# kazuotani14/iLQR

Hardware: AMD Instinct MI355X
Metric: iLQR iterations/sec (batch x T timesteps/sec), acrobot T=500 batch=4096 (higher is better)
Workload: dtype f64; 1 GPU; acrobot n=4 m=1 T=499 (500 knots), box-QP limits active, FD derivatives + backward/box-QP + 11-alpha search + accept, fixed work; batch_per_gpu=4096, global_batch=4096, T=499, parallelism=batch shards x1, one all_gather of costs

## Files before the change

### ilqr_amd/batch.py

```python
import ctypes as C

import numpy as np

from . import capi

ALPHAS = np.array([1.0000, 0.5012, 0.2512, 0.1259, 0.0631, 0.0316, 0.0158, 0.0079, 0.0040,
                   0.0020, 0.0010])
STATUS_NAMES = {0: "running", 1: "converged_grad", 2: "converged_cost", 3: "lambda_max", 4: "max_iter"}
_MODELS = {"acrobot": (capi.MODEL_ACROBOT, 4, 1), "double_integrator": (capi.MODEL_DOUBLE_INTEGRATOR, 4, 2),
           "integrator": (capi.MODEL_DOUBLE_INTEGRATOR, 4, 2),
           "host": (capi.MODEL_HOST, None, None),
           "lq": (capi.MODEL_LQ, None, None),
           "user": (capi.MODEL_USER, None, None)}
_dp = C.POINTER(C.c_double)
_ip = C.POINTER(C.c_int)


def _c(a):
    return np.ascontiguousarray(a, dtype=np.float64)


def _p(a):
    return a.ctypes.data_as(_dp) if a is not None else None

# ... 397 lines not shown
        nw = int(C.shape[-1])
        Cc = self._mat_input(C, self.nx, nw)
        B, T, n, m = self.B, self.T, self.nx, self.nu
        o = dict(K=np.zeros((B, T, n, m)) if K else None,
                 k=np.zeros((B, T, m)) if k else None, Vx=np.zeros((B, T + 1, n)) if Vx else None,
                 Vxx=np.zeros((B, T + 1, n, n)) if Vxx else None, risk_cost=np.zeros(B) if risk_cost else None)
        flags = np.zeros(B, dtype=np.int32) if info else None
        self._check(self.lib.ilqr_get_risk_sensitive(self.h, nw, float(theta), capi.LQ_HOLD_CLAMPED if hold_clamped else 0, float(mu), _p(Cc),
                                                     _p(o["K"]), _p(o["k"]), _p(o["Vx"]), _p(o["Vxx"]), _p(o["risk_cost"]), _pi(flags)))
        out = {name: (np.swapaxes(a, -1, -2) if name in ("K", "Vxx") else a) for name, a in o.items() if a is not None}
        if info:
            out["info"] = flags
        return out

    def copy_risk_sensitive_to_device(self, nw, theta, C_ptr, mu=0.0, hold_clamped=False, K_ptr=None, k_ptr=None, Vx_ptr=None, Vxx_ptr=None,
                                      risk_cost_ptr=None, info_ptr=None):
        self._check(self.lib.ilqr_copy_risk_sensitive_to_device(self.h, int(nw), float(theta), capi.LQ_HOLD_CLAMPED if hold_clamped else 0,
                                                                float(mu), C_ptr, K_ptr, k_ptr, Vx_ptr, Vxx_ptr, risk_cost_ptr, info_ptr))

    def _dirs_input(self, a, lead, width, what):
        if a is None:
            return None, None, False
        a = _c(a)
        flat = a.ndim == 2 + len(lead)
        if flat:
            a = np.ascontiguousarray(a[..., None, :])
        if a.ndim != 3 + len(lead) or a.shape[:1 + len(lead)] != (self.B,) + lead or a.shape[-1] != width or a.shape[-2] < 1:
            raise ValueError("%s must be %s, or the same without the direction axis S; got %s" % (what, ["B"] + list(lead) + ["S", width], a.shape))
        return a, a.shape[-2], flat

    def _dirs_pair(self, x, u, what):
        (x, Sx, fx), (u, Su, fu) = x, u
        if x is None and u is None:
            raise ValueError("%s are both None: the answer would be zero" % what)
        if x is not None and u is not None and (Sx != Su or fx != fu):
            raise ValueError("%s disagree on the directions: %s and %s" % (what, x.shape, u.shape))
        return (Sx if x is not None else Su), (fx if x is not None else fu)

    def _nku(self, t0, n):
        return max(min(int(t0) + n, self.T) - int(t0), 0)

    def tangent(self, dx0=None, dv=None, t0=0, n=None):
        n = self.T + 1 - int(t0) if n is None else int(n)
        X, V = self._dirs_input(dx0, (), self.nx, "dx0"), self._dirs_input(dv, (self.T,), self.nu, "dv")
        S, flat = self._dirs_pair(X, V, "dx0 and dv")
        nku = self._nku(t0, n)
        dxs = np.zeros((self.B, max(n, 0), S, self.nx))
        dus = np.zeros((self.B, nku, S, self.nu))
        self._check(self.lib.ilqr_get_tangent(self.h, int(t0), n, S, _p(X[0]), _p(V[0]), _p(dxs), _p(dus) if nku else None))
        return (dxs[:, :, 0], dus[:, :, 0]) if flat else (dxs, dus)

    def adjoint(self, gx=None, gu=None, t0=0, n=None):
        n = self.T + 1 - int(t0) if n is None else int(n)
        nku = self._nku(t0, n)
        X, U = self._dirs_input(gx, (max(n, 0),), self.nx, "gx"), self._dirs_input(gu, (nku,), self.nu, "gu")
        S, flat = self._dirs_pair(X, U, "gx and gu")
        g_x0, g_v = np.zeros((self.B, S, self.nx)), np.zeros((self.B, self.T, S, self.nu))
        self._check(self.lib.ilqr_get_adjoint(self.h, int(t0), n, S, _p(X[0]), _p(U[0]), _p(g_x0), _p(g_v)))
        return (g_x0[:, 0], g_v[:, :, 0]) if flat else (g_x0, g_v)

    def transition_matrices(self, t0=0, n=None):
        dxs, dus = self.tangent(dx0=np.broadcast_to(np.eye(self.nx), (self.B, self.nx, self.nx)), t0=t0, n=n)
        return np.swapaxes(dxs, -1, -2), np.swapaxes(dus, -1, -2)

    def copy_tangent_to_device(self, t0, n, S, dx0_ptr=None, dv_ptr=None, dxs_ptr=None, dus_ptr=None):
        self._check(self.lib.ilqr_copy_tangent_to_device(self.h, int(t0), int(n), int(S), dx0_ptr, dv_ptr, dxs_ptr, dus_ptr))

    def copy_adjoint_to_device(self, t0, n, S, gx_ptr=None, gu_ptr=None, g_x0_ptr=None, g_v_ptr=None):
        self._check(self.lib.ilqr_copy_adjoint_to_device(self.h, int(t0), int(n), int(S), gx_ptr, gu_ptr, g_x0_ptr, g_v_ptr))

    def lq_solve(self, gx=None, gu=None, dx0=None, mu=0.0, hold_clamped=True, dlam=False):
        X = self._dirs_input(gx, (self.T + 1,), self.nx, "gx")
        U = self._dirs_input(gu, (self.T,), self.nu, "gu")
        X0 = self._dirs_input(dx0, (), self.nx, "dx0")
        given = [a for a in (X, U, X0) if a[0] is not None]
        if not given:
            raise ValueError("gx, gu and dx0 are all None: the answer would be zero")
        S, flat = given[0][1], given[0][2]
        if any(a[1] != S or a[2] != flat for a in given):
            raise ValueError("gx, gu and dx0 disagree on the directions: %s" % [a[0].shape for a in given])
        dxs, dus = np.zeros((self.B, self.T + 1, S, self.nx)), np.zeros((self.B, self.T, S, self.nu))
        lam = np.zeros((self.B, self.T + 1, S, self.nx)) if dlam else None
        info = np.zeros(self.B, dtype=np.int32)
        self._check(self.lib.ilqr_solve_lq(self.h, S, capi.LQ_HOLD_CLAMPED if hold_clamped else 0, float(mu), _p(X0[0]), _p(X[0]), _p(U[0]), _p(dxs),
                                           _p(dus), _p(lam), _pi(info)))
        out = (dxs, dus) + ((lam,) if dlam else ())
        if flat:
            out = tuple(a[:, :, 0] for a in out)
        return out + (info,)

    def copy_lq_solve_to_device(self, S, mu=0.0, hold_clamped=True, dx0_ptr=None, gx_ptr=None, gu_ptr=None, dxs_ptr=None, dus_ptr=None, dlam_ptr=None,
                                info_ptr=None):
        self._check(self.lib.ilqr_solve_lq_on_device(self.h, int(S), capi.LQ_HOLD_CLAMPED if hold_clamped else 0, float(mu), dx0_ptr, gx_ptr, gu_ptr,
                                                     dxs_ptr, dus_ptr, dlam_ptr, info_ptr))

    def derivatives(self):
        n, m, B, T1 = self.nx, self.nu, self.B, self.T + 1
        mem = dict(fx=np.zeros((B, T1, n, n)), fu=np.zeros((B, T1, m, n)), cx=np.zeros((B, T1, n)),
                   cu=np.zeros((B, T1, m)), cxx=np.zeros((B, T1, n, n)), cxu=np.zeros((B, T1, m, n)),
                   cuu=np.zeros((B, T1, m, m)))
        order = ("fx", "fu", "cx", "cu", "cxx", "cxu", "cuu")
        self._check(self.lib.ilqr_get_derivatives(self.h, *[_p(mem[k]) for k in order]))
        return {k: (v if k in ("cx", "cu") else np.swapaxes(v, -1, -2)) for k, v in mem.items()}

    def cost(self):
        c = np.zeros(self.B)
        self._check(self.lib.ilqr_get_cost(self.h, _p(c)))
        return c

    def lambdas(self):
        lam, dlam = np.zeros(self.B), np.zeros(self.B)
        self._check(self.lib.ilqr_get_lambda(self.h, _p(lam), _p(dlam)))
        return lam, dlam

    def dV(self):
        d = np.zeros((self.B, 2))
        self._check(self.lib.ilqr_get_dV(self.h, _p(d)))
        return d

    def gnorm(self):
        g = np.zeros(self.B)
        self._check(self.lib.ilqr_get_gnorm(self.h, _p(g)))
        return g

    def status(self):
        st, it, al = (np.zeros(self.B, dtype=np.int32) for _ in range(3))
        self._check(self.lib.ilqr_get_status(self.h, st.ctypes.data_as(_ip), it.ctypes.data_as(_ip),
                                            al.ctypes.data_as(_ip)))
        return st, it, al

    def candidate(self, a):
        xs = np.zeros((self.B, self.T + 1, self.nx))
        us = np.zeros((self.B, self.T, self.nu))
        self._check(self.lib.ilqr_get_candidate(self.h, int(a), _p(xs), _p(us)))
        return xs, us

    def count_running(self):
        n = C.c_int(0)
        self._check(self.lib.ilqr_count_running(self.h, C.byref(n)))
        return n.value

    def profile(self, enable=True):
        self._check(self.lib.ilqr_profile_enable(self.h, int(enable)))

    def profile_reset(self):
        self._check(self.lib.ilqr_profile_reset(self.h))

    def profile_read(self):
        ms = (C.c_double * capi.NUM_STAGES)()
        n = (C.c_int * capi.NUM_STAGES)()
        self._check(self.lib.ilqr_profile_read(self.h, ms, n))
        return {capi.STAGE_NAMES[i]: (ms[i], n[i]) for i in range(capi.NUM_STAGES)}

    def shader_clock_mhz(self):
        mhz = C.c_double(0)
        self._check(self.lib.ilqr_profile_shader_clock(self.h, C.byref(mhz)))
        return mhz.value
```

### ilqr_amd/capi.py

```python
import ctypes as C
import os

from . import _build

ABI_VERSION = 6
MODEL_ACROBOT, MODEL_DOUBLE_INTEGRATOR, MODEL_LQ, MODEL_HOST, MODEL_USER = 0, 1, 2, 3, 4
FLAG_FIXED_WORK, FLAG_BACKWARD_THREAD_PER_TRAJ, _FLAG_RESERVED_4, FLAG_UNFUSED, FLAG_ANALYTIC_DERIVATIVES, FLAG_STAGED, FLAG_REFERENCE_FIXES, FLAG_REGULARIZE_VXX = 1, 2, 4, 8, 16, 32, 64, 128
DTYPE_F64, DTYPE_F32 = 0, 1
TAIL_HOLD, TAIL_ZERO = 0, 1
RESET_NONFINITE, RESET_LAMBDA_MAX = 1, 2
WAS_MASKED, WAS_NONFINITE, WAS_LAMBDA_MAX = 1, 2, 4
WAS_CLONED, CLONE_REFUSED = 1, 2
LQ_HOLD_CLAMPED = 1
EVAL_CLAMP = 1
ROUTE_TILE_PER_CU, ROUTE_TWO_TILES_PER_CU, ROUTE_WIDE_TILES = 1, 2, 3
ROUTE_WIDE_ONE_PER_CU, ROUTE_WIDE_TWO_PER_CU, ROUTE_NO_COMPACTION, ROUTE_FULL_RECORDS, ROUTE_LQ_THREAD_ROLLOUT, ROUTE_QUAD_CHAIN, ROUTE_LQ_RECOMMIT, ROUTE_BACKWARD_W2, ROUTE_LQ_DENSE_FD = 4, 8, 16, 32, 64, 256, 512, 1024, 2048
ROUTE_WAVE_PER_TRAJECTORY = 4096
ROUTE_TWO_CONTROL_TILES = 8192
NUM_STAGES = 5
STAGE_NAMES = ("derivatives", "backward", "rollout", "accept", "solve")

_dp = C.POINTER(C.c_double)
_ip = C.POINTER(C.c_int)


class Params(C.Structure):
    _fields_ = [("max_iter", C.c_int), ("tol_fun", C.c_double), ("tol_grad", C.c_double),
                ("lambda_init", C.c_double), ("dlambda_init", C.c_double),
                ("lambda_factor", C.c_double), ("lambda_max", C.c_double),
                ("lambda_min", C.c_double), ("z_min", C.c_double)]


class Desc(C.Structure):
    _fields_ = [("abi_version", C.c_int), ("model", C.c_int), ("nx", C.c_int), ("nu", C.c_int),
                ("T", C.c_int), ("B", C.c_int), ("dt", C.c_double), ("device", C.c_int),
                ("flags", C.c_int), ("dtype", C.c_int), ("u_min", _dp), ("u_max", _dp), ("goal", _dp),
                ("lq_A", _dp), ("lq_B", _dp), ("lq_Q", _dp), ("lq_R", _dp), ("lq_Qf", _dp),
                ("stream", C.c_void_p), ("params", C.POINTER(Params)), ("user_params", _dp), ("n_user_params", C.c_int),
                ("route", C.c_int), ("assume_cus", C.c_int)]


_H = C.c_void_p
SYMBOLS = {
    "ilqr_last_error": (C.c_char_p, []),
    "ilqr_abi_version": (C.c_int, []),
    "ilqr_has_user_model": (C.c_int, []),
    "ilqr_default_params": (None, [C.POINTER(Params)]),
    "ilqr_create": (C.c_int, [C.POINTER(Desc), C.POINTER(_H)]),
    "ilqr_destroy": (None, [_H]),
    "ilqr_set_stream": (C.c_int, [_H, C.c_void_p]),
    "ilqr_synchronize": (C.c_int, [_H]),
    "ilqr_init_traj": (C.c_int, [_H, _dp, _dp, _dp]),
    "ilqr_generate_trajectory": (C.c_int, [_H]),
    "ilqr_solve": (C.c_int, [_H, _dp, _dp]),
    "ilqr_warm_start": (C.c_int, [_H, _dp]),
    "ilqr_iterate": (C.c_int, [_H, C.c_int]),
    "ilqr_shift_horizon": (C.c_int, [_H, C.c_int, C.c_int]),
    "ilqr_mpc_step": (C.c_int, [_H, _dp, C.c_void_p, C.c_int, C.c_int, C.c_int]),
    "ilqr_copy_controls_to_device": (C.c_int, [_H, C.c_int, C.c_int, C.c_void_p]),
    "ilqr_set_reset_controls": (C.c_int, [_H, _dp, C.c_void_p]),
    "ilqr_reset_trajectories": (C.c_int, [_H, _ip, C.c_void_p, C.c_int]),
    "ilqr_mpc_step_reset": (C.c_int, [_H, _dp, C.c_void_p, C.c_int, C.c_int, C.c_int, _ip, C.c_void_p, C.c_int]),
    "ilqr_get_reset_flags": (C.c_int, [_H, _ip]),
    "ilqr_copy_reset_flags_to_device": (C.c_int, [_H, C.c_void_p]),
    "ilqr_select_best": (C.c_int, [_H, C.c_int, _ip, C.c_void_p]),
    "ilqr_clone_trajectories": (C.c_int, [_H, _ip, C.c_void_p, C.c_void_p]),
    "ilqr_clone_best": (C.c_int, [_H, C.c_int, C.c_void_p]),
    "ilqr_get_clone_flags": (C.c_int, [_H, _ip]),
    "ilqr_copy_clone_flags_to_device": (C.c_int, [_H, C.c_void_p]),
    "ilqr_get_value": (C.c_int, [_H, C.c_int, C.c_int, _dp, _dp]),
    "ilqr_copy_value_to_device": (C.c_int, [_H, C.c_int, C.c_int, C.c_void_p, C.c_void_p]),
    "ilqr_get_covariance": (C.c_int, [_H, C.c_int, C.c_int, _dp, _dp, _dp, _dp, _dp]),
    "ilqr_copy_covariance_to_device": (C.c_int, [_H, C.c_int, C.c_int, C.c_void_p, C.c_void_p, C.c_void_p, C.c_void_p, C.c_void_p]),
    "ilqr_get_tangent": (C.c_int, [_H, C.c_int, C.c_int, C.c_int, _dp, _dp, _dp, _dp]),
    "ilqr_copy_tangent_to_device": (C.c_int, [_H, C.c_int, C.c_int, C.c_int, C.c_void_p, C.c_void_p, C.c_void_p, C.c_void_p]),
    "ilqr_get_adjoint": (C.c_int, [_H, C.c_int, C.c_int, C.c_int, _dp, _dp, _dp, _dp]),
    "ilqr_copy_adjoint_to_device": (C.c_int, [_H, C.c_int, C.c_int, C.c_int, C.c_void_p, C.c_void_p, C.c_void_p, C.c_void_p]),
    "ilqr_solve_lq": (C.c_int, [_H, C.c_int, C.c_int, C.c_double, _dp, _dp, _dp, _dp, _dp, _dp, _ip]),
    "ilqr_solve_lq_on_device": (C.c_int, [_H, C.c_int, C.c_int, C.c_double, C.c_void_p, C.c_void_p, C.c_void_p, C.c_void_p, C.c_void_p, C.c_void_p, C.c_void_p]),
    "ilqr_get_estimator": (C.c_int, [_H, C.c_int, C.c_int, C.c_int, _dp, _dp, _dp, _dp, _dp, _dp, _dp, _dp, _dp, _dp, _ip]),
    "ilqr_copy_estimator_to_device": (C.c_int, [_H, C.c_int, C.c_int, C.c_int] + [C.c_void_p] * 11),
    "ilqr_get_risk_sensitive": (C.c_int, [_H, C.c_int, C.c_double, C.c_int, C.c_double, _dp, _dp, _dp, _dp, _dp, _dp, _ip]),
    "ilqr_copy_risk_sensitive_to_device": (C.c_int, [_H, C.c_int, C.c_double, C.c_int, C.c_double] + [C.c_void_p] * 7),
    "ilqr_evaluate_policy": (C.c_int, [_H, C.c_int, C.c_int, C.c_int, C.c_int, _dp, _dp, _dp, _dp]),
    "ilqr_evaluate_policy_on_device": (C.c_int, [_H, C.c_int, C.c_int, C.c_int, C.c_int, C.c_void_p, C.c_void_p, C.c_void_p, C.c_void_p]),
    "ilqr_trajectory_params_count": (C.c_int, []),
    "ilqr_set_trajectory_params": (C.c_int, [_H, _dp, C.c_void_p, C.c_int]),
    "ilqr_get_trajectory_params": (C.c_int, [_H, _dp, C.c_int]),
    "ilqr_clear_trajectory_params": (C.c_int, [_H]),
    "ilqr_get_param_gradient": (C.c_int, [_H, C.c_int, C.c_int, C.c_double, _dp, _dp, _dp, _dp, _dp]),
    "ilqr_param_gradient_on_device": (C.c_int, [_H, C.c_int, C.c_int, C.c_double] + [C.c_void_p] * 5),
    "ilqr_compute_derivatives": (C.c_int, [_H]),
    "ilqr_backward_pass": (C.c_int, [_H, _ip]),
    "ilqr_backward_step": (C.c_int, [_H]),
    "ilqr_rollout_candidates": (C.c_int, [_H, _dp]),
    "ilqr_line_search": (C.c_int, [_H]),
    "ilqr_accept_candidates": (C.c_int, [_H, _dp, _ip]),
    "ilqr_reset_state": (C.c_int, [_H, C.c_int]),
    "ilqr_set_trajectory": (C.c_int, [_H, _dp, _dp, _dp, _dp]),
    "ilqr_set_gains": (C.c_int, [_H, _dp, _dp]),
    "ilqr_set_derivatives": (C.c_int, [_H] + [_dp] * 7),
    "ilqr_set_lambda": (C.c_int, [_H, _dp, _dp]),
    "ilqr_get_trajectory": (C.c_int, [_H, _dp, _dp]),
    "ilqr_get_gains": (C.c_int, [_H, _dp, _dp]),
    "ilqr_get_derivatives": (C.c_int, [_H] + [_dp] * 7),
    "ilqr_get_cost": (C.c_int, [_H, _dp]),
    "ilqr_get_lambda": (C.c_int, [_H, _dp, _dp]),
    "ilqr_get_dV": (C.c_int, [_H, _dp]),
    "ilqr_get_gnorm": (C.c_int, [_H, _dp]),
    "ilqr_get_status": (C.c_int, [_H, _ip, _ip, _ip]),
    "ilqr_get_candidate": (C.c_int, [_H, C.c_int, _dp, _dp]),
    "ilqr_count_running": (C.c_int, [_H, _ip]),
    "ilqr_copy_cost_to_device": (C.c_int, [_H, C.c_void_p]),
    "ilqr_copy_trajectory_to_device": (C.c_int, [_H, C.c_void_p, C.c_void_p]),
    "ilqr_copy_gains_to_device": (C.c_int, [_H, C.c_void_p, C.c_void_p]),
    "ilqr_get_results_async": (C.c_int, [_H, _dp, _dp, _dp, _dp, _dp]),
    "ilqr_host_register": (C.c_int, [C.c_void_p, C.c_size_t]),
    "ilqr_host_unregister": (C.c_int, [C.c_void_p]),
    "ilqr_group_create": (C.c_int, [C.POINTER(_H), C.c_int, C.c_int, C.POINTER(C.c_void_p)]),
    "ilqr_group_destroy": (None, [C.c_void_p]),
    "ilqr_group_gather_costs": (C.c_int, [C.c_void_p, _dp]),
    "ilqr_group_uses_rccl": (C.c_int, [C.c_void_p, _ip]),
    "ilqr_profile_enable": (C.c_int, [_H, C.c_int]),
    "ilqr_profile_reset": (C.c_int, [_H]),
    "ilqr_profile_read": (C.c_int, [_H, _dp, _ip]),
    "ilqr_profile_shader_clock": (C.c_int, [_H, _dp]),
    "ilqr_stage_kernel_name": (C.c_char_p, [_H, C.c_int]),
}

_lib = None
_libs = {}


class ILQRError(RuntimeError):
    pass


def lib_path():
    return _build.LIB


def _bind(path):
    lib = C.CDLL(path)
    for name, (res, args) in SYMBOLS.items():
        fn = getattr(lib, name)
        fn.restype = res
        fn.argtypes = args
    return lib


def load(build_if_missing=True, path=None):
    global _lib
    if path is not None:
        path = os.path.abspath(path)
        if path not in _libs:
            if not os.path.exists(path):
                raise ILQRError("%s is missing: build it with ilqr_amd._build.build_user(header, out)" % path)
            _libs[path] = _bind(path)
        return _libs[path]
    if _lib is None:
        if build_if_missing and os.path.exists(_build.HIPCC):
            _build.build()
        if not os.path.exists(_build.LIB):
            raise ILQRError("libilqr_amd.so is missing (%s): build it with "
                            "`python -m ilqr_amd._build`; there is no fallback path" % _build.LIB)
        lib = C.CDLL(os.environ.get("ILQR_AMD_LIB", _build.LIB))
        for name, (res, args) in SYMBOLS.items():
            fn = getattr(lib, name)
            fn.restype = res
            fn.argtypes = args
        _lib = lib
    return _lib


def check(rc, lib=None):
    if rc != 0:
        msg = (lib or load()).ilqr_last_error()
        raise ILQRError("libilqr_amd error %d: %s" % (rc, msg.decode() if msg else "?"))
```

### ilqr_amd/csrc/backward_hex.hpp

```cpp
#pragma once
#include "solve_tile.hpp"

namespace ilqr {

#ifndef ILQR_COMMIT_ROLLED
#define ILQR_COMMIT_ROLLED 1
#endif

#ifndef ILQR_COMMIT_BATCH
#define ILQR_COMMIT_BATCH 2
#endif
constexpr int kCommitBatch = ILQR_COMMIT_BATCH;

constexpr int HT = 4;
#ifndef ILQR_HEX_SLOT_PAD
#define ILQR_HEX_SLOT_PAD 8
#endif
#ifndef ILQR_HEX_PAIR_PERM
#define ILQR_HEX_PAIR_PERM 1
#endif
#ifndef ILQR_HEX_CAND_T
#define ILQR_HEX_CAND_T 1
#endif
constexpr bool kHexCandT = ILQR_HEX_CAND_T != 0;
#ifndef ILQR_HEX_QUAD_ROLLOUT
#define ILQR_HEX_QUAD_ROLLOUT 1
#endif
constexpr bool kHexQuadRollout = ILQR_HEX_QUAD_ROLLOUT != 0;
#ifndef ILQR_HEX_SLOT_PHASES
#define ILQR_HEX_SLOT_PHASES 4
#endif
constexpr int kHexSlotPhases = ILQR_HEX_SLOT_PHASES;
static_assert(kHexSlotPhases == 1 || kHexSlotPhases == 2 || kHexSlotPhases == 4, "backward_hex's step loop is written out for groups of 1, 2 or 4 knots");
#ifndef ILQR_HEX_MFMA_SPREAD
#define ILQR_HEX_MFMA_SPREAD 0
#endif
constexpr bool kHexMfmaSpread = ILQR_HEX_MFMA_SPREAD != 0;

template <int NX, int NU, class real, int SLOTS_, bool COMPACT_ = false>
struct HexRing {
  static constexpr bool COMPACT = COMPACT_;
  static constexpr int US = Rec<NX, NU>::SIZE;
  static constexpr int PAIRS = COMPACT ? CompactRec<NX, NU>::PAIRS : (Rec<NX, NU>::SIZE + NU + 1) / 2;
  static constexpr int ROW = 2 * HT;
  static constexpr int PAD = ROW - 2 * TW;
  static constexpr int ELEMS = PAIRS * ROW + ILQR_HEX_SLOT_PAD;
  static constexpr int Z = PAIRS * ROW;
  static_assert(!COMPACT || ILQR_HEX_SLOT_PAD >= ROW, "the compact slot keeps Z in its pad row");
  static_assert(!COMPACT || (NX == 4 && NU == 1), "compact slots: nx = 4, nu = 1");
  static constexpr int SLOTS = SLOTS_;
  static constexpr bool PERM = (ILQR_HEX_PAIR_PERM != 0) && NX == 4 && NU == 1;
  static constexpr int pos(int pair) { return PERM && (!COMPACT || pair < 8) ? hex_pair_pos(pair) : pair; }
};

constexpr int kHexKnotsPerRound = 64 / HT;
constexpr int kHexFullSlots = 24;
template <int NX, int NU, class real, bool COMPACT>
struct HexRingSize {
  using Full = HexRing<NX, NU, real, kHexFullSlots, false>;
  static constexpr int TERM = COMPACT ? ((NX + NX * NX) / 2) * Full::ROW : 0;
  static constexpr int FIT = COMPACT ? (kHexFullSlots * Full::ELEMS - TERM) / HexRing<NX, NU, real, 1, COMPACT>::ELEMS : kHexFullSlots;
  static constexpr int SLOTS = FIT / kHexSlotPhases * kHexSlotPhases;
  static_assert(SLOTS % kHexSlotPhases == 0 && kHexKnotsPerRound % kHexSlotPhases == 0, "the ring and a producer round are whole groups of slots");
  static constexpr int LEAD = SLOTS - kHexKnotsPerRound - 1;
  static constexpr int STALE = kHexSlotPhases - 1;
  static_assert(SLOTS > LEAD + kHexKnotsPerRound - 1, "a round must not reach a slot the chain has not left");
  static_assert(LEAD - STALE >= 1, "the producer is released ahead of the chain, the published index being up to STALE knots old");
  static_assert(SLOTS * HexRing<NX, NU, real, 1, COMPACT>::ELEMS + TERM <= kHexFullSlots * Full::ELEMS, "the pair's records fit the bytes of 24 full slots");
};

template <class real, int N>
struct HexTerm {
  alignas(16) real term[N];
};
template <class real>
struct HexTerm<real, 0> {
  static constexpr real* term = nullptr;
};

template <class real, int NX, int NU, bool COMPACT = false>
struct HexPair : HexTerm<real, HexRingSize<NX, NU, real, COMPACT>::TERM> {
  using Size = HexRingSize<NX, NU, real, COMPACT>;
  using RS = HexRing<NX, NU, real, Size::SLOTS, COMPACT>;
  static constexpr int LEAD = Size::LEAD;
  alignas(16) real ring[RS::SLOTS * RS::ELEMS];
  int rounds_done;
  int consumer_at;
  int passes_started;
  unsigned long long pass_lanes;
};

template <class P>
struct HexGate {
  static constexpr bool kRing = true;
  static constexpr int NPH = kHexSlotPhases;
  static constexpr int GROUP = NPH * P::RS::ELEMS, RING = P::RS::SLOTS * P::RS::ELEMS;
  P& sh;
  const int T, nrounds, N;
  int pass = -1, have = 0;
  int g_grp = 0, off_grp = 0;
  __device__ __forceinline__ HexGate(P& s, int T_) : sh(s), T(T_), nrounds((T_ + 1 + kHexKnotsPerRound - 1) / kHexKnotsPerRound), N(nrounds * kHexKnotsPerRound) {}
  __device__ __forceinline__ int begin_pass() {
    pass++;
    have = pass * N;
    g_grp = pass * N;
    const int was = off_grp;
    off_grp = (g_grp % P::RS::SLOTS) * P::RS::ELEMS;
    __hip_atomic_store(&sh.pass_lanes, __ballot(1), __ATOMIC_RELAXED, __HIP_MEMORY_SCOPE_WORKGROUP);
    __hip_atomic_store(&sh.passes_started, pass + 1, __ATOMIC_RELEASE, __HIP_MEMORY_SCOPE_WORKGROUP);
    return off_grp - was;
  }
  __device__ __forceinline__ int next_group() {
    g_grp += NPH;
    const int d = (off_grp + GROUP == RING) ? GROUP - RING : GROUP;
    off_grp += d;
    return d;
  }
  template <int PH>
  __device__ __forceinline__ void wait() {
    if constexpr (PH != 0) return;
    const int G = g_grp;
    __hip_atomic_store(&sh.consumer_at, G, __ATOMIC_RELAXED, __HIP_MEMORY_SCOPE_WORKGROUP);
    if (G < have) return;
    const int round = pass * nrounds + (G - pass * N) / kHexKnotsPerRound;
    while (__hip_atomic_load(&sh.rounds_done, __ATOMIC_ACQUIRE, __HIP_MEMORY_SCOPE_WORKGROUP) <= round) __builtin_amdgcn_s_sleep(1);
    have = pass * N + ((G - pass * N) / kHexKnotsPerRound + 1) * kHexKnotsPerRound;
  }
  __device__ __forceinline__ void finish() {
    __hip_atomic_store(&sh.consumer_at, 0x3fffffff, __ATOMIC_RELAXED, __HIP_MEMORY_SCOPE_WORKGROUP);
    __hip_atomic_store(&sh.passes_started, -1, __ATOMIC_RELEASE, __HIP_MEMORY_SCOPE_WORKGROUP);
  }
};

__device__ __forceinline__ int hex_first(unsigned long long bal, int t4) {
  return __builtin_ctzll(((bal >> t4) & 0x000F000F000F000Full) | 0x8000000000000000ull);
}
template <class Under>
__device__ __forceinline__ void qp1_search_hex(QP1StateT<double>& q, int j, int t4, double step_j0, const double* __restrict__ lds_steps, Under under_read) {
  const double t_x1 = clamp_of(q.x + step_j0 * q.search, q.lo, q.hi);
  const double t_v1 = qp1_value(q, t_x1);
  const bool t_pass = !qp1_armijo_fails(q, t_v1, step_j0);
  const int pp = hex_first(__ballot(t_pass), t4);
  const bool success = pp < 52;
  const int jw = success ? (((pp >> 4) << 2) | (pp & 3)) : 0;
#ifdef ILQR_EXP_NO_STEP_LDS
  const double step_w = jw == 0 ? 1.0 : 0.6;
#else
  const double step_w = lds_steps[jw];
#endif
  under_read();
  q.step = step_w;
  q.x1 = clamp_of(q.x + q.step * q.search, q.lo, q.hi);
  q.v1 = qp1_value(q, q.x1);
  bool more = p_and(!success, !q.early);
  if (__builtin_expect(__ballot(more) == 0ull, 1)) return;
  {
    const bool stuck = p_and(j >= 1, t_x1 == q.x);
    const int qs = hex_first(__ballot(p_and(stuck, more)), t4);
    if (p_and(more, qs < 52)) {
      q.ls_failed = true;
      more = false;
    }
    if (__ballot(more) == 0ull) return;
  }
  for (int base = 16;; base += 16) {
    const int kn = base + j;
    const double my_step = lds_steps[kn < 104 ? kn : 103];
    const double my_x1 = qp1_trial(q, my_step);
    const double my_v1 = qp1_value(q, my_x1);
    const bool pass = !qp1_armijo_fails(q, my_v1, my_step);
    const bool stuck = p_or(my_step < kMinStep, my_x1 == q.x);
    const int qp = hex_first(__ballot(p_and(pass, more)), t4), qs = hex_first(__ballot(p_and(stuck, more)), t4);
    if (more) {
      if (qp < qs) {
        q.step = lds_steps[base + (((qp >> 4) << 2) | (qp & 3))];
        q.x1 = qp1_trial(q, q.step);
        q.v1 = qp1_value(q, q.x1);
        more = false;
      } else if (qs < 52) {
        q.ls_failed = true;
        more = false;
      }
    }
    if (__ballot(more) == 0ull) return;
  }
}

template <class RS>
__device__ __forceinline__ int hex_pos_rt(int pair) { return RS::pos(pair); }

template <class real>
struct HexStep {
  typedef real pair_t __attribute__((ext_vector_type(2)));
  real F, cxx_rc, cxx_cr, fu_r, cx_r, cxu_r, cxu_c;
  pair_t tail, uw;
};

template <class M, class Gate, class RS>
__device__ __forceinline__ void backward_hex(const BatchViewT<typename M::real>& v, const M& model, const SolverParams& sp, int mode, int tile, int sub,
                                             int lane, const double* __restrict__ lds_steps, Gate& gate, const typename M::real* __restrict__ ring,
                                             const typename M::real* __restrict__ term ) {
  using real = typename M::real;
  using creal = double;
  static_assert(M::NX == 4 && M::NU == 1, "hex chain: nx = 4, nu = 1");
  using R = Rec<4, 1>;
  typedef real real2_t __attribute__((ext_vector_type(2)));
  const int r_ = lane >> 4, t_ = (lane >> 2) & 3, c_ = lane & 3, j16 = 4 * r_ + c_;
  const int t4 = 4 * t_;
  const int l = sub * HT + t_;
  const int b = tile * TW + l;
  if (b >= v.B) return;
  if (mode == 1 && v.status[b] != 0) return;
  const int T = v.T;
  double lambda = v.lambda[b], dlambda = v.dlambda[b];
  const real* __restrict__ ust = v.us + tidx(tile, 0, 0, l, T, 1);
  real* __restrict__ kt = v.kff + tidx(tile, 0, 0, l, T, 1);
  real* __restrict__ Kt = v.Kfb + tidx(tile, 0, 0, l, T, 4);
  typedef const __attribute__((address_space(3))) real lds_cd;
  typedef const __attribute__((address_space(3))) real2_t lds_cd2;
  const creal step_j0 = lds_steps[j16];
  auto mm = [](creal a, creal bb) __attribute__((always_inline)) { return __builtin_amdgcn_mfma_f64_4x4x4f64(a, bb, 0.0, 0, 0, 0); };

  using C = CompactRec<4, 1>;
  enum { A_ROW, A_FX, A_FU, A_CXX_RC, A_CXX_CR, A_CX, A_CXU_R, A_CXU_C, A_FULL };
  constexpr int NADDR = RS::COMPACT ? A_FU + 1 : A_FULL;
  lds_cd* at[NADDR];
  {
    lds_cd* r = (lds_cd*)(ring + t_ * 2);
    auto one = [&](int e) { return r + hex_pos_rt<RS>(e >> 1) * RS::ROW + (e & 1); };
    at[A_ROW] = r;
    at[A_FX] = one((RS::COMPACT ? C::FX : R::FX) + r_ + 4 * c_);
    at[A_FU] = one((RS::COMPACT ? C::FU : R::FU) + r_);
    if constexpr (!RS::COMPACT) {
      at[A_CXX_RC] = one(R::CXX + r_ + 4 * c_);
      at[A_CXX_CR] = one(R::CXX + c_ + 4 * r_);
      at[A_CX] = one(R::CX + r_);
      at[A_CXU_R] = one(R::CXU + r_);
      at[A_CXU_C] = one(R::CXU + c_);
    }
  }
  auto move = [&](int d) __attribute__((always_inline)) {
#pragma unroll
    for (int a = 0; a < NADDR; a++) at[a] += d;
  };
  constexpr int NPH = kHexSlotPhases;
  auto load = [&](auto phase, HexStep<real>& d) __attribute__((always_inline)) {
    constexpr int PH = decltype(phase)::value, o = PH * RS::ELEMS;
    gate.template wait<PH>();
    auto pair = [&](int e) { return *(lds_cd2*)(at[A_ROW] + o + RS::pos(e >> 1) * RS::ROW); };
    if constexpr (RS::COMPACT) {
      d.F = at[A_FX][o];
      d.fu_r = at[A_FU][o];
      d.cxx_rc = d.cxx_cr = d.cx_r = d.cxu_r = d.cxu_c = at[A_ROW][o + RS::Z];
      d.tail = pair(C::CU);
      d.uw = pair(C::US);
    } else {
      d.F = at[A_FX][o];
      d.cxx_rc = at[A_CXX_RC][o];
      d.cxx_cr = at[A_CXX_CR][o];
      d.fu_r = at[A_FU][o];
      d.cx_r = at[A_CX][o];
      d.cxu_r = at[A_CXU_R][o];
      d.cxu_c = at[A_CXU_C][o];
      d.tail = pair(R::CU);
      d.uw = pair(RS::US);
    }
    if constexpr (PH == NPH - 1) move(gate.next_group());
  };

  int diverge = 0;
  bool done = false;
  double dV0 = 0, dV1 = 0, gacc = 0;
  auto one_pass = [&]() __attribute__((always_inline)) {
    move(gate.begin_pass());
    creal V, RVx, kprev;
    const creal lam_r = (creal)lambda;
    {
      gate.template wait<0>();
      if constexpr (RS::COMPACT) {
        lds_cd* r = (lds_cd*)(term + t_ * 2);
        RVx = (creal)r[((C::TERM_CX + r_) >> 1) * RS::ROW + ((C::TERM_CX + r_) & 1)];
        V = (creal)r[((C::TERM_CXX + r_ + 4 * c_) >> 1) * RS::ROW + ((C::TERM_CXX + r_ + 4 * c_) & 1)];
      } else {
        RVx = (creal)at[A_CX][0];
        V = (creal)at[A_CXX_RC][0];
      }
      if constexpr (NPH == 1) move(gate.next_group());
    }
    kprev = (creal)kt[(unsigned)((T - 1) * TW)];
    __builtin_amdgcn_s_waitcnt(0x0F70);
    dV0 = dV1 = 0;
    diverge = 0;
    gacc = 0;
    real* __restrict__ Kt_i = Kt + (unsigned)(((T - 1) * 4 + c_) * TW);
    real* __restrict__ kt_i = kt + (unsigned)((T - 1) * TW);

    auto step = [&](auto phase, int i, const HexStep<real>& raw, HexStep<real>& nxt) -> bool {
      const creal F = (creal)raw.F, Rfu = (creal)raw.fu_r;
      const creal cu = (creal)raw.tail.x, cuu = (creal)raw.tail.y, us = (creal)raw.uw.x, usw = (creal)raw.uw.y;
      creal W, aQx, Tm, Tt, aQux_c, aQux_r;
      auto products_1 = [&]() __attribute__((always_inline)) {
        W = mm(V, F);
        aQx = mm(F, RVx);
        Tm = mm(F, W);
      };
      auto products_2 = [&]() __attribute__((always_inline)) {
        Tt = mm(W, F);
        aQux_c = mm(Rfu, W);
        aQux_r = mm(W, Rfu);
      };
      const creal wv = mm(V, Rfu);
      const creal aQu = mm(Rfu, RVx);
      const creal aQuu = mm(Rfu, wv);
      if constexpr (!kHexMfmaSpread) {
        products_1();
        products_2();
      }
      const creal Qu = cu + aQu;
      const creal Quu = cuu + aQuu, QuuF = (cuu + lam_r) + aQuu;
      const creal lo = (creal)model.u_min[0] - us, hi = (creal)model.u_max[0] - us;
      __builtin_amdgcn_sched_barrier(0);
      if (i >= 1) load(phase, nxt);
      __builtin_amdgcn_sched_barrier(0);
      creal x;
      int free0;
      creal minv;
      QP1StateT<creal> q1;
      qp1_begin<false>(QuuF, Qu, kprev, lo, hi, q1, false);
      qp1_search_hex(q1, j16, t4, step_j0, lds_steps, [&]() __attribute__((always_inline)) {
        if constexpr (kHexMfmaSpread) {
          __builtin_amdgcn_sched_barrier(0);
          products_1();
          __builtin_amdgcn_sched_barrier(0);
        }
      });
      if constexpr (kHexMfmaSpread) products_2();
      bool goes_on;
      bool ok = qp1_finish_ok(q1, x, free0, minv, goes_on);
      if (goes_on)
        ok = qp1_continue(
                 q1, [&](QP1StateT<creal>& qs) __attribute__((always_inline)) { qp1_search_hex(qs, j16, t4, step_j0, lds_steps, [] {}); }, x, free0) >= 1;
      if (!ok) diverge = i;
      const creal Qxx_rc = (creal)raw.cxx_rc + Tm, Qxx_cr = (creal)raw.cxx_cr + Tt;
      const creal Qx_r = (creal)raw.cx_r + aQx;
      const creal Qux_c = (creal)raw.cxu_c + aQux_c, Qux_r = (creal)raw.cxu_r + aQux_r;
      const creal k_scale = free0 ? -minv : creal(0);
      const creal K_r = k_scale * Qux_r, K_c = k_scale * Qux_c;
      creal d0 = 0, d1 = 0;
      {
        d0 += x * Qu;
        creal rq = 0;
        rq += (creal(0.5) * x) * Quu;
        d1 += rq * x;
      }
      creal T1_r, T1_c;
      {
        creal acc = 0;
        acc += K_r * Quu;
        T1_r = acc;
      }
      {
        creal acc = 0;
        acc += K_c * Quu;
        T1_c = acc;
      }
      creal Vxn_r, Vn_rc, Vn_cr;
      {
        creal t1 = 0, t2 = 0, t3 = 0;
        t1 += T1_r * x;
        t2 += K_r * Qu;
        t3 += Qux_r * x;
        Vxn_r = ((Qx_r + t1) + t2) + t3;
      }
      {
        creal u1 = 0, u2 = 0, u3 = 0;
        u1 += T1_r * K_c;
        u2 += K_r * Qux_c;
        u3 += Qux_r * K_c;
        Vn_rc = ((Qxx_rc + u1) + u2) + u3;
      }
      {
        creal u1 = 0, u2 = 0, u3 = 0;
        u1 += T1_c * K_r;
        u2 += K_c * Qux_r;
        u3 += Qux_c * K_r;
        Vn_cr = ((Qxx_cr + u1) + u2) + u3;
      }
      V = creal(0.5) * (Vn_rc + Vn_cr);
      RVx = Vxn_r;
      if (ok) {
        dV0 += (double)d0;
        dV1 += (double)d1;
        gacc += (double)(abs_of(x) * usw);
        kprev = (creal)(real)x;
        Kt_i[0] = (real)K_c;
        kt_i[0] = (real)x;
      }
      Kt_i -= 4 * TW;
      kt_i -= TW;
      return ok;
    };

    HexStep<real> A, Bd;
    int i = T - 1;
    auto ph = [](auto n) { return std::integral_constant<int, decltype(n)::value % NPH>(); };
    load(ph(std::integral_constant<int, 1>()), A);
    while (true) {
      if (!step(ph(std::integral_constant<int, 2>()), i, A, Bd)) break;
      if (--i < 0) break;
      if (!step(ph(std::integral_constant<int, 3>()), i, Bd, A)) break;
      if (--i < 0) break;
      if constexpr (NPH == 4) {
        if (!step(ph(std::integral_constant<int, 4>()), i, A, Bd)) break;
        if (--i < 0) break;
        if (!step(ph(std::integral_constant<int, 5>()), i, Bd, A)) break;
        if (--i < 0) break;
      }
    }
  };

  while (true) {
    one_pass();
    if (mode == 0) {
      done = (diverge == 0);
      break;
    }
    if (diverge != 0) {
      dlambda = raised_dlambda(dlambda, sp);
      lambda = raised_lambda(lambda, dlambda, sp);
      if (lambda > sp.lambda_max) break;
      continue;
    }
    done = true;
    break;
  }

  double acc = gacc;
  if (!done) {
    __builtin_amdgcn_fence(__ATOMIC_RELEASE, "workgroup");
    __builtin_amdgcn_s_waitcnt(0);
    acc = 0;
    for (int t0 = 0; t0 < T; t0 += 8) {
      real kv[8], uv[8];
#pragma unroll
      for (int jj = 0; jj < 8; jj++) {
        const int t = (t0 + jj < T) ? t0 + jj : T - 1;
        kv[jj] = kt[(size_t)t * TW];
        uv[jj] = ust[(size_t)t * TW];
      }
#pragma unroll
      for (int jj = 0; jj < 8; jj++) {
        const real mx = abs_of(kv[jj]) / (abs_of(uv[jj]) + 1);
        if (t0 + jj < T) acc += (double)mx;
      }
    }
  }
  const double gnorm = acc / T;
  if (j16 == 0) {
    v.dV[b] = dV0;
    v.dV[v.Bp + b] = dV1;
    v.diverge[b] = diverge;
    v.backpass_done[b] = done ? 1 : 0;
    v.gnorm[b] = gnorm;
    if (mode == 1) {
      v.lambda[b] = lambda;
      v.dlambda[b] = dlambda;
      if (!sp.fixed_work && gnorm < sp.tol_grad && lambda < kLambdaConverged) {
        v.status[b] = 1;
        v.iters[b] += 1;
      }
    }
  }
}

template <class M, class MFD, class P>
__device__ __forceinline__ void sweep_backward_hex(const BatchViewT<typename M::real>& v, const M& model, const MFD& fdm, const SolverParams& sp, int mode,
                                                   int force, int tile, P* pairs, const double* __restrict__ lds_steps, int role) {
  using RS = typename P::RS;
  const int lane = threadIdx.x & 63;
  if (threadIdx.x < 4) {
    pairs[threadIdx.x].rounds_done = 0;
    pairs[threadIdx.x].consumer_at = 0;
    pairs[threadIdx.x].passes_started = 0;
  }
  __syncthreads();
  const int T = v.T;
  P& sh = pairs[role & 3];
  if (role < 4) {
    __builtin_amdgcn_s_setprio(3);
    HexGate<P> gate(sh, T);
    backward_hex<M, decltype(gate), RS>(v, model, sp, mode, tile, role, lane, lds_steps, gate, sh.ring, sh.term);
    gate.finish();
    __builtin_amdgcn_s_setprio(0);
  } else {
    const int sub = role - 4;
    const int lp = lane & (HT - 1), ks = lane >> 2;
    const int l = sub * HT + lp;
    const int nrounds = (T + 1 + kHexKnotsPerRound - 1) / kHexKnotsPerRound, N = nrounds * kHexKnotsPerRound;
    for (int pass = 0;; pass++) {
      unsigned long long lanes = ~0ull;
      if (pass > 0) {
        int started;
        while ((started = __hip_atomic_load(&sh.passes_started, __ATOMIC_ACQUIRE, __HIP_MEMORY_SCOPE_WORKGROUP)) >= 0 && started <= pass)
          __builtin_amdgcn_s_sleep(8);
        if (started < 0) break;
        lanes = __hip_atomic_load(&sh.pass_lanes, __ATOMIC_RELAXED, __HIP_MEMORY_SCOPE_WORKGROUP);
      }
      const bool mine = (lanes >> (4 * lp)) & 1ull;
      for (int r = 0; r < nrounds; r++) {
        const int j0 = r * kHexKnotsPerRound, G0 = pass * N + j0;
        while (G0 > __hip_atomic_load(&sh.consumer_at, __ATOMIC_RELAXED, __HIP_MEMORY_SCOPE_WORKGROUP) + P::LEAD) __builtin_amdgcn_s_sleep(4);
        const int started = __hip_atomic_load(&sh.passes_started, __ATOMIC_RELAXED, __HIP_MEMORY_SCOPE_WORKGROUP);
        if ((started < 0) | (started > pass + 1)) break;
        const int t = T - (j0 + ks);
        if (t >= 0 && (pass == 0 || mine)) {
          typename M::real* rs = sh.ring + ((G0 + ks) % RS::SLOTS) * RS::ELEMS + lp * 2;
          if constexpr (RS::COMPACT) {
            if (t == T) rs = sh.term + lp * 2;
          }
          derivatives_of_knot<M, true, MFD, RS::PAD, RS::PERM, RS::COMPACT>(v, model, fdm, force, nullptr, tile, t, l, rs, true);
        }
        __builtin_amdgcn_s_waitcnt(0xC07F);
        if (lane == 0) __hip_atomic_store(&sh.rounds_done, pass * nrounds + r + 1, __ATOMIC_RELEASE, __HIP_MEMORY_SCOPE_WORKGROUP);
      }
    }
  }
}

template <class M, bool CANDT = false>
__device__ __forceinline__ void commit_tile_chunks(const BatchViewT<typename M::real>& v, const M& model, const int* commit_of_lane , int tile) {
  using real = typename M::real;
  constexpr int NX = M::NX, NU = M::NU;
  static_assert(!CANDT || (NX == 4 && NU == 1 && CT == 8 && CG == 4), "grouped candidates: nx = 4, nu = 1");
  static_assert(HT == kQuad, "a chain wavefront rolls out its own sub-tile");
  const int T = v.T;
  const real dt = (real)v.dt;
  const int ntask = v.nch * TW;
  struct Task {
    int l, c;
    real x[NX], uq[CT][NU];
  };
  auto load = [&](int task, Task& k) __attribute__((always_inline)) {
    k.l = 0;
    k.c = -1;
    if (task < 0) return;
    const int l = task & (TW - 1), c = task >> 4;
    const int b = tile * TW + l;
    const int ci = (b < v.B) ? commit_of_lane[l] : -1;
    if (ci < 0) return;
    k.l = l;
    k.c = c;
    const int ta = ci * v.ntiles + tile;
    real* const x = k.x;
    real(*const uq)[NU] = k.uq;
    if constexpr (CANDT) {
      typedef real real4v __attribute__((ext_vector_type(4)));
      const real4v xv = *reinterpret_cast<const real4v*>(v.cand_x + cand_g_x(ta, c, l, v.nch, NX));
      x[0] = xv.x;
      x[1] = xv.y;
      x[2] = xv.z;
      x[3] = xv.w;
      const real4v u0 = *reinterpret_cast<const real4v*>(v.cand_u + cand_g_u(ta, 2 * c, l, T));
      const real4v u1 = *reinterpret_cast<const real4v*>(v.cand_u + cand_g_u(ta, 2 * c + 1, l, T));
      uq[0][0] = u0.x;
      uq[1][0] = u0.y;
      uq[2][0] = u0.z;
      uq[3][0] = u0.w;
      uq[4][0] = u1.x;
      uq[5][0] = u1.y;
      uq[6][0] = u1.z;
      uq[7][0] = u1.w;
    } else {
#pragma unroll
    for (int i = 0; i < NX; i++) x[i] = v.cand_x[tidx(ta, c, i, l, v.nch, NX)];
#pragma unroll
    for (int q = 0; q < CT; q++) {
      const int tq = (c * CT + q < T) ? c * CT + q : T - 1;
#pragma unroll
      for (int jj = 0; jj < NU; jj++) uq[q][jj] = v.cand_u[tidx(ta, tq, jj, l, T, NU)];
    }
    }
  };
  auto steps = [&](Task& k) __attribute__((always_inline)) {
    if (k.c < 0) return;
    const int l = k.l, c = k.c;
    real* const x = k.x;
    real(*const uq)[NU] = k.uq;
#if ILQR_COMMIT_ROLLED
#pragma unroll 1
    for (int q = 0; q < CT; q++) {
      const int t = c * CT + q;
      if (t > T) break;
#pragma unroll
      for (int i = 0; i < NX; i++) v.xs[tidx(tile, t, i, l, T + 1, NX)] = x[i];
      if (t < T) {
#pragma unroll
        for (int jj = 0; jj < NU; jj++) v.us[tidx(tile, t, jj, l, T, NU)] = uq[0][jj];
        if (q + 1 < CT) {
          real x1[NX];
          integrate_dynamics(model, x, uq[0], dt, x1);
#pragma unroll
          for (int i = 0; i < NX; i++) x[i] = x1[i];
        }
      }
#pragma unroll
      for (int qq = 0; qq + 1 < CT; qq++)
#pragma unroll
        for (int jj = 0; jj < NU; jj++) uq[qq][jj] = uq[qq + 1][jj];
    }
#else
#pragma unroll
    for (int q = 0; q < CT; q++) {
      const int t = c * CT + q;
      if (t <= T) {
#pragma unroll
        for (int i = 0; i < NX; i++) v.xs[tidx(tile, t, i, l, T + 1, NX)] = x[i];
        if (t < T) {
#pragma unroll
          for (int jj = 0; jj < NU; jj++) v.us[tidx(tile, t, jj, l, T, NU)] = uq[q][jj];
          if (q + 1 < CT) {
            real x1[NX];
            integrate_dynamics(model, x, uq[q], dt, x1);
#pragma unroll
            for (int i = 0; i < NX; i++) x[i] = x1[i];
          }
        }
      }
    }
#endif
  };
  for (int first = ntask - 1 - (int)threadIdx.x; first >= 0; first -= kCommitBatch * (int)blockDim.x) {
    Task k[kCommitBatch];
#pragma unroll
    for (int j = 0; j < kCommitBatch; j++) load(first - j * (int)blockDim.x, k[j]);
#pragma unroll
    for (int j = 0; j < kCommitBatch; j++) steps(k[j]);
  }
}

template <class M, class MFD>
__global__ __launch_bounds__(512) __attribute__((amdgpu_waves_per_eu(2, 2))) void k_solve_hex(BatchViewT<typename M::real> v, M model, MFD fdm, AlphaSet alphas,
                                                                                                 SolverParams sp, int n_iters, int force,
                                                                                                 int* __restrict__ commit_idx, int commit_pending,
                                                                                                 long long* __restrict__ phase_ticks) {
  using real = typename M::real;
  using P = HexPair<real, M::NX, M::NU, state_free_running_cost<M>::value>;
  __shared__ P pairs[4];
  __shared__ double steps[104];
  __shared__ double lds_cost[NALPHA * TW];
  __shared__ int tile_running;
  __shared__ int simd_count[4];
  __shared__ int lds_commit[TW];
  if (threadIdx.x < 4) simd_count[threadIdx.x] = 0;
  load_step_table(steps);
  const int wave = (int)(threadIdx.x >> 6);
  int role = wave;
  {
    const int simd = hw_simd_id();
    int slot = 0;
    if ((threadIdx.x & 63) == 0) slot = atomicAdd(&simd_count[simd], 1);
    slot = __shfl(slot, 0, 64);
    __syncthreads();
    if (simd_count[0] == 2 && simd_count[1] == 2 && simd_count[2] == 2 && simd_count[3] == 2) role = simd + 4 * slot;
  }
  const int rwave = kHexQuadRollout ? ((role < 4) ? role : 4) : ((role < 3) ? role : 3);
  const int tile = blockIdx.x;
  constexpr int kShareReals = 4 * ((2 * M::NU + M::NU * M::NX + M::NX + 3) / 4) * TW;
  static_assert(kShareReals <= (int)(sizeof(pairs[0].ring) / sizeof(real)), "a pair's ring holds a wavefront's rollout rows");
  long long t_sweep = 0, t_roll = 0, t0 = 0;
#ifdef ILQR_HEX_SECTIONS
  long long t_sweep_last = 0;
#endif
  const bool timing = (phase_ticks != nullptr) & (threadIdx.x == 0);
  const long long c_begin = timing ? clock64() : 0, w_begin = timing ? wall_clock64() : 0;
  if (commit_pending) {
    commit_tile_chunks<M>(v, model, commit_idx + tile * TW, tile);
    phase_barrier();
  }
  int it = 0;
  for (; it < n_iters; it++) {
    if (timing) t0 = wall_clock64();
    sweep_backward_hex<M, MFD, P>(v, model, fdm, sp, 1, force, tile, pairs, steps, role);
    phase_barrier();
    if (timing) {
      const long long t1 = wall_clock64();
#ifdef ILQR_HEX_SECTIONS
      t_sweep_last = t1 - t0;
#endif
      t_sweep += t1 - t0;
      t0 = t1;
    }
    rollout_tile<M, true, true, kDeepPrefetch<M>, true, true, true, 1, kHexCandT, kHexQuadRollout>(v, model, alphas, NALPHA, v.cost_c, 1, sp, commit_idx, tile, lds_cost, it == n_iters - 1, rwave,
                                               pairs[role & 3].ring);
#ifdef ILQR_HEX_SECTIONS
#define ILQR_HEX_MARK(n)                                   \
    if (ILQR_HEX_SECTIONS == n && timing) {                \
      const long long t1 = wall_clock64();                 \
      t_sweep = t_sweep - t_sweep_last + (t1 - t0);        \
      t0 = t1;                                             \
    }
#else
#define ILQR_HEX_MARK(n)
#endif
    ILQR_HEX_MARK(1)
    if (threadIdx.x < TW) lds_commit[threadIdx.x] = commit_idx[tile * TW + threadIdx.x];
    if (threadIdx.x == 0) tile_running = 0;
    phase_barrier();
    ILQR_HEX_MARK(2)
    commit_tile_chunks<M, kHexCandT>(v, model, lds_commit, tile);
    ILQR_HEX_MARK(3)
    phase_barrier();
    if (timing) t_roll += wall_clock64() - t0;
    if (!sp.fixed_work) {
      const int b = tile * TW + (int)threadIdx.x;
      if (threadIdx.x < TW && b < v.B && v.status[b] == 0) tile_running = 1;
      __syncthreads();
      if (!tile_running) {
        it++;
        break;
      }
    }
  }
  if (timing) {
    phase_ticks[5 * tile + 0] += t_sweep;
    phase_ticks[5 * tile + 1] += t_roll;
    phase_ticks[5 * tile + 2] += it;
    phase_ticks[5 * tile + 3] += clock64() - c_begin;
    phase_ticks[5 * tile + 4] += wall_clock64() - w_begin;
  }
}

}
```

### ilqr_amd/csrc/capi.hip

```cpp
#include "../../include/ilqr_amd.h"

#include <stdarg.h>
#include <stdio.h>
#include <limits.h>
#include <string.h>

#include <algorithm>
#include <cstdlib>
#include <string>
#include <vector>

#include "backward_wave.hpp"
#include "backward_wave2.hpp"
#include "backward_wave3.hpp"
#include "generic.hpp"
#include "kernels_wide.hpp"
#include "kernels_wide2.hpp"
#include "kernels.hpp"
#include "value_thread.hpp"
#include "value_wave.hpp"
#include "covariance_thread.hpp"
#include "covariance_wave.hpp"
#include "sensitivity_thread.hpp"
#include "sensitivity_wave.hpp"
#include "lq_solve_thread.hpp"
#include "lq_solve_wave.hpp"
#include "estimator_thread.hpp"
#include "estimator_wave.hpp"
#include "risk_thread.hpp"
#include "risk_wave.hpp"
#include "evaluate.hpp"
#include "param_gradient.hpp"
#include "clone.hpp"

using namespace ilqr;

#include "route.hpp"
#include "handle.hpp"
#include "launch.hpp"

extern "C" {

const char* ilqr_last_error(void) { return g_err; }
int ilqr_abi_version(void) { return ILQR_AMD_ABI_VERSION; }
int ilqr_has_user_model(void) {
#ifdef ILQR_HAVE_USER_MODEL
  return 1;
#else
  return 0;
#endif
}

void ilqr_default_params(ilqr_params* p) {
  p->max_iter = 100;
  p->tol_fun = 1e-6;
  p->tol_grad = 1e-6;
  p->lambda_init = 1;
  p->dlambda_init = 1;
  p->lambda_factor = 1.6;
  p->lambda_max = 1e11;
  p->lambda_min = 1e-8;
  p->z_min = 0;
}

void ilqr_destroy(ilqr_batch* h) {
  if (!h) return;
  (void)hipSetDevice(h->device);
  if (h->stream) (void)hipStreamSynchronize(h->stream);
#ifdef ILQR_W2_TIMING
  if (h->aos) {
    long long st[8], qp[8], cnt[4];
    if (hipMemcpyFromSymbol(st, HIP_SYMBOL(g_w2_cycles), sizeof(st)) == hipSuccess && hipMemcpyFromSymbol(qp, HIP_SYMBOL(g_q_cycles), sizeof(qp)) == hipSuccess &&
        hipMemcpyFromSymbol(cnt, HIP_SYMBOL(g_q_counts), sizeof(cnt)) == hipSuccess && cnt[0] > 0) {
      const double q = (double)cnt[0];
      fprintf(stderr, "[k_backward_w2, wavefront 0] shader cycles per step: load+Qx/Qu %.0f  Vxx'fx,Vxx'fu %.0f  Qxx/Qux/Quu %.0f  box-QP %.0f  K %.0f  dV+T1+Vx %.0f  Vn+symmetrise+stores %.0f  (loop top %.0f)\n",
              st[0] / q, st[1] / q, st[2] / q, st[3] / q, st[4] / q, st[5] / q, st[6] / q, st[7] / q);
      fprintf(stderr, "[box-QP] per QP: %.2f iterations, %.2f factorisations, %.2f Armijo trips beyond the first; cycles: gradient+clamp set %.0f  Cholesky %.0f  inverse+R^-1R^-T %.0f  direction %.0f  line search %.0f  rest %.0f\n",
              cnt[1] / q, cnt[2] / q, cnt[3] / q, qp[0] / q, qp[1] / q, qp[2] / q, qp[3] / q, qp[4] / q, qp[5] / q);
    }
    long long w3[4];
    if (hipMemcpyFromSymbol(w3, HIP_SYMBOL(g_w3_counts), sizeof(w3)) == hipSuccess && w3[0] + w3[1] > 0)
      fprintf(stderr, "[k_backward_w3, wavefront 0] box-QPs on the matrix-core path %lld, handed to the literal path %lld, Newton-Schulz iterations per refinement %.2f\n",
              w3[0], w3[1], (double)w3[2] / (double)(w3[0] > 0 ? w3[0] : 1));
  }
#endif
  for (void* p : h->allocs) (void)hipFree(p);
  if (h->staging) (void)hipFree(h->staging);
  if (h->lq_scratch) (void)hipFree(h->lq_scratch);
  if (h->est_scratch) (void)hipFree(h->est_scratch);
  if (h->pg_scratch) (void)hipFree(h->pg_scratch);
  if (h->d_perm) (void)hipFree(h->d_perm);
  if (h->perm_scratch) (void)hipFree(h->perm_scratch);
  (void)timers_drain(h);
  for (hipEvent_t e : h->event_pool) (void)hipEventDestroy(e);
  if (h->own_stream && h->stream) (void)hipStreamDestroy(h->stream);
  delete h;
}

static int check_desc(const ilqr_desc* d) {
  REQUIRE(d->abi_version == ILQR_AMD_ABI_VERSION || d->abi_version == 5, "ABI version %d, library is %d (accepts 5 and %d)", d->abi_version,
          ILQR_AMD_ABI_VERSION, ILQR_AMD_ABI_VERSION);
  REQUIRE(d->B >= 1 && d->T >= 1 && d->nx >= 1 && d->nu >= 1, "B, T, nx, nu must be positive");
  REQUIRE(d->nx <= MAXN && d->nu <= kMaxControls, "nx <= %d and nu <= %d", MAXN, kMaxControls);
  REQUIRE(d->dt > 0, "dt must be positive");
  if (d->route & 128)
    return fail(ILQR_ERR_UNSUPPORTED, "route bit 128 (round 1's LDS kernel k_backward_w) was retired in ABI 5: ILQR_ROUTE_BACKWARD_W2 gives the same bits");
  if ((d->route & ILQR_ROUTE_WIDE_TWO_PER_CU) && d->nu == 2 && d->nx == 4)
    return fail(ILQR_ERR_UNSUPPORTED, "ILQR_ROUTE_WIDE_TWO_PER_CU: the m = 2 wide tiles (k_solve_wide2) run one tile per CU (four wavefronts at <= 512 registers); the bit applies to k_solve_wide (m = 1)");
  if (d->dtype != ILQR_DTYPE_F64 && d->dtype != ILQR_DTYPE_F32) return fail(ILQR_ERR_INVALID, "dtype %d: ILQR_DTYPE_F64 or ILQR_DTYPE_F32", d->dtype);
  if (d->nu > WM) {
    const char* what = (d->dtype == ILQR_DTYPE_F32) ? "fp32" : (d->route & ILQR_ROUTE_BACKWARD_W2) ? "ILQR_ROUTE_BACKWARD_W2" : (d->route & ILQR_ROUTE_LQ_DENSE_FD) ? "ILQR_ROUTE_LQ_DENSE_FD"
                       : (d->flags & ILQR_FLAG_REGULARIZE_VXX) ? "ILQR_FLAG_REGULARIZE_VXX" : nullptr;
    if (what) return fail(ILQR_ERR_UNSUPPORTED, "%s supports at most %d controls (nu = %d)", what, WM, d->nu);
  }
  if ((d->route & ILQR_ROUTE_TWO_CONTROL_TILES) && (d->route & ILQR_ROUTE_BACKWARD_W2))
    return fail(ILQR_ERR_UNSUPPORTED, "ILQR_ROUTE_TWO_CONTROL_TILES and ILQR_ROUTE_BACKWARD_W2 name two different backward kernels");
  if ((d->route & ILQR_ROUTE_TWO_CONTROL_TILES) && (d->flags & ILQR_FLAG_REGULARIZE_VXX))
    return fail(ILQR_ERR_UNSUPPORTED, "ILQR_FLAG_REGULARIZE_VXX is implemented in k_backward_w3 (at most 16 controls): drop ILQR_ROUTE_TWO_CONTROL_TILES");
  const bool aos = generic_layout(d->model, d->route, kUserTiled, kUserSmall);
  if (d->dtype == ILQR_DTYPE_F32 && aos) {
    if (d->model == ILQR_MODEL_HOST)
      return fail(ILQR_ERR_UNSUPPORTED, "fp32 is not available for ILQR_MODEL_HOST: the caller evaluates the model and owns its records (fp64)");
    if (d->route & ILQR_ROUTE_BACKWARD_W2)
      return fail(ILQR_ERR_UNSUPPORTED, "fp32 is not available on ILQR_ROUTE_BACKWARD_W2 (the literal-order fp64 cross-check): fp32 handles run k_backward_w3");
    if (d->route & ILQR_ROUTE_TWO_CONTROL_TILES)
      return fail(ILQR_ERR_UNSUPPORTED, "fp32 is not available on ILQR_ROUTE_TWO_CONTROL_TILES: fp32 handles run k_backward_w3 with one control tile");
  }
  if (d->model == ILQR_MODEL_ACROBOT) {
    REQUIRE(d->nx == 4 && d->nu == 1, "acrobot is nx=4 nu=1 (include/acrobot.h:27-28), got %d/%d", d->nx, d->nu);
  } else if (d->model == ILQR_MODEL_DOUBLE_INTEGRATOR) {
    REQUIRE(d->nx == 4 && d->nu == 2, "double integrator is nx=4 nu=2 (include/double_integrator.h:16-17), got %d/%d", d->nx, d->nu);
#ifdef ILQR_HAVE_USER_MODEL
  } else if (d->model == ILQR_MODEL_USER) {
    using UM = UserModelT<double>;
    REQUIRE(d->nx == UM::NX && d->nu == UM::NU, "this build's user model is nx=%d nu=%d, got %d/%d", UM::NX, UM::NU, d->nx, d->nu);
    REQUIRE(d->u_min && d->u_max, "ILQR_MODEL_USER needs u_min/u_max (Model::u_min/u_max, include/model.h:17)");
    REQUIRE(!(d->flags & ILQR_FLAG_ANALYTIC_DERIVATIVES) || has_analytic_record<UM>::value, "this user model has no analytic_record()");
    if (aos && kUserSmall) REQUIRE(d->dtype == ILQR_DTYPE_F64, "ILQR_ROUTE_WAVE_PER_TRAJECTORY on a small twin is the fp64 cross-check of its tiled kernels: fp64 only");
    REQUIRE(d->n_user_params >= 0 && (d->n_user_params == 0 || d->user_params), "ILQR_MODEL_USER: n_user_params = %d with user_params = %p", d->n_user_params, (const void*)d->user_params);
#endif
  } else if (d->model == ILQR_MODEL_HOST || d->model == ILQR_MODEL_LQ) {
    REQUIRE(d->nx <= WN && d->nu <= WMW, "generic kernels: nx <= %d, nu <= %d", WN, WMW);
    REQUIRE(d->u_min && d->u_max, "generic handles need u_min/u_max (Model::u_min/u_max, include/model.h:17)");
    if (d->model == ILQR_MODEL_LQ)
      REQUIRE(d->lq_A && d->lq_B && d->lq_Q && d->lq_R && d->lq_Qf, "ILQR_MODEL_LQ needs lq_A, lq_B, lq_Q, lq_R, lq_Qf");
  } else {
    return fail(ILQR_ERR_UNSUPPORTED, "model id %d is not available in this build", d->model);
  }
  if ((d->flags & ILQR_FLAG_REGULARIZE_VXX) && aos && (d->route & ILQR_ROUTE_BACKWARD_W2))
    return fail(ILQR_ERR_UNSUPPORTED, "ILQR_FLAG_REGULARIZE_VXX on the generic path is implemented in k_backward_w3: drop ILQR_ROUTE_BACKWARD_W2");
  return 0;
}

static void copy_desc(const ilqr_desc* d, ilqr_batch* h) {
  h->lq_wide = d->model == ILQR_MODEL_LQ && d->nu > WM;
  h->route.full_records = (d->route & ILQR_ROUTE_FULL_RECORDS) != 0;
  h->route.no_compaction = (d->route & ILQR_ROUTE_NO_COMPACTION) != 0;
  h->route.wide_occ = (d->route & ILQR_ROUTE_WIDE_ONE_PER_CU) ? 1 : (d->route & ILQR_ROUTE_WIDE_TWO_PER_CU) ? 2 : 0;
  h->aos = generic_layout(d->model, d->route, kUserTiled, kUserSmall);
  h->model = d->model; h->dtype = d->dtype; h->flags = d->flags;
  h->nx = d->nx; h->nu = d->nu; h->T = d->T; h->B = d->B; h->dt = d->dt;
  h->Bp = ((d->B + 63) / 64) * 64;
  h->ntiles = h->Bp / TW;
  if (d->params)
    h->params = *d->params;
  else
    ilqr_default_params(&h->params);
}

static int open_device(const ilqr_desc* d, ilqr_batch* h) {
  int ndev = 0;
  if (hipGetDeviceCount(&ndev) != hipSuccess || ndev <= 0)
    return fail(ILQR_ERR_NO_DEVICE, "no HIP device visible: libilqr_amd has no CPU path");
  if (d->device < 0 || d->device >= ndev) return fail(ILQR_ERR_NO_DEVICE, "device %d out of range (%d visible)", d->device, ndev);
  HIPCHK(hipSetDevice(d->device));
  h->device = d->device;
  HIPCHK(hipDeviceGetAttribute(&h->num_cus, hipDeviceAttributeMultiprocessorCount, d->device));
  if (d->assume_cus > 0) h->num_cus = d->assume_cus;
  int khz = 0;
  if (hipDeviceGetAttribute(&khz, hipDeviceAttributeWallClockRate, d->device) == hipSuccess && khz > 0) h->wall_clock_khz = khz;
  h->stream = (hipStream_t)d->stream;
  h->own_stream = !d->stream;
  if (h->own_stream) HIPCHK(hipStreamCreateWithFlags(&h->stream, hipStreamNonBlocking));
  return 0;
}

static void set_model_params(const ilqr_desc* d, ilqr_batch* h) {
  if (d->model == ILQR_MODEL_ACROBOT) {
    AcrobotModel& m = h->acrobot;
    m.goal[0] = 3.1415;
    m.goal[1] = m.goal[2] = m.goal[3] = 0;
    m.u_min[0] = d->u_min ? d->u_min[0] : -5.0;
    m.u_max[0] = d->u_max ? d->u_max[0] : 5.0;
    if (h->dtype == ILQR_DTYPE_F32) {
      AcrobotModelT<float>& f = h->acrobot_f;
      for (int i = 0; i < 4; i++) m.goal[i] = (double)(f.goal[i] = (float)m.goal[i]);
      m.u_min[0] = (double)(f.u_min[0] = (float)m.u_min[0]);
      m.u_max[0] = (double)(f.u_max[0] = (float)m.u_max[0]);
    }
  } else if (d->model == ILQR_MODEL_DOUBLE_INTEGRATOR) {
    DoubleIntegratorModel& m = h->dint;
    const double g0[4] = {1.0, 0.5, 0.0, 0.0};
    for (int i = 0; i < 4; i++) m.goal[i] = d->goal ? d->goal[i] : g0[i];
    for (int j = 0; j < 2; j++) {
      m.u_min[j] = d->u_min ? d->u_min[j] : -0.5;
      m.u_max[j] = d->u_max ? d->u_max[j] : 0.5;
    }
    if (h->dtype == ILQR_DTYPE_F32) {
      DoubleIntegratorModelT<float>& f = h->dint_f;
      for (int i = 0; i < 4; i++) m.goal[i] = (double)(f.goal[i] = (float)m.goal[i]);
      for (int j = 0; j < 2; j++) {
        m.u_min[j] = (double)(f.u_min[j] = (float)m.u_min[j]);
        m.u_max[j] = (double)(f.u_max[j] = (float)m.u_max[j]);
      }
    }
#ifdef ILQR_HAVE_USER_MODEL
  } else if (d->model == ILQR_MODEL_USER) {
    using UM = UserModelT<double>;
    h->user_f.set_params(d->user_params, d->n_user_params);
    if (h->dtype == ILQR_DTYPE_F32) {
      std::vector<double> p32(d->user_params, d->user_params + (d->user_params ? d->n_user_params : 0));
      for (double& q : p32) q = (double)(float)q;
      h->user.set_params(p32.data(), (int)p32.size());
    } else {
      h->user.set_params(d->user_params, d->n_user_params);
    }
    for (int j = 0; j < UM::NU; j++) {
      h->user_f.u_min[j] = (float)d->u_min[j];
      h->user_f.u_max[j] = (float)d->u_max[j];
      h->user.u_min[j] = (h->dtype == ILQR_DTYPE_F32) ? (double)h->user_f.u_min[j] : d->u_min[j];
      h->user.u_max[j] = (h->dtype == ILQR_DTYPE_F32) ? (double)h->user_f.u_max[j] : d->u_max[j];
    }
    static_cast<UM&>(h->user_g) = h->user;
    static_cast<UserModelT<float>&>(h->user_gf) = h->user_f;
#endif
  }
}

static int alloc_arrays(const ilqr_desc* d, ilqr_batch* h) {
  const size_t nt = h->ntiles, T = h->T, T1 = h->T + 1, nx = h->nx, nu = h->nu, REC = rec_of(h), Bp = h->Bp;
  BatchView& v = h->v;
  v.B = h->B; v.Bp = h->Bp; v.ntiles = h->ntiles; v.T = h->T; v.dt = h->dt;
  v.analytic = (h->flags & ILQR_FLAG_ANALYTIC_DERIVATIVES) ? 1 : 0;
  v.D = nullptr;
  int rc = 0;
  if (h->aos) {
    const size_t Bn = h->B;
    v.nch = 0;
    rc |= dev_alloc_real(h, &v.x0, Bn * nx);
    rc |= dev_alloc_real(h, &v.xs, Bn * T1 * nx);
    rc |= dev_alloc_real(h, &v.us, Bn * T * nu);
    rc |= dev_alloc_real(h, &v.kff, Bn * T * nu);
    rc |= dev_alloc_real(h, &v.Kfb, Bn * T * nu * nx);
    rc |= dev_alloc(h, &h->const_rec, 2 * REC + GN);
    rc |= dev_alloc(h, &h->d_umin, nu);
    rc |= dev_alloc(h, &h->d_umax, nu);
    v.cand_u = nullptr;
    v.cand_x = nullptr;
    if (lq_matrix_core_search(d->model, d->nu, d->route) && !(d->route & ILQR_ROUTE_LQ_RECOMMIT) && d->dtype == ILQR_DTYPE_F64) {
      void *cx = nullptr, *cu = nullptr;
      if (hipMalloc(&cx, Bn * NALPHA * T1 * nx * sizeof(double)) == hipSuccess && hipMalloc(&cu, Bn * NALPHA * T * nu * sizeof(double)) == hipSuccess) {
        h->allocs.push_back(cx);
        h->allocs.push_back(cu);
        v.cand_x = (double*)cx;
        v.cand_u = (double*)cu;
      } else {
        if (cx) (void)hipFree(cx);
        (void)hipGetLastError();
      }
    }
  } else {
    rc |= dev_alloc_real(h, &v.x0, nt * nx * TW);
    const size_t slack = rollout_fetch_slack_elems(h->nx, h->nu);
    rc |= dev_alloc_real(h, &v.xs, nt * T1 * nx * TW + slack);
    rc |= dev_alloc_real(h, &v.us, nt * T * nu * TW + slack);
    rc |= dev_alloc_real(h, &v.kff, nt * T * nu * TW + slack);
    rc |= dev_alloc_real(h, &v.Kfb, nt * T * nu * nx * TW + slack);
    v.nch = h->T / CT + 1;
    rc |= dev_alloc_real(h, &v.cand_u, (size_t)(NALPHA + 1) * nt * (size_t)(cand_groups(T) * CG) * nu * TW);
    rc |= dev_alloc_real(h, &v.cand_x, (size_t)(NALPHA + 1) * nt * v.nch * nx * TW);
  }
  rc |= dev_alloc(h, &v.cost_c, (size_t)NALPHA * Bp);
  for (double** p : {&v.cost, &v.lambda, &v.dlambda, &v.gnorm}) rc |= dev_alloc(h, p, Bp);
  for (int** p : {&v.status, &v.iters, &v.flg_change, &v.alpha_idx, &v.diverge, &v.backpass_done, &h->commit_idx}) rc |= dev_alloc(h, p, Bp);
  rc |= dev_alloc(h, &v.dV, 2 * Bp);
  rc |= dev_alloc(h, &v.n_running, 1);
  rc |= dev_alloc(h, &h->x0_stage, (size_t)h->B * nx);
  rc |= dev_alloc(h, &h->phase_ticks, 5 * (size_t)h->ntiles);
  if (rc) return ILQR_ERR_HIP;
  HIPCHK(hipMemsetAsync(h->commit_idx, 0xFF, Bp * sizeof(int), h->stream));
  sync_float_view(h);
  return 0;
}

static int upload_generic_model(const ilqr_desc* d, ilqr_batch* h) {
  if (!h->aos) return 0;
  const size_t nx = h->nx, nu = h->nu;
  std::vector<double> hp;
  std::vector<float> hf;
  if (d->model == ILQR_MODEL_LQ) {
    const size_t GMC = h->lq_wide ? GMW : GM;
    const size_t nA = GN * GN, nB = GN * GMC, nR = GMC * GMC, tot = 3 * nA + nB + nR;
    double* pad = nullptr;
    if (int rc = dev_alloc(h, &pad, tot)) return rc;
    hp.assign(tot, 0.0);
    double *pA = hp.data(), *pB = pA + nA, *pQ = pB + nB, *pR = pQ + nA, *pQf = pR + nR;
    for (size_t i = 0; i < nx; i++) {
      for (size_t j = 0; j < nx; j++) {
        pA[i * GN + j] = d->lq_A[i * nx + j];
        pQ[i * GN + j] = d->lq_Q[i * nx + j];
        pQf[i * GN + j] = d->lq_Qf[i * nx + j];
      }
      for (size_t j = 0; j < nu; j++) pB[i * GMC + j] = d->lq_B[i * nu + j];
    }
    for (size_t i = 0; i < nu; i++)
      for (size_t j = 0; j < nu; j++) pR[i * GMC + j] = d->lq_R[i * nu + j];
    if (h->dtype == ILQR_DTYPE_F32) {
      float* padf = nullptr;
      if (int rc = dev_alloc(h, &padf, tot)) return rc;
      hf.resize(tot);
      for (size_t e = 0; e < tot; e++) hp[e] = (double)(hf[e] = (float)hp[e]);
      HIPCHK(hipMemcpyAsync(padf, hf.data(), tot * sizeof(float), hipMemcpyHostToDevice, h->stream));
      bind_lq(h->lq_f, padf, GMC, h);
    }
    HIPCHK(hipMemcpyAsync(pad, hp.data(), tot * sizeof(double), hipMemcpyHostToDevice, h->stream));
    bind_lq(h->lq, pad, GMC, h);
    bind_lq(h->lq_w, pad, GMC, h);
  }
  std::vector<double> lim(d->u_min, d->u_min + nu);
  lim.insert(lim.end(), d->u_max, d->u_max + nu);
  if (h->dtype == ILQR_DTYPE_F32)
    for (double& q : lim) q = (double)(float)q;
  HIPCHK(hipMemcpyAsync(h->d_umin, lim.data(), nu * sizeof(double), hipMemcpyHostToDevice, h->stream));
  HIPCHK(hipMemcpyAsync(h->d_umax, lim.data() + nu, nu * sizeof(double), hipMemcpyHostToDevice, h->stream));
  HIPCHK(hipStreamSynchronize(h->stream));
  return 0;
}

static int plan_and_reset(const ilqr_desc* d, ilqr_batch* h) {
  h->plan = plan_route({d->model, d->nx, d->nu, d->flags, d->route, h->ntiles, h->num_cus, kUserTiled, kUserSmall, h->v.cand_x != nullptr, d->dtype});
  SolverParams& sp = h->sp;
  const ilqr_params& p = h->params;
  sp.max_iter = p.max_iter; sp.tol_fun = p.tol_fun; sp.tol_grad = p.tol_grad; sp.z_min = p.z_min;
  sp.lambda_factor = p.lambda_factor; sp.lambda_max = p.lambda_max; sp.lambda_min = p.lambda_min;
  sp.fixed_work = (h->flags & ILQR_FLAG_FIXED_WORK) ? 1 : 0;
  sp.fixes = ((h->flags & ILQR_FLAG_REFERENCE_FIXES) ? 3 : 0) | ((h->flags & ILQR_FLAG_REGULARIZE_VXX) ? 4 : 0);
  if (int rc = launch_per_slot(h, k_reset_state<double>, h->v, p.lambda_init, p.dlambda_init)) return rc;
  if (h->plan.derivatives == Derivatives::fused_lq) {
    BatchView cv = h->v;
    if (h->dtype == ILQR_DTYPE_F32) cv.xs = h->const_rec + 2 * rec_of(h);
    hipLaunchKernelGGL(k_analytic_lq<double>, dim3(1), dim3(64), 0, h->stream, cv, h->lq, 1, 3, h->const_rec, kAnalyticChunk);
    HIPCHK(hipGetLastError());
  }
  HIPCHK(hipStreamSynchronize(h->stream));
  return 0;
}

static int create_impl(const ilqr_desc* d, ilqr_batch* h) {
  copy_desc(d, h);
  if (int rc = open_device(d, h)) return rc;
  set_model_params(d, h);
  if (int rc = alloc_arrays(d, h)) return rc;
  if (int rc = upload_generic_model(d, h)) return rc;
  return plan_and_reset(d, h);
}

int ilqr_create(const ilqr_desc* d, ilqr_batch** out) {
  if (!d || !out) return fail(ILQR_ERR_INVALID, "null argument");
  *out = nullptr;
  if (int rc = check_desc(d)) return rc;
  ilqr_batch* h = new ilqr_batch();
  const int rc = create_impl(d, h);
  if (rc) {
    char keep[sizeof(g_err)];
    memcpy(keep, g_err, sizeof(keep));
    if (rc != ILQR_ERR_NO_DEVICE) ilqr_destroy(h); else delete h;
    memcpy(g_err, keep, sizeof(keep));
    return rc;
  }
  *out = h;
  return 0;
}

int ilqr_set_stream(ilqr_batch* h, void* s) {
  if (!h) return fail(ILQR_ERR_INVALID, "null handle");
  HIPCHK(hipSetDevice(h->device));
  HIPCHK(hipStreamSynchronize(h->stream));
  if (h->own_stream) {
    HIPCHK(hipStreamDestroy(h->stream));
    h->own_stream = false;
  }
  if (s) {
    h->stream = (hipStream_t)s;
  } else {
    HIPCHK(hipStreamCreateWithFlags(&h->stream, hipStreamNonBlocking));
    h->own_stream = true;
  }
  return 0;
}

int ilqr_synchronize(ilqr_batch* h) {
  if (!h) return fail(ILQR_ERR_INVALID, "null handle");
  HIPCHK(hipSetDevice(h->device));
  HIPCHK(hipStreamSynchronize(h->stream));
  return 0;
}

int ilqr_init_traj(ilqr_batch* h, const double* x0, const double* u0, double* cost_out) {
  if (!h || !x0 || !u0) return fail(ILQR_ERR_INVALID, "null argument");
  if (host_model(h)) return no_device_model();
  HIPCHK(hipSetDevice(h->device));
  if (int rc = upload(h, x0, {h->v.x0, 1, h->nx})) return rc;
  if (int rc = upload(h, u0, {h->v.us, h->T, h->nu})) return rc;
  if (int rc = fresh_trajectory(h)) return rc;
  AlphaSet al = line_search_alphas();
  if (int rc = launch_rollout(h, false, false, al, 1, h->v.cost, 0)) return rc;
  h->initialised = true;
  if (cost_out) return scalars_to_host(h, h->v.cost, cost_out);
  return 0;
}

int ilqr_iterate(ilqr_batch* h, int n_iters) {
  if (!h) return fail(ILQR_ERR_INVALID, "null handle");
  if (host_model(h)) return no_device_model();
  if (!h->initialised) return fail(ILQR_ERR_STATE, "ilqr_iterate before ilqr_init_traj/ilqr_set_trajectory");
  HIPCHK(hipSetDevice(h->device));
  struct Chain {
    ilqr_batch* h;
    explicit Chain(ilqr_batch* hh) : h(hh) { h->chain_timers = true; h->chain_event = nullptr; }
    ~Chain() { h->chain_timers = false; h->chain_event = nullptr; }
  } chain(h);
  if (n_iters > 0) h->cands = (h->active_tiles > 0 && h->active_tiles < h->ntiles) ? Cands::none : Cands::planes;
  if (h->plan.solve != Solve::none && n_iters > 0) {
    if (int rc = launch_solve_tiles(h, n_iters)) return rc;
    return flush_commit(h);
  }
  for (int it = 0; it < n_iters; it++) {
    if (h->plan.sweep != Sweep::none) {
      if (int rc = launch_sweep_backward(h, 1, h->sp.fixed_work)) return rc;
    } else {
      if (int rc = launch_derivatives(h, h->sp.fixed_work)) return rc;
      if (int rc = launch_backward(h, 1)) return rc;
    }
    if (h->plan.rollout == Rollout::tiled || h->plan.rollout == Rollout::lq_accept) {
      if (int rc = launch_rollout(h, true, true, line_search_alphas(), NALPHA, h->v.cost_c, 1, true)) return rc;
      h->commit_pending = true;
    } else {
      if (int rc = do_rollout_candidates(h, 1)) return rc;
      if (int rc = launch_accept(h)) return rc;
    }
  }
  if (!h->aos && n_iters > 0) h->recs = ilqr_batch::REC_STALE;
  return flush_commit(h);
}

int ilqr_count_running(ilqr_batch* h, int* n) {
  if (!h || !n) return fail(ILQR_ERR_INVALID, "null argument");
  HIPCHK(hipSetDevice(h->device));
  std::vector<int> st(h->B);
  if (int rc = scalars_to_host(h, h->v.status, st.data())) return rc;
  int c = 0;
  for (int s : st) c += (s == 0);
  *n = c;
  return 0;
}

static int apply_permutation(ilqr_batch* h, const std::vector<int>& perm) {
  const size_t es = elem_size(h), Bp = (size_t)h->Bp;
  const size_t biggest = std::max<size_t>((size_t)h->ntiles * (h->T + 1) * h->nx * TW, (size_t)h->ntiles * h->T * h->nu * h->nx * TW) * es;
  const size_t need = std::max<size_t>(biggest, 2 * Bp * sizeof(double));
  if (h->perm_scratch_bytes < need) {
    if (h->perm_scratch) HIPCHK(hipFree(h->perm_scratch));
    h->perm_scratch = nullptr;
    HIPCHK(hipMalloc(&h->perm_scratch, need));
    h->perm_scratch_bytes = need;
  }
  if (!h->d_perm) HIPCHK(hipMalloc((void**)&h->d_perm, Bp * sizeof(int)));
  HIPCHK(hipMemcpyAsync(h->d_perm, perm.data(), Bp * sizeof(int), hipMemcpyHostToDevice, h->stream));
  auto tiled = [&](void* arr, int S, int E) -> int {
    const size_t n = (size_t)h->ntiles * S * E * TW;
    with_real(h, [&](auto r) {
      using real = decltype(r);
      hipLaunchKernelGGL(k_permute_tiled<real>, dim3(grid_for(n, 256)), dim3(256), 0, h->stream, (const real*)arr, (real*)h->perm_scratch, h->d_perm, h->ntiles, S, E);
      return 0;
    });
    HIPCHK(hipGetLastError());
    HIPCHK(hipMemcpyAsync(arr, h->perm_scratch, n * es, hipMemcpyDeviceToDevice, h->stream));
    return 0;
  };
  auto scalar = [&](auto* arr, size_t n) -> int {
    using T = std::remove_pointer_t<decltype(arr)>;
    hipLaunchKernelGGL(k_permute_scalar<T>, dim3((unsigned)((n + 255) / 256)), dim3(256), 0, h->stream, (const T*)arr, (T*)h->perm_scratch, h->d_perm, (int)n);
    HIPCHK(hipGetLastError());
    HIPCHK(hipMemcpyAsync(arr, h->perm_scratch, n * sizeof(T), hipMemcpyDeviceToDevice, h->stream));
    return 0;
  };
  BatchView& v = h->v;
  int rc = 0;
  rc |= tiled(v.x0, 1, h->nx);
  rc |= tiled(v.xs, h->T + 1, h->nx);
  rc |= tiled(v.us, h->T, h->nu);
  rc |= tiled(v.kff, h->T, h->nu);
  rc |= tiled(v.Kfb, h->T, h->nu * h->nx);
  rc |= scalar(v.cost, Bp);
  rc |= scalar(v.lambda, Bp);
  rc |= scalar(v.dlambda, Bp);
  rc |= scalar(v.dV, Bp);
  rc |= scalar(v.dV + Bp, Bp);
  rc |= scalar(v.gnorm, Bp);
  rc |= scalar(v.status, Bp);
  rc |= scalar(v.iters, Bp);
  rc |= scalar(v.flg_change, Bp);
  rc |= scalar(v.alpha_idx, Bp);
  rc |= scalar(v.diverge, Bp);
  rc |= scalar(v.backpass_done, Bp);
  if (rc) return rc;
  h->recs = ilqr_batch::REC_STALE;
  h->cands = Cands::none;
  return 0;
}

int ilqr_generate_trajectory(ilqr_batch* h) {
  if (!h) return fail(ILQR_ERR_INVALID, "null handle");
  if (!h->initialised) return fail(ILQR_ERR_STATE, "generate_trajectory needs x0/xs/us (asserts of ilqr_core.cpp:80-82)");
  const bool persistent = h->plan.solve != Solve::none;
  const bool compacting = persistent && h->ntiles > h->num_cus && !(h->sp.fixed_work) && !h->route.no_compaction;
  int done_iters = 0;
  const int chunk = persistent ? (compacting ? std::min(std::max(1, h->params.max_iter), 8) : std::max(1, h->params.max_iter)) : 10;
  std::vector<int> slot_orig;
  h->active_tiles = h->ntiles;
  auto chunks = [&]() -> int {
  while (done_iters < h->params.max_iter) {
    const int n = std::min(chunk, h->params.max_iter - done_iters);
    if (int rc = ilqr_iterate(h, n)) return rc;
    done_iters += n;
    int running = 0;
    HIPCHK(hipMemcpyAsync(&running, h->v.n_running, sizeof(int), hipMemcpyDeviceToHost, h->stream));
    HIPCHK(hipStreamSynchronize(h->stream));
    if (running == 0) break;
    if (compacting && done_iters < h->params.max_iter && 2 * ((running + TW - 1) / TW) <= h->active_tiles && h->active_tiles > 1) {
      std::vector<int> st(h->Bp);
      HIPCHK(hipMemcpyAsync(st.data(), h->v.status, (size_t)h->Bp * sizeof(int), hipMemcpyDeviceToHost, h->stream));
      HIPCHK(hipStreamSynchronize(h->stream));
      if (slot_orig.empty()) {
        slot_orig.resize(h->Bp);
        for (int j = 0; j < h->Bp; j++) slot_orig[j] = j;
      }
      std::vector<int> perm;
      perm.reserve(h->Bp);
      for (int j = 0; j < h->Bp; j++)
        if (st[j] == 0) perm.push_back(j);
      const int n_run = (int)perm.size();
      for (int j = 0; j < h->Bp; j++)
        if (st[j] != 0) perm.push_back(j);
      if (int rc = apply_permutation(h, perm)) {
        h->initialised = false;
        return rc;
      }
      std::vector<int> so(h->Bp);
      for (int j = 0; j < h->Bp; j++) so[j] = slot_orig[perm[j]];
      slot_orig.swap(so);
      h->active_tiles = std::max(1, (n_run + TW - 1) / TW);
    }
  }
  return 0;
  };
  const int rc_out = chunks();
  h->active_tiles = h->ntiles;
  if (!slot_orig.empty() && h->initialised) {
    std::vector<int> back(h->Bp);
    for (int j = 0; j < h->Bp; j++) back[slot_orig[j]] = j;
    if (int rc = apply_permutation(h, back)) {
      h->initialised = false;
      return rc_out ? rc_out : rc;
    }
  }
  return rc_out;
}

int ilqr_solve(ilqr_batch* h, const double* x0, const double* u0) {
  if (int rc = ilqr_init_traj(h, x0, u0, nullptr)) return rc;
  return ilqr_generate_trajectory(h);
}

static int warm_rollout_commit(ilqr_batch* h, bool repeat) {
  AlphaSet al;
  for (int i = 0; i < NALPHA; i++) al.a[i] = 0.0;
  if (h->plan.commit != Commit::tiled) {
    if (!repeat) HIPCHK(hipMemsetAsync(h->commit_idx, 0, (size_t)h->Bp * sizeof(int), h->stream));
    if (int rc = launch_rollout(h, true, true, al, 1, h->v.cost, 0)) return rc;
  } else {
    if (int rc = launch_rollout(h, true, true, al, 1, repeat ? h->v.cost_c : h->v.cost, 0)) return rc;
    if (!repeat) HIPCHK(hipMemsetAsync(h->commit_idx, 0, (size_t)h->Bp * sizeof(int), h->stream));
    if (int rc = launch_commit(h)) return rc;
    if (repeat) {
      hipLaunchKernelGGL(k_take_reset_cost, dim3((h->B + 255) / 256), dim3(256), 0, h->stream, h->v.cost_c, reset_sel(h), h->v.cost, h->B);
      HIPCHK(hipGetLastError());
    }
  }
  HIPCHK(hipMemsetAsync(h->commit_idx, 0xFF, (size_t)h->Bp * sizeof(int), h->stream));
  return 0;
}

int ilqr_warm_start(ilqr_batch* h, const double* x0) {
  if (!h || !x0) return fail(ILQR_ERR_INVALID, "null argument");
  if (host_model(h)) return no_device_model();
  if (!h->initialised) return fail(ILQR_ERR_STATE, "warm start needs a previous solve (assert us.size()>0, ilqr_core.cpp:66)");
  HIPCHK(hipSetDevice(h->device));
  if (int rc = upload(h, x0, {h->v.x0, 1, h->nx})) return rc;
  if (int rc = warm_rollout_commit(h, false)) return rc;
  if (int rc = launch_per_slot(h, k_warm_reset<double>, h->v)) return rc;
  return ilqr_generate_trajectory(h);
}

static int shift_nominal(ilqr_batch* h, int shift, int tail) {
  if (int rc = nominal_changes(h)) return rc;
  if (shift == 0) return 0;
  const NominalArrays n = nominal_arrays(h);
  const int tails[4] = {SHIFT_TAIL_HOLD, tail, SHIFT_TAIL_ZERO, tail};
  ShiftSet set;
  for (int i = 0; i < 4; i++) set.arr[i] = {n.arr[i].p, n.arr[i].S, n.arr[i].W, tails[i]};
  set.nseg = n.nseg;
  set.shift = shift;
  const dim3 grid((unsigned)std::min(set.nseg, 65535), 4), block(256);
  with_real(h, [&](auto r) {
    hipLaunchKernelGGL(k_shift_horizon<decltype(r)>, grid, block, 0, h->stream, set);
    return 0;
  });
  HIPCHK(hipGetLastError());
  return 0;
}
static int check_shift(ilqr_batch* h, int shift, int tail) {
  REQUIRE(shift >= 0 && shift < h->T, "shift %d: 0 <= shift < T = %d", shift, h->T);
  REQUIRE(tail == ILQR_TAIL_HOLD || tail == ILQR_TAIL_ZERO, "tail %d: ILQR_TAIL_HOLD or ILQR_TAIL_ZERO", tail);
  return 0;
}

int ilqr_shift_horizon(ilqr_batch* h, int shift, int tail) {
  if (!h) return fail(ILQR_ERR_INVALID, "null handle");
  if (int rc = check_shift(h, shift, tail)) return rc;
  if (!h->initialised) return fail(ILQR_ERR_STATE, "shift_horizon before ilqr_init_traj/ilqr_set_trajectory: there is no nominal to shift");
  HIPCHK(hipSetDevice(h->device));
  return shift_nominal(h, shift, tail == ILQR_TAIL_HOLD ? SHIFT_TAIL_HOLD : SHIFT_TAIL_ZERO);
}

int ilqr_copy_controls_to_device(ilqr_batch* h, int t0, int n_knots, void* u_device) {
  if (!h || !u_device) return fail(ILQR_ERR_INVALID, "null argument");
  REQUIRE(t0 >= 0 && n_knots >= 1 && t0 + n_knots <= h->T, "control window [%d, %d): inside [0, T = %d), at least one knot", t0, t0 + n_knots, h->T);
  if (!h->initialised) return fail(ILQR_ERR_STATE, "copy_controls_to_device before ilqr_init_traj/ilqr_set_trajectory");
  HIPCHK(hipSetDevice(h->device));
  return to_canonical(h, {h->v.us, h->T, h->nu, t0, n_knots}, (double*)u_device);
}

static int check_reset_args(const int* mask, const void* mask_device, int rules, const char* who) {
  REQUIRE(!(mask && mask_device), "%s: at most one of mask (host) and mask_device", who);
  REQUIRE((rules & ~(ILQR_RESET_NONFINITE | ILQR_RESET_LAMBDA_MAX)) == 0, "%s: rules %d: bits of ILQR_RESET_NONFINITE | ILQR_RESET_LAMBDA_MAX", who, rules);
  return 0;
}
static int stage_reset_mask(ilqr_batch* h, const int* mask, const void* mask_device, const int** out) {
  if (!h->reset_ints)
    if (int rc = dev_alloc(h, &h->reset_ints, 3 * (size_t)h->Bp)) return rc;
  *out = (const int*)mask_device;
  if (mask) {
    HIPCHK(hipMemcpyAsync(reset_mask_stage(h), mask, (size_t)h->B * sizeof(int), hipMemcpyHostToDevice, h->stream));
    *out = reset_mask_stage(h);
  }
  return 0;
}
static int select_and_reset(ilqr_batch* h, const int* d_mask, int rules, int repeat) {
// ... 690 lines not shown
  return 0;
}

int ilqr_clear_trajectory_params(ilqr_batch* h) {
  if (!h) return fail(ILQR_ERR_INVALID, "null handle");
  if (int rc = check_trajectory_params(h, "ilqr_clear_trajectory_params")) return rc;
  h->plan.traj_params = false;
  return 0;
}

static int prepare_param_gradient(ilqr_batch* h, int n_dirs, int flags, double eps_p, const void* dxs, const void* dus, const void* dlam, const void* gp,
                                  const void* lam, const char* who) {
  REQUIRE(n_dirs >= 1, "%s: n_dirs %d must be >= 1", who, n_dirs);
  REQUIRE(flags == 0, "%s: unknown flag bits 0x%x", who, (unsigned)flags);
  REQUIRE(eps_p >= 0.0 && eps_p <= 1.7976931348623157e308, "%s: eps_p %g must be finite and >= 0", who, eps_p);
  REQUIRE(dxs || dus || dlam, "%s: dxs, dus and dlam are all null: the answer would be zero", who);
  REQUIRE(gp || lam, "%s: gp and lam are both null", who);
  if (!h) return fail(ILQR_ERR_INVALID, "null handle");
  if (int rc = check_trajectory_params(h, who)) return rc;
  const long long widest = (long long)h->B * (h->T + 1) * n_dirs * std::max(std::max(h->nx, h->nu), kUserNTP);
  REQUIRE(widest <= (long long)INT_MAX, "%s: B * (T + 1) * n_dirs * max(nx, nu, NTP) = %lld elements do not fit an int", who, widest);
  if (!h->initialised) return fail(ILQR_ERR_STATE, "%s before ilqr_init_traj/ilqr_set_trajectory: no trajectory is stored", who);
  if (!h->plan.traj_params)
    return fail(ILQR_ERR_STATE, "%s: no per-trajectory parameters are set (ilqr_create's user_params have no mapping onto the NTP fields)", who);
  HIPCHK(hipSetDevice(h->device));
  if (int rc = flush_commit(h)) return rc;
  return materialise_records(h);
}
static int run_param_gradient(ilqr_batch* h, int n_dirs, double eps_p, const double* dxs, const double* dus, const double* dlam, double* gp, double* lam,
                              const char* who) {
  const size_t nchunk = ((size_t)h->T + 1 + kPgChunk - 1) / kPgChunk;
  const size_t n_lam = lam ? 0 : (size_t)h->B * (h->T + 1) * h->nx, n_part = gp ? (size_t)h->B * nchunk * n_dirs * kUserNTP : 0;
  if (int rc = ensure_pg_scratch(h, n_lam + n_part)) return rc;
  PgArgs a;
  a.nd = n_dirs, a.nchunk = (int)nchunk, a.eps_p = eps_p == 0.0 ? 1e-3 : eps_p;
  a.dxs = dxs, a.dus = dus, a.dlam = dlam, a.gp = gp;
  a.lam = lam ? lam : h->pg_scratch;
  a.part = h->pg_scratch + n_lam;
  const char* kernel = "";
  const int rc = launch_param_gradient(h, a, &kernel);
  return name_refused_kernel(rc, who, kernel);
}

int ilqr_param_gradient_on_device(ilqr_batch* h, int n_dirs, int flags, double eps_p, const void* dxs_device, const void* dus_device,
                                  const void* dlam_device, void* gp_device, void* lam_device) {
  const char* who = "ilqr_param_gradient_on_device";
  if (int rc = prepare_param_gradient(h, n_dirs, flags, eps_p, dxs_device, dus_device, dlam_device, gp_device, lam_device, who)) return rc;
  return run_param_gradient(h, n_dirs, eps_p, (const double*)dxs_device, (const double*)dus_device, (const double*)dlam_device, (double*)gp_device,
                            (double*)lam_device, who);
}

int ilqr_get_param_gradient(ilqr_batch* h, int n_dirs, int flags, double eps_p, const double* dxs, const double* dus, const double* dlam, double* gp,
                            double* lam) {
  const char* who = "ilqr_get_param_gradient";
  if (int rc = prepare_param_gradient(h, n_dirs, flags, eps_p, dxs, dus, dlam, gp, lam, who)) return rc;
  const size_t per_x = (size_t)h->B * n_dirs * h->nx, per_u = (size_t)h->B * n_dirs * h->nu;
  const size_t n_dx = dxs ? per_x * (h->T + 1) : 0, n_du = dus ? per_u * h->T : 0, n_dl = dlam ? per_x * (h->T + 1) : 0,
               n_gp = gp ? (size_t)h->B * n_dirs * kUserNTP : 0, n_lam = lam ? (size_t)h->B * (h->T + 1) * h->nx : 0;
  if (int rc = ensure_staging(h, n_dx + n_du + n_dl + n_gp + n_lam)) return rc;
  double* const d_dx = dxs ? h->staging : nullptr;
  double* const d_du = dus ? h->staging + n_dx : nullptr;
  double* const d_dl = dlam ? h->staging + n_dx + n_du : nullptr;
  double* const d_gp = gp ? h->staging + n_dx + n_du + n_dl : nullptr;
  double* const d_lam = lam ? h->staging + n_dx + n_du + n_dl + n_gp : nullptr;
  if (dxs) HIPCHK(hipMemcpyAsync(d_dx, dxs, n_dx * sizeof(double), hipMemcpyHostToDevice, h->stream));
  if (dus) HIPCHK(hipMemcpyAsync(d_du, dus, n_du * sizeof(double), hipMemcpyHostToDevice, h->stream));
  if (dlam) HIPCHK(hipMemcpyAsync(d_dl, dlam, n_dl * sizeof(double), hipMemcpyHostToDevice, h->stream));
  if (int rc = run_param_gradient(h, n_dirs, eps_p, d_dx, d_du, d_dl, d_gp, d_lam, who)) return rc;
  if (gp) HIPCHK(hipMemcpyAsync(gp, d_gp, n_gp * sizeof(double), hipMemcpyDeviceToHost, h->stream));
  if (lam) HIPCHK(hipMemcpyAsync(lam, d_lam, n_lam * sizeof(double), hipMemcpyDeviceToHost, h->stream));
  HIPCHK(hipStreamSynchronize(h->stream));
  return 0;
}

static int begin_stage(ilqr_batch* h, bool device_model) {
  if (!h) return fail(ILQR_ERR_INVALID, "null handle");
  if (device_model && host_model(h)) return no_device_model();
  HIPCHK(hipSetDevice(h->device));
  if (!h->initialised) return fail(ILQR_ERR_STATE, "stage call before ilqr_init_traj/ilqr_set_trajectory (the reference asserts, ilqr_core.cpp:80-82)");
  return 0;
}
int ilqr_compute_derivatives(ilqr_batch* h) {
  if (int rc = begin_stage(h, true)) return rc;
  return launch_derivatives(h, 1);
}

int ilqr_backward_pass(ilqr_batch* h, int* diverge_out) {
  if (int rc = begin_stage(h, false)) return rc;
  if (int rc = launch_backward(h, 0)) return rc;
  if (diverge_out) return scalars_to_host(h, h->v.diverge, diverge_out);
  return 0;
}

int ilqr_backward_step(ilqr_batch* h) {
  if (int rc = begin_stage(h, false)) return rc;
  return launch_backward(h, 1);
}

int ilqr_rollout_candidates(ilqr_batch* h, double* cost_out) {
  if (int rc = begin_stage(h, true)) return rc;
  if (int rc = do_rollout_candidates(h, 0)) return rc;
  if (cost_out) {
    std::vector<double> tmp((size_t)NALPHA * h->Bp);
    HIPCHK(hipMemcpyAsync(tmp.data(), h->v.cost_c, tmp.size() * sizeof(double), hipMemcpyDeviceToHost, h->stream));
    HIPCHK(hipStreamSynchronize(h->stream));
    for (int b = 0; b < h->B; b++)
      for (int a = 0; a < NALPHA; a++) cost_out[(size_t)b * NALPHA + a] = tmp[(size_t)a * h->Bp + b];
  }
  return 0;
}

int ilqr_line_search(ilqr_batch* h) {
  if (int rc = begin_stage(h, true)) return rc;
  if (int rc = flush_commit(h)) return rc;
  if (int rc = do_rollout_candidates(h, 1)) return rc;
  if (int rc = launch_accept(h)) return rc;
  return flush_commit(h);
}

int ilqr_accept_candidates(ilqr_batch* h, const double* cost_c, int* accepted) {
  if (!h || !cost_c || !accepted) return fail(ILQR_ERR_INVALID, "null argument");
  if (!h->v.cost_c) return fail(ILQR_ERR_UNSUPPORTED, "this handle has no candidate-cost buffer");
  if (int rc = begin_stage(h, false)) return rc;
  if (int rc = flush_commit(h)) return rc;
  std::vector<double> tmp((size_t)NALPHA * h->Bp, 0.0);
  for (int b = 0; b < h->B; b++)
    for (int a = 0; a < NALPHA; a++) tmp[(size_t)a * h->Bp + b] = cost_c[(size_t)b * NALPHA + a];
  HIPCHK(hipMemcpyAsync(h->v.cost_c, tmp.data(), tmp.size() * sizeof(double), hipMemcpyHostToDevice, h->stream));
  HIPCHK(hipMemsetAsync(h->v.n_running, 0, sizeof(int), h->stream));
  if (int rc = launch_accept(h)) return rc;
  std::vector<int> ci(h->Bp);
  HIPCHK(hipMemcpyAsync(ci.data(), h->commit_idx, (size_t)h->Bp * sizeof(int), hipMemcpyDeviceToHost, h->stream));
  HIPCHK(hipMemsetAsync(h->commit_idx, 0xFF, (size_t)h->Bp * sizeof(int), h->stream));
  HIPCHK(hipStreamSynchronize(h->stream));
  h->commit_pending = false;
  for (int b = 0; b < h->B; b++) accepted[b] = ci[b];
  return 0;
}

int ilqr_reset_state(ilqr_batch* h, int warm) {
  if (!h) return fail(ILQR_ERR_INVALID, "null handle");
  HIPCHK(hipSetDevice(h->device));
  if (int rc = flush_commit(h)) return rc;
  return warm ? launch_per_slot(h, k_warm_reset<double>, h->v) : fresh_trajectory(h);
}

int ilqr_set_trajectory(ilqr_batch* h, const double* x0, const double* xs, const double* us, const double* cost) {
  if (!h) return fail(ILQR_ERR_INVALID, "null handle");
  HIPCHK(hipSetDevice(h->device));
  if (x0) if (int rc = upload(h, x0, {h->v.x0, 1, h->nx})) return rc;
  if (xs) if (int rc = upload(h, xs, {h->v.xs, h->T + 1, h->nx})) return rc;
  if (us) if (int rc = upload(h, us, {h->v.us, h->T, h->nu})) return rc;
  if (cost) if (int rc = scalars_to_dev(h, cost, h->v.cost)) return rc;
  h->initialised = true;
  return 0;
}
int ilqr_set_gains(ilqr_batch* h, const double* k, const double* K) {
  if (!h) return fail(ILQR_ERR_INVALID, "null handle");
  HIPCHK(hipSetDevice(h->device));
  if (k) if (int rc = upload(h, k, {h->v.kff, h->T, h->nu})) return rc;
  if (K) if (int rc = upload(h, K, {h->v.Kfb, h->T, h->nu * h->nx})) return rc;
  return 0;
}
int ilqr_set_derivatives(ilqr_batch* h, const double* fx, const double* fu, const double* cx, const double* cu,
                         const double* cxx, const double* cxu, const double* cuu) {
  if (!h) return fail(ILQR_ERR_INVALID, "null handle");
  HIPCHK(hipSetDevice(h->device));
  int off[7], len[7];
  rec_offsets(h->nx, h->nu, off, len);
  const double* srcs[7] = {fx, fu, cx, cu, cxx, cxu, cuu};
  for (int i = 0; i < 7; i++)
    if (srcs[i]) if (int rc = upload_rec(h, srcs[i], off[i], len[i])) return rc;
  return 0;
}
int ilqr_set_lambda(ilqr_batch* h, const double* lambda, const double* dlambda) {
  if (!h) return fail(ILQR_ERR_INVALID, "null handle");
  HIPCHK(hipSetDevice(h->device));
  if (lambda) if (int rc = scalars_to_dev(h, lambda, h->v.lambda)) return rc;
  if (dlambda) if (int rc = scalars_to_dev(h, dlambda, h->v.dlambda)) return rc;
  return 0;
}

int ilqr_get_trajectory(ilqr_batch* h, double* xs, double* us) {
  if (!h) return fail(ILQR_ERR_INVALID, "null handle");
  HIPCHK(hipSetDevice(h->device));
  if (xs) if (int rc = download(h, {h->v.xs, h->T + 1, h->nx}, xs)) return rc;
  if (us) if (int rc = download(h, {h->v.us, h->T, h->nu}, us)) return rc;
  return 0;
}
int ilqr_get_gains(ilqr_batch* h, double* k, double* K) {
  if (!h) return fail(ILQR_ERR_INVALID, "null handle");
  HIPCHK(hipSetDevice(h->device));
  if (k) if (int rc = download(h, {h->v.kff, h->T, h->nu}, k)) return rc;
  if (K) if (int rc = download(h, {h->v.Kfb, h->T, h->nu * h->nx}, K)) return rc;
  return 0;
}
int ilqr_get_derivatives(ilqr_batch* h, double* fx, double* fu, double* cx, double* cu, double* cxx, double* cxu,
                         double* cuu) {
  if (!h) return fail(ILQR_ERR_INVALID, "null handle");
  HIPCHK(hipSetDevice(h->device));
  int off[7], len[7];
  rec_offsets(h->nx, h->nu, off, len);
  double* dsts[7] = {fx, fu, cx, cu, cxx, cxu, cuu};
  if (int rc = materialise_records(h)) return rc;
  for (int i = 0; i < 7; i++)
    if (dsts[i]) if (int rc = download(h, rec_block(h, off[i], len[i]), dsts[i])) return rc;
  return 0;
}
int ilqr_get_cost(ilqr_batch* h, double* cost) {
  if (!h || !cost) return fail(ILQR_ERR_INVALID, "null argument");
  HIPCHK(hipSetDevice(h->device));
  return scalars_to_host(h, h->v.cost, cost);
}
int ilqr_get_lambda(ilqr_batch* h, double* lambda, double* dlambda) {
  if (!h) return fail(ILQR_ERR_INVALID, "null handle");
  HIPCHK(hipSetDevice(h->device));
  if (lambda) if (int rc = scalars_to_host(h, h->v.lambda, lambda)) return rc;
  if (dlambda) if (int rc = scalars_to_host(h, h->v.dlambda, dlambda)) return rc;
  return 0;
}
int ilqr_get_dV(ilqr_batch* h, double* dV) {
  if (!h || !dV) return fail(ILQR_ERR_INVALID, "null argument");
  HIPCHK(hipSetDevice(h->device));
  std::vector<double> tmp(2 * (size_t)h->Bp);
  HIPCHK(hipMemcpyAsync(tmp.data(), h->v.dV, tmp.size() * sizeof(double), hipMemcpyDeviceToHost, h->stream));
  HIPCHK(hipStreamSynchronize(h->stream));
  for (int b = 0; b < h->B; b++) {
    dV[2 * b] = tmp[b];
    dV[2 * b + 1] = tmp[h->Bp + b];
  }
  return 0;
}
int ilqr_get_gnorm(ilqr_batch* h, double* g) {
  if (!h || !g) return fail(ILQR_ERR_INVALID, "null argument");
  HIPCHK(hipSetDevice(h->device));
  return scalars_to_host(h, h->v.gnorm, g);
}
int ilqr_get_status(ilqr_batch* h, int* status, int* iters, int* alpha_idx) {
  if (!h) return fail(ILQR_ERR_INVALID, "null handle");
  HIPCHK(hipSetDevice(h->device));
  if (status) if (int rc = scalars_to_host(h, h->v.status, status)) return rc;
  if (iters) if (int rc = scalars_to_host(h, h->v.iters, iters)) return rc;
  if (alpha_idx) if (int rc = scalars_to_host(h, h->v.alpha_idx, alpha_idx)) return rc;
  return 0;
}
int ilqr_get_candidate(ilqr_batch* h, int a, double* xs, double* us) {
  if (!h) return fail(ILQR_ERR_INVALID, "null handle");
  if (host_model(h)) return no_device_model();
  REQUIRE(a >= 0 && a < NALPHA, "alpha index %d out of range", a);
  if (h->cands == Cands::none)
    return fail(ILQR_ERR_STATE, "no candidates: none rolled out yet, or the solve re-packed running trajectories (compaction) and left the "
                                "candidate buffers behind -- call ilqr_rollout_candidates / ilqr_iterate first");
  HIPCHK(hipSetDevice(h->device));
  if (h->aos) {
    if (!(h->plan.commit == Commit::lq_copy && h->lq_cands_kept))
      return fail(ILQR_ERR_UNSUPPORTED, "this handle's line search keeps no candidate trajectories (only their costs: ilqr_rollout_candidates)");
    const size_t wx = (size_t)(h->T + 1) * h->nx * sizeof(double), wu = (size_t)h->T * h->nu * sizeof(double);
    if (xs) HIPCHK(hipMemcpy2DAsync(xs, wx, (const char*)h->v.cand_x + (size_t)a * wx, (size_t)NALPHA * wx, wx, h->B, hipMemcpyDeviceToHost, h->stream));
    if (us) HIPCHK(hipMemcpy2DAsync(us, wu, (const char*)h->v.cand_u + (size_t)a * wu, (size_t)NALPHA * wu, wu, h->B, hipMemcpyDeviceToHost, h->stream));
    HIPCHK(hipStreamSynchronize(h->stream));
    return 0;
  }
  const size_t nx_el = (size_t)h->B * (h->T + 1) * h->nx, nu_el = (size_t)h->B * h->T * h->nu;
  if (int rc = ensure_staging(h, nx_el + nu_el)) return rc;
  double* dxs = h->staging;
  double* dus = h->staging + nx_el;
  const dim3 grid(grid_for((size_t)h->B * (h->T + 1), 256)), block(256);
  if (int rc = with_model(h, [&](auto& v, auto& m, auto&) {
        using MM = std::decay_t<decltype(m)>;
        constexpr bool kHexModel = MM::NX == 4 && MM::NU == 1;
        return with_bool(h->cands == Cands::grouped, [&](auto grouped) {
          hipLaunchKernelGGL((k_unpack_cand<MM, kHexModel && decltype(grouped)::value>), grid, block, 0, h->stream, v, m, a, dxs, dus);
          return 0;
        });
      }))
    return rc;
  HIPCHK(hipGetLastError());
  if (xs) HIPCHK(hipMemcpyAsync(xs, dxs, nx_el * sizeof(double), hipMemcpyDeviceToHost, h->stream));
  if (us) HIPCHK(hipMemcpyAsync(us, dus, nu_el * sizeof(double), hipMemcpyDeviceToHost, h->stream));
  HIPCHK(hipStreamSynchronize(h->stream));
  return 0;
}
int ilqr_copy_cost_to_device(ilqr_batch* h, void* dst) {
  if (!h || !dst) return fail(ILQR_ERR_INVALID, "null argument");
  HIPCHK(hipSetDevice(h->device));
  HIPCHK(hipMemcpyAsync(dst, h->v.cost, (size_t)h->B * sizeof(double), hipMemcpyDeviceToDevice, h->stream));
  return 0;
}
int ilqr_copy_trajectory_to_device(ilqr_batch* h, void* xs_dev, void* us_dev) {
  if (!h) return fail(ILQR_ERR_INVALID, "null handle");
  HIPCHK(hipSetDevice(h->device));
  if (xs_dev) if (int rc = to_canonical(h, {h->v.xs, h->T + 1, h->nx}, (double*)xs_dev)) return rc;
  if (us_dev) if (int rc = to_canonical(h, {h->v.us, h->T, h->nu}, (double*)us_dev)) return rc;
  return 0;
}
int ilqr_copy_gains_to_device(ilqr_batch* h, void* k_dev, void* K_dev) {
  if (!h) return fail(ILQR_ERR_INVALID, "null handle");
  HIPCHK(hipSetDevice(h->device));
  if (k_dev) if (int rc = to_canonical(h, {h->v.kff, h->T, h->nu}, (double*)k_dev)) return rc;
  if (K_dev) if (int rc = to_canonical(h, {h->v.Kfb, h->T, h->nu * h->nx}, (double*)K_dev)) return rc;
  return 0;
}
int ilqr_get_results_async(ilqr_batch* h, double* xs, double* us, double* k, double* K, double* cost) {
  if (!h) return fail(ILQR_ERR_INVALID, "null handle");
  HIPCHK(hipSetDevice(h->device));
  struct Item { DevArray src; double* dst; };
// ... 37 lines not shown
```

### ilqr_amd/csrc/common.hpp

```cpp
#pragma once
#include <type_traits>
#include <hip/hip_runtime.h>
#include <stddef.h>
#include <stdint.h>

namespace ilqr {

constexpr int TW = 16;
constexpr int NALPHA = 11;
constexpr int MAXN = 32;
constexpr int MAXM = 16;
constexpr int kMaxControls = 32;

__device__ __constant__ const double kAlpha[NALPHA] = {1.0000, 0.5012, 0.2512, 0.1259, 0.0631, 0.0316,
                                                       0.0158, 0.0079, 0.0040, 0.0020, 0.0010};
static const double kAlphaHost[NALPHA] = {1.0000, 0.5012, 0.2512, 0.1259, 0.0631, 0.0316,
                                          0.0158, 0.0079, 0.0040, 0.0020, 0.0010};

constexpr double kEps = 1e-3;

constexpr int kQpMaxIter = 100;
constexpr double kMinGrad = 1e-8;
constexpr double kMinRelImprove = 1e-8;
constexpr double kStepDec = 0.6;
constexpr double kMinStep = 1e-22;
constexpr double kArmijo = 0.1;
constexpr double kClampTol = 1e-4;

constexpr int CT = 8;

__host__ __device__ inline size_t tidx(int tile, int s, int e, int l, int S, int E) {
  return (((size_t)tile * S + s) * E + e) * TW + l;
}

template <int NX, int NU>
struct Rec {
  static constexpr int FX = 0;
  static constexpr int FU = FX + NX * NX;
  static constexpr int CX = FU + NX * NU;
  static constexpr int CXX = CX + NX;
  static constexpr int CXU = CXX + NX * NX;
  static constexpr int CU = CXU + NX * NU;
  static constexpr int CUU = CU + NU;
  static constexpr int SIZE = CUU + NU * NU;
  static_assert(NX % 2 == 0, "pair layout assumes an even state dimension");
  static_assert(SIZE % 2 == 0, "record must be a whole number of pairs");
};
inline int rec_size(int nx, int nu) { return 2 * nx * nx + 2 * nx * nu + nx + nu + nu * nu; }
inline void rec_offsets(int nx, int nu, int off[7], int len[7]) {
  const int FX = 0, FU = FX + nx * nx, CX = FU + nx * nu, CXX = CX + nx, CXU = CXX + nx * nx, CU = CXU + nx * nu, CUU = CU + nu;
  const int o[7] = {FX, FU, CX, CU, CXX, CXU, CUU};
  const int n[7] = {nx * nx, nx * nu, nx, nu, nx * nx, nx * nu, nu * nu};
  for (int i = 0; i < 7; i++) {
    off[i] = o[i];
    len[i] = n[i];
  }
}
template <int N, int I = 0, class F>
__host__ __device__ __forceinline__ void static_for(F&& f) {
  if constexpr (I < N) {
    f(std::integral_constant<int, I>());
    static_for<N, I + 1>(f);
  }
}
__host__ __device__ inline size_t didx(int tile, int t, int e, int l, int T1, int REC) {
  return ((((size_t)tile * T1 + t) * (REC / 2) + (e >> 1)) * TW + l) * 2 + (e & 1);
}

struct SolverParams {
  int max_iter;
  double tol_fun, tol_grad, lambda_factor, lambda_max, lambda_min, z_min;
  int fixed_work;
  int fixes;
};

template <class real>
struct BatchViewT {
  int B, Bp, ntiles, T;
  double dt;
  real* x0;
  real* xs;
  real* us;
  real* kff;
  real* Kfb;
  real* D;
  real* cand_u;
  real* cand_x;
  int nch;
  double* cost_c;
  double* cost;
  double* lambda;
  double* dlambda;
  double* dV;
  double* gnorm;
  int* status;
  int* iters;
  int* flg_change;
  int* alpha_idx;
  int* diverge;
  int* backpass_done;
  int* n_running;
  int analytic;
};
using BatchView = BatchViewT<double>;

}
```

### ilqr_amd/csrc/handle.hpp

```cpp
#pragma once
static thread_local char g_err[512] = "";
static int fail(int code, const char* fmt, ...) {
  va_list ap;
  va_start(ap, fmt);
  vsnprintf(g_err, sizeof(g_err), fmt, ap);
  va_end(ap);
  return code;
}
#define HIPCHK(call)                                                                         \
  do {                                                                                       \
    hipError_t e_ = (call);                                                                  \
    if (e_ != hipSuccess)                                                                    \
      return fail(ILQR_ERR_HIP, "%s failed: %s (%s:%d)", #call, hipGetErrorString(e_), __FILE__, __LINE__); \
  } while (0)
#define REQUIRE(cond, ...)                              \
  do {                                                  \
    if (!(cond)) return fail(ILQR_ERR_INVALID, __VA_ARGS__); \
  } while (0)

struct StageTimer {
  std::vector<std::pair<hipEvent_t, hipEvent_t>> pending;
  double ms = 0;
  int launches = 0;
};

enum class Cands { none, planes, grouped };

struct ilqr_batch {
  int model, nx, nu, T, B, Bp, ntiles, device, flags;
  int dtype = ILQR_DTYPE_F64;
  double dt;
  ilqr_params params;
  AcrobotModel acrobot;
  DoubleIntegratorModel dint;
  AcrobotModelT<float> acrobot_f;
  DoubleIntegratorModelT<float> dint_f;
  LqModel lq;
  LqModelT<float> lq_f;
  LqModelW lq_w;
  bool lq_wide = false;
#ifdef ILQR_HAVE_USER_MODEL
  UserModelT<double> user;
  GenericModelOf<UserModelT<double>> user_g;
  UserModelT<float> user_f;
  GenericModelOf<UserModelT<float>> user_gf;
#endif
  double* traj_params = nullptr;
  int* reset_ints = nullptr;
  double* reset_us = nullptr;
  double* reset_us_stage = nullptr;
  bool reset_us_set = false;
  bool reset_flags_valid = false;
  int* clone_ints = nullptr;
  bool clone_flags_valid = false;
  double* lq_scratch = nullptr;
  size_t lq_scratch_elems = 0;
  double* est_scratch = nullptr;
  size_t est_scratch_elems = 0;
  int* risk_fail = nullptr;
  double* pg_scratch = nullptr;
  size_t pg_scratch_elems = 0;
  BatchView v;
  BatchViewT<float> vf;
  SolverParams sp;
  hipStream_t stream = nullptr;
  bool own_stream = false;
  int* commit_idx = nullptr;
  long long* phase_ticks = nullptr;
  double wall_clock_khz = 100000.0;
  double* staging = nullptr;
  double* x0_stage = nullptr;
  double* const_rec = nullptr;
  bool records_partial = false;
  bool lq_fused_stale = false;
  bool lq_caller_records = false;
  enum { REC_ZERO, REC_VALID, REC_STALE } recs = REC_ZERO;
  size_t staging_elems = 0;
  std::vector<void*> allocs;
  bool initialised = false;
  bool commit_pending = false;
  bool lq_cands_kept = false;
  Cands cands = Cands::none;
  bool aos = false;
  double* d_umin = nullptr;
  double* d_umax = nullptr;
  bool profile = false;
  int num_cus = 256;
  int active_tiles = 0;
  int* d_perm = nullptr;
  void* perm_scratch = nullptr;
  size_t perm_scratch_bytes = 0;
  RoutePlan plan;
  struct {
    bool full_records = false, no_compaction = false;
    int wide_occ = 0;
  } route;
  StageTimer timers[ILQR_NUM_STAGES];
  std::vector<hipEvent_t> event_pool;
  bool chain_timers = false;
  hipEvent_t chain_event = nullptr;
};

static int* reset_mask_stage(ilqr_batch* h) { return h->reset_ints; }
static int* reset_sel(ilqr_batch* h) { return h->reset_ints + h->Bp; }
static int* reset_flags(ilqr_batch* h) { return h->reset_ints + 2 * (size_t)h->Bp; }
static int* clone_map(ilqr_batch* h) { return h->clone_ints; }
static int* clone_sel(ilqr_batch* h) { return h->clone_ints + h->Bp; }
static int* clone_flags(ilqr_batch* h) { return h->clone_ints + 2 * (size_t)h->Bp; }
static int rec_of(const ilqr_batch* h) { return rec_size(h->nx, h->nu); }
static size_t elem_size(const ilqr_batch* h) { return h->dtype == ILQR_DTYPE_F32 ? sizeof(float) : sizeof(double); }
static void sync_float_view(ilqr_batch* h) {
  const BatchView& v = h->v;
  BatchViewT<float>& f = h->vf;
  f.B = v.B; f.Bp = v.Bp; f.ntiles = v.ntiles; f.T = v.T; f.dt = v.dt;
  f.x0 = (float*)v.x0; f.xs = (float*)v.xs; f.us = (float*)v.us; f.kff = (float*)v.kff; f.Kfb = (float*)v.Kfb;
  f.D = (float*)v.D; f.cand_u = (float*)v.cand_u; f.cand_x = (float*)v.cand_x; f.nch = v.nch;
  f.cost_c = v.cost_c; f.cost = v.cost; f.lambda = v.lambda; f.dlambda = v.dlambda; f.dV = v.dV; f.gnorm = v.gnorm;
  f.status = v.status; f.iters = v.iters; f.flg_change = v.flg_change; f.alpha_idx = v.alpha_idx; f.diverge = v.diverge;
  f.backpass_done = v.backpass_done; f.n_running = v.n_running; f.analytic = v.analytic;
}
template <class F>
static int with_real(ilqr_batch* h, F&& f) {
  if (h->dtype == ILQR_DTYPE_F32) return f(float());
  return f(double());
}
template <class R>
static const BatchViewT<R>& view_of(const ilqr_batch* h) {
  if constexpr (std::is_same<R, float>::value) return h->vf; else return h->v;
}
template <class F>
static int with_view(ilqr_batch* h, F&& f) {
  return with_real(h, [&](auto r) { return f(view_of<decltype(r)>(h)); });
}
template <class F>
static int with_bool(bool b, F&& f) {
  return b ? f(std::true_type()) : f(std::false_type());
}
template <int... Is, class F>
static int with_int(int i, F&& f) {
  int rc = 0;
  const bool found = ((i == Is && ((rc = f(std::integral_constant<int, Is>())), true)) || ...);
  return found ? rc : fail(ILQR_ERR_STATE, "no kernel is built for the value %d of a launch-time switch", i);
}
template <class F>
static int with_model(ilqr_batch* h, F&& f) {
  if (h->dtype == ILQR_DTYPE_F32) {
    switch (h->model) {
      case ILQR_MODEL_ACROBOT: return f(h->vf, h->acrobot_f, h->acrobot);
      case ILQR_MODEL_DOUBLE_INTEGRATOR: return f(h->vf, h->dint_f, h->dint);
#ifdef ILQR_HAVE_USER_MODEL
      case ILQR_MODEL_USER:
        if constexpr (kUserTiled) return f(h->vf, h->user_f, h->user);
        break;
#endif
      default: break;
    }
  } else {
    switch (h->model) {
      case ILQR_MODEL_ACROBOT: return f(h->v, h->acrobot, h->acrobot);
      case ILQR_MODEL_DOUBLE_INTEGRATOR: return f(h->v, h->dint, h->dint);
#ifdef ILQR_HAVE_USER_MODEL
      case ILQR_MODEL_USER:
        if constexpr (kUserTiled) return f(h->v, h->user, h->user);
        break;
#endif
      default: break;
    }
  }
  return fail(ILQR_ERR_UNSUPPORTED, "model %d has no device kernels of this kind", h->model);
}
static bool host_model(const ilqr_batch* h) { return h->model == ILQR_MODEL_HOST; }
static int no_device_model();
static size_t dev_elems(const ilqr_batch* h, size_t S, size_t E) {
  return layout_elems(h->aos, h->B, h->ntiles, S, E);
}

template <class T>
static int dev_alloc(ilqr_batch* h, T** p, size_t n) {
  void* q = nullptr;
  HIPCHK(hipMalloc(&q, std::max<size_t>(n, 1) * sizeof(T)));
  HIPCHK(hipMemsetAsync(q, 0, std::max<size_t>(n, 1) * sizeof(T), h->stream));
  h->allocs.push_back(q);
  *p = (T*)q;
  return 0;
}

static int dev_alloc_real(ilqr_batch* h, double** p, size_t n) {
  void* q = nullptr;
  const size_t bytes = std::max<size_t>(n, 1) * elem_size(h);
  HIPCHK(hipMalloc(&q, bytes));
  HIPCHK(hipMemsetAsync(q, 0, bytes, h->stream));
  h->allocs.push_back(q);
  *p = (double*)q;
  return 0;
}

template <class M, class Real>
static void bind_lq(M& m, const Real* pad, size_t gm, const ilqr_batch* h) {
  const size_t nA = (size_t)GN * GN, nB = GN * gm, nR = gm * gm;
  m.nx = h->nx; m.nu = h->nu; m.umin = h->d_umin; m.umax = h->d_umax;
  m.A = pad; m.Bm = pad + nA; m.Q = pad + nA + nB; m.R = pad + 2 * nA + nB; m.Qf = pad + 2 * nA + nB + nR;
}

static int grid_for(size_t n, int block) { return (int)std::min<size_t>((n + block - 1) / block, 65535u * 16u); }

static int no_device_model() {
  return fail(ILQR_ERR_UNSUPPORTED, "host-evaluated model: rollouts and finite differences stay on the host; only the backward pass (ilqr_set_derivatives + ilqr_backward_pass/_step) runs on the device");
}

static int timer_event(ilqr_batch* h, hipEvent_t* e) {
  if (!h->event_pool.empty()) {
    *e = h->event_pool.back();
    h->event_pool.pop_back();
    return 0;
  }
  HIPCHK(hipEventCreate(e));
  return 0;
}
static int timer_begin(ilqr_batch* h, int stage, std::pair<hipEvent_t, hipEvent_t>* ev) {
  if (!h->profile) return 0;
  (void)stage;
  if (h->chain_timers && h->chain_event) {
    ev->first = h->chain_event;
  } else {
    if (int rc = timer_event(h, &ev->first)) return rc;
    HIPCHK(hipEventRecord(ev->first, h->stream));
  }
  h->chain_event = nullptr;
  return timer_event(h, &ev->second);
}
static int timer_end(ilqr_batch* h, int stage, const std::pair<hipEvent_t, hipEvent_t>& ev) {
  if (!h->profile) return 0;
  HIPCHK(hipEventRecord(ev.second, h->stream));
  h->timers[stage].pending.push_back(ev);
  h->timers[stage].launches++;
  h->chain_event = h->chain_timers ? ev.second : nullptr;
  return 0;
}
static int timers_drain(ilqr_batch* h) {
  std::vector<hipEvent_t> used;
  for (int s = 0; s < ILQR_NUM_STAGES; s++) {
    StageTimer& t = h->timers[s];
    for (auto& ev : t.pending) {
      float ms = 0;
      HIPCHK(hipEventSynchronize(ev.second));
      HIPCHK(hipEventElapsedTime(&ms, ev.first, ev.second));
      t.ms += ms;
      used.push_back(ev.first);
      used.push_back(ev.second);
    }
    t.pending.clear();
  }
  std::sort(used.begin(), used.end());
  used.erase(std::unique(used.begin(), used.end()), used.end());
  h->event_pool.insert(h->event_pool.end(), used.begin(), used.end());
  h->chain_event = nullptr;
  return 0;
}

static int ensure_staging(ilqr_batch* h, size_t elems) {
  if (elems <= h->staging_elems) return 0;
  if (h->staging) {
    HIPCHK(hipStreamSynchronize(h->stream));
    HIPCHK(hipFree(h->staging));
    h->staging = nullptr;
    h->staging_elems = 0;
  }
  HIPCHK(hipMalloc((void**)&h->staging, elems * sizeof(double)));
  h->staging_elems = elems;
  return 0;
}
static int ensure_lq_scratch(ilqr_batch* h, size_t elems) {
// ... 156 lines not shown
```

### ilqr_amd/csrc/launch.hpp

```cpp
#pragma once
#include "handle.hpp"

template <class... P, class... A>
static int launch_per_slot(ilqr_batch* h, void (*kernel)(P...), const A&... a) {
  hipLaunchKernelGGL(kernel, dim3((h->Bp + 255) / 256), dim3(256), 0, h->stream, static_cast<P>(a)...);
  HIPCHK(hipGetLastError());
  return 0;
}

template <class V, class M>
static int launch_rollout_t(ilqr_batch* h, const V& v, const M& m, bool gains, bool cand, const AlphaSet& al, int n_alpha,
                            double* cost_out, int mode, bool with_accept) {
  if (gains != cand) return fail(ILQR_ERR_INVALID, "unsupported rollout variant");
  const int aw = (n_alpha + 3) / 4;
  const int depth = h->ntiles <= h->num_cus ? kDeepPrefetch<M> : 4;
  return with_bool(gains, [&](auto g) { return with_bool(with_accept, [&](auto acc) { return with_int<kDeepPrefetch<M>, 4>(depth, [&](auto pd) {
    constexpr bool G = decltype(g)::value, ACCEPT = G && decltype(acc)::value;
    hipLaunchKernelGGL((k_rollout<M, G, G, G ? decltype(pd)::value : 4, ACCEPT>), dim3(h->ntiles), dim3(64 * aw), 0, h->stream, v, m, al, n_alpha,
                       cost_out, mode, h->sp, ACCEPT ? h->commit_idx : nullptr);
    HIPCHK(hipGetLastError());
    return 0;
  }); }); });
}
template <class F>
static int with_generic_model(ilqr_batch* h, F&& f) {
  if (h->model == ILQR_MODEL_LQ) return h->lq_wide ? f(h->lq_w) : f(h->lq);
#ifdef ILQR_HAVE_USER_MODEL
  if constexpr (kUserGeneric)
    if (h->model == ILQR_MODEL_USER) return f(h->user_g);
#endif
  return fail(ILQR_ERR_UNSUPPORTED, "model %d has no generic device kernels", h->model);
}
template <class F>
static int with_rollout_model(ilqr_batch* h, F&& f) {
  if (h->dtype != ILQR_DTYPE_F32) return with_generic_model(h, f);
  if (h->model == ILQR_MODEL_LQ) return f(h->lq_f);
#ifdef ILQR_HAVE_USER_MODEL
  if constexpr (kUserGeneric)
    if (h->model == ILQR_MODEL_USER) return f(h->user_gf);
#endif
  return fail(ILQR_ERR_UNSUPPORTED, "model %d has no fp32 generic device kernels", h->model);
}
template <class M>
static PerTrajectory<M> per_trajectory(const ilqr_batch* h, const M& m) {
  PerTrajectory<M> pm;
  static_cast<M&>(pm) = m;
  pm.traj_params = h->traj_params;
  return pm;
}
template <class M, class F>
static int with_trajectory_params(const ilqr_batch* h, const M& m, F&& f) {
  if constexpr (has_trajectory_params<M>::value)
    if (h->plan.traj_params) return f(per_trajectory(h, m), std::true_type());
  return f(m, std::false_type());
}
template <int WHAT, class M>
static int launch_rollout_g(ilqr_batch* h, const M& m, const AlphaSet& al, double* cost_out, int mode, int write_cost, bool with_accept = false) {
  constexpr bool search = WHAT == RG_SEARCH, commit = WHAT == RG_COMMIT;
  const int md = search ? mode : 0, wc = search ? 0 : commit ? write_cost : 1;
  if constexpr (std::is_same<M, LqModel>::value)
  if (h->plan.rollout != Rollout::generic) {
    const bool keeps = h->plan.rollout == Rollout::lq_accept;
    if (search) h->lq_cands_kept = keeps;
    return with_bool(search && with_accept && keeps, [&](auto acc) {
      constexpr bool ACCEPT = search && decltype(acc)::value;
      hipLaunchKernelGGL((k_rollout_lq<WHAT, ACCEPT>), dim3(h->B), dim3(64), 0, h->stream, h->v, m, al, cost_out,
                         (ACCEPT || commit) ? h->commit_idx : nullptr, md, wc, h->sp);
      HIPCHK(hipGetLastError());
      return 0;
    });
  }
  const dim3 grid(search ? (h->B + kSearchTraj - 1) / kSearchTraj : (h->B + 63) / 64);
  return with_trajectory_params(h, m, [&](const auto& pm, auto pt) {
    hipLaunchKernelGGL((k_rollout_g<M, WHAT, decltype(pt)::value>), grid, dim3(64), 0, h->stream, view_of<typename M::real>(h), pm, al, cost_out,
                       commit ? h->commit_idx : nullptr, md, wc, h->sp.fixes);
    HIPCHK(hipGetLastError());
    return 0;
  });
}

static int launch_rollout(ilqr_batch* h, bool gains, bool cand, const AlphaSet& al, int n_alpha, double* cost_out, int mode,
                          bool with_accept = false) {
  std::pair<hipEvent_t, hipEvent_t> ev;
  if (int rc = timer_begin(h, ILQR_STAGE_ROLLOUT, &ev)) return rc;
  const int rc = (h->plan.rollout != Rollout::tiled)
      ? with_rollout_model(h, [&](auto& m) {
          if (!gains) return launch_rollout_g<RG_INIT>(h, m, al, cost_out, 0, 1);
          if (n_alpha == NALPHA) return launch_rollout_g<RG_SEARCH>(h, m, al, cost_out, mode, 0, with_accept);
          return launch_rollout_g<RG_COMMIT>(h, m, al, cost_out, 0, 1);
        })
      : with_model(h, [&](auto& v, auto& m, auto&) { return launch_rollout_t(h, v, m, gains, cand, al, n_alpha, cost_out, mode, with_accept); });
  if (rc) return rc;
  if (cand && h->cands == Cands::grouped) h->cands = Cands::planes;
  return timer_end(h, ILQR_STAGE_ROLLOUT, ev);
}

static int refuse_grouped_cands(ilqr_batch* h) {
  return h->cands != Cands::grouped ? 0 : fail(ILQR_ERR_STATE, "the candidate buffers hold k_solve_hex's grouped layout: nothing reads them as alpha planes");
}

static AlphaSet line_search_alphas();
static int launch_commit(ilqr_batch* h) {
  if (h->plan.commit == Commit::lq_copy && h->lq_cands_kept) {
    hipLaunchKernelGGL(k_commit_lq, dim3(h->B), dim3(256), 0, h->stream, h->v, h->nx, h->nu, h->commit_idx);
    HIPCHK(hipGetLastError());
    return 0;
  }
  if (h->plan.commit != Commit::tiled)
    return with_rollout_model(h, [&](auto& m) { return launch_rollout_g<RG_COMMIT>(h, m, line_search_alphas(), h->v.cost, 0, 0); });
  if (int rc = refuse_grouped_cands(h)) return rc;
  dim3 grid((h->T + 1 + 15) / 16, h->ntiles), block(256);
  if (int rc = with_model(h, [&](auto& v, auto& m, auto&) {
        hipLaunchKernelGGL((k_commit<std::decay_t<decltype(m)>>), grid, block, 0, h->stream, v, m, h->commit_idx);
        return 0;
      }))
    return rc;
  HIPCHK(hipGetLastError());
  return 0;
}

static int flush_commit(ilqr_batch* h) {
  if (!h->commit_pending) return 0;
  std::pair<hipEvent_t, hipEvent_t> ev;
  if (int rc = timer_begin(h, ILQR_STAGE_ACCEPT, &ev)) return rc;
  if (int rc = launch_commit(h)) return rc;
  h->commit_pending = false;
  HIPCHK(hipMemsetAsync(h->commit_idx, 0xFF, (size_t)h->Bp * sizeof(int), h->stream));
  return timer_end(h, ILQR_STAGE_ACCEPT, ev);
}

static int forget_pending(ilqr_batch* h) {
  h->records_partial = false;
  h->lq_fused_stale = false;
  h->lq_caller_records = false;
  h->cands = Cands::none;
  h->commit_pending = false;
  HIPCHK(hipMemsetAsync(h->commit_idx, 0xFF, (size_t)h->Bp * sizeof(int), h->stream));
  return 0;
}
static int fresh_trajectory(ilqr_batch* h) {
  const size_t T = h->T, T1 = h->T + 1;
  if (h->v.D) HIPCHK(hipMemsetAsync(h->v.D, 0, dev_elems(h, T1, rec_of(h)) * elem_size(h), h->stream));
  h->recs = ilqr_batch::REC_ZERO;
  HIPCHK(hipMemsetAsync(h->v.kff, 0, dev_elems(h, T, h->nu) * elem_size(h), h->stream));
  HIPCHK(hipMemsetAsync(h->v.Kfb, 0, dev_elems(h, T, h->nu * h->nx) * elem_size(h), h->stream));
  if (int rc = forget_pending(h)) return rc;
  return launch_per_slot(h, k_reset_state<double>, h->v, h->params.lambda_init, h->params.dlambda_init);
}
static int nominal_changes(ilqr_batch* h) {
  if (int rc = flush_commit(h)) return rc;
  h->cands = Cands::none;
  h->lq_cands_kept = false;
  if (!h->aos && h->recs == ilqr_batch::REC_VALID) h->recs = ilqr_batch::REC_STALE;
  return 0;
}
struct NominalArrays {
  struct { void* p; int S, W; } arr[4];
  int nseg, lanes;
};
static NominalArrays nominal_arrays(const ilqr_batch* h) {
  const int nx = h->nx, nu = h->nu, T = h->T, lanes = h->aos ? 1 : TW;
  return {{{h->v.xs, T + 1, nx * lanes}, {h->v.us, T, nu * lanes}, {h->v.kff, T, nu * lanes}, {h->v.Kfb, T, nu * nx * lanes}},
          h->aos ? h->B : h->ntiles, lanes};
}

template <class M>
static int launch_derivatives_g(ilqr_batch* h, const M& m, int force, int t_only) {
  const dim3 grid(t_only < 0 ? h->B * (h->T + 1) : h->B);
  return with_trajectory_params(h, m, [&](const auto& pm, auto pt) { return with_view(h, [&](auto& v) {
    using S = std::remove_pointer_t<decltype(v.D)>;
    if constexpr (std::is_same_v<S, float> && (M::NU > WM)) {
      return fail(ILQR_ERR_UNSUPPORTED, "k_derivatives_g: no fp32 handle has more than %d controls", WM);
    } else {
      hipLaunchKernelGGL((k_derivatives_g<M, S, decltype(pt)::value>), grid, dim3(64), 0, h->stream, v, pm, force, t_only);
      return 0;
    }
  }); });
}
static int launch_derivatives(ilqr_batch* h, int force) {
  const Derivatives route = h->plan.derivatives;
  if (route != Derivatives::tiled)
    if (int rc = flush_commit(h)) return rc;
  if (route == Derivatives::fused_lq) {
    h->lq_fused_stale = true;
    h->lq_caller_records = false;
    return 0;
  }
  if (route == Derivatives::tiled && h->commit_pending)
    if (int rc = refuse_grouped_cands(h)) return rc;
  if (int rc = ensure_records(h)) return rc;
  h->recs = ilqr_batch::REC_VALID;
  std::pair<hipEvent_t, hipEvent_t> ev;
  if (int rc = timer_begin(h, ILQR_STAGE_DERIVATIVES, &ev)) return rc;
  dim3 grid((h->T + 1 + 15) / 16, h->ntiles), block(256);
  const int* ci = h->commit_pending ? h->commit_idx : nullptr;
  if (route != Derivatives::tiled) {
    int rc = 0;
    if (route == Derivatives::analytic_lq) {
      const int what = (h->route.full_records || h->dtype == ILQR_DTYPE_F32) ? 0 : 1;
      const int chunk = (what == 1) ? 4 * kAnalyticChunk : kAnalyticChunk;
      const int nchunk = (h->T + 1 + chunk - 1) / chunk;
      rc = with_view(h, [&](auto& v) {
        hipLaunchKernelGGL((k_analytic_lq<std::remove_pointer_t<decltype(v.D)>>), dim3(h->B * nchunk), dim3(64), 0, h->stream, v, h->lq, force, what, h->const_rec, chunk);
        return 0;
      });
      h->records_partial = (what == 1);
    } else if (route == Derivatives::lq) {
      const int nchunk = (h->T + kLqKnotsPerWave - 1) / kLqKnotsPerWave;
      rc = with_view(h, [&](auto& v) {
        hipLaunchKernelGGL((k_derivatives_lq<std::remove_pointer_t<decltype(v.D)>>), dim3(h->B * nchunk), dim3(64), 0, h->stream, v, h->lq, force);
        return launch_derivatives_g(h, h->lq, force, h->T);
      });
    } else {
      rc = with_generic_model(h, [&](auto& m) { return launch_derivatives_g(h, m, force, -1); });
    }
    if (rc) return rc;
    HIPCHK(hipGetLastError());
    return timer_end(h, ILQR_STAGE_DERIVATIVES, ev);
  }
  if (int rc = with_model(h, [&](auto& v, auto& m, auto& fdm) {
        hipLaunchKernelGGL((k_derivatives<std::decay_t<decltype(m)>, std::decay_t<decltype(fdm)>>), grid, block, 0, h->stream, v, m, fdm, force, ci);
        return 0;
      }))
    return rc;
  HIPCHK(hipGetLastError());
  h->commit_pending = false;
  return timer_end(h, ILQR_STAGE_DERIVATIVES, ev);
}

static int launch_backward_w(ilqr_batch* h, const WaveVariant& w, bool w2, int mode, const double* crec) {
  const dim3 grid(h->B), block(64);
  if (w2)
    return with_int<1, 2>(w.nt, [&](auto nt) {
      hipLaunchKernelGGL(k_backward_w2<decltype(nt)::value>, grid, block, 0, h->stream, h->v, h->nx, h->nu, h->d_umin, h->d_umax, h->sp, mode, crec);
      return 0;
    });
  return with_int<1, 2>(w.nt, [&](auto nt) { return with_int<1, 2>(w.mt, [&](auto mt) { return with_bool(w.full, [&](auto full) {
    return with_bool(w.lqf, [&](auto lqf) { return with_bool(w.regv, [&](auto regv) { return with_bool(w.f32, [&](auto f32) {
      constexpr int NT = decltype(nt)::value, MT = decltype(mt)::value;
      constexpr bool FULL = decltype(full)::value, LQF = decltype(lqf)::value, REGV = decltype(regv)::value, F32 = decltype(f32)::value;
      if constexpr ((FULL && NT != 2) || (REGV && (FULL || LQF)) || (MT == 2 && (FULL || LQF || REGV || F32))) {
        return fail(ILQR_ERR_STATE, "k_backward_w3<%d, %d, %d, %d, %d, %s> is not built", NT, FULL, LQF, REGV, MT, F32 ? "float" : "double");
      } else {
        using S = std::conditional_t<F32, float, double>;
        hipLaunchKernelGGL((k_backward_w3<NT, FULL, LQF, REGV, MT, S>), grid, block, 0, h->stream, view_of<S>(h), h->nx, h->nu, h->d_umin, h->d_umax,
                           h->sp, mode, crec);
        return 0;
      }
    }); }); });
  }); }); });
}

static int launch_backward(ilqr_batch* h, int mode) {
  if (!h->aos)
    if (int rc = materialise_records(h)) return rc;
  std::pair<hipEvent_t, hipEvent_t> ev;
  if (int rc = timer_begin(h, ILQR_STAGE_BACKWARD, &ev)) return rc;
  const Backward route = h->plan.backward;
  if (route != Backward::quad && route != Backward::thread) {
    const bool fused = h->plan.derivatives == Derivatives::fused_lq && !h->lq_caller_records;
    if (!fused)
      if (int rc = ensure_records(h)) return rc;
    const double* crec = (fused || h->records_partial) ? h->const_rec : nullptr;
    if (int rc = launch_backward_w(h, backward_wave_variant(route, h->nx, h->nu, h->dtype, fused), route == Backward::w2, mode, crec)) return rc;
  } else if (int rc = with_model(h, [&](auto& v, auto& m, auto&) {
               using MM = std::decay_t<decltype(m)>;
               if (route == Backward::thread)
                 hipLaunchKernelGGL((k_backward_t<MM>), dim3(h->Bp / 64), dim3(64), 0, h->stream, v, m, h->sp, mode);
               else if constexpr (MM::NX == 4)
                 hipLaunchKernelGGL((k_backward_q<MM>), dim3(h->ntiles), dim3(64), 0, h->stream, v, m, h->sp, mode);
               return 0;
             }))
    return rc;
  HIPCHK(hipGetLastError());
  return timer_end(h, ILQR_STAGE_BACKWARD, ev);
}

constexpr int kRingKbTwoBlocks = 60;
static int launch_sweep_backward(ilqr_batch* h, int mode, int force) {
  std::pair<hipEvent_t, hipEvent_t> ev;
  if (int rc = timer_begin(h, ILQR_STAGE_BACKWARD, &ev)) return rc;
  const int* ci = h->commit_pending ? h->commit_idx : nullptr;
  if (int rc = with_model(h, [&](auto& v, auto& m, auto& fdm) {
        using MM = std::decay_t<decltype(m)>;
        using MF = std::decay_t<decltype(fdm)>;
        if constexpr (MM::NX == 4)
          return with_bool(h->plan.sweep == Sweep::one_producer, [&](auto one) {
            constexpr int P = decltype(one)::value ? 1 : kProducers, KB = decltype(one)::value ? kRingKbTwoBlocks : ILQR_RING_KB;
            hipLaunchKernelGGL((k_sweep_backward<MM, P, KB, MF>), dim3(h->ntiles), dim3(64 * (1 + P)), 0, h->stream, v, m, fdm, h->sp, mode, force, ci);
            return 0;
          });
        return 0;
      }))
    return rc;
  HIPCHK(hipGetLastError());
  h->commit_pending = false;
  h->recs = ilqr_batch::REC_STALE;
  return timer_end(h, ILQR_STAGE_BACKWARD, ev);
}

static int launch_accept(ilqr_batch* h) {
  std::pair<hipEvent_t, hipEvent_t> ev;
  if (int rc = timer_begin(h, ILQR_STAGE_ACCEPT, &ev)) return rc;
  if (int rc = launch_per_slot(h, k_accept<double>, h->v, h->sp, h->commit_idx)) return rc;
  h->commit_pending = true;
  return timer_end(h, ILQR_STAGE_ACCEPT, ev);
}

static int launch_solve_tiles(ilqr_batch* h, int n_iters) {
  std::pair<hipEvent_t, hipEvent_t> ev;
  HIPCHK(hipMemsetAsync(h->v.n_running, 0, sizeof(int), h->stream));
  if (int rc = timer_begin(h, ILQR_STAGE_SOLVE, &ev)) return rc;
  const AlphaSet al = line_search_alphas();
  const int pending = h->commit_pending ? 1 : 0;
  long long* ticks = h->profile ? h->phase_ticks : nullptr;
  const Solve solve = h->plan.solve;
  const int grid_tiles = (h->active_tiles > 0 && h->active_tiles < h->ntiles) ? h->active_tiles : h->ntiles;
  if (int rc = with_model(h, [&](auto& v, auto& m, auto& fdm) {
        using MM = std::decay_t<decltype(m)>;
        using MF = std::decay_t<decltype(fdm)>;
        if constexpr (MM::NX != 4) {
          return fail(ILQR_ERR_STATE, "persistent tiles are nx = 4 kernels");
        } else {
          auto solve_with = [&](auto kernel, int blocks, int threads) {
            hipLaunchKernelGGL(kernel, dim3(blocks), dim3(threads), 0, h->stream, v, m, fdm, al, h->sp, n_iters, h->sp.fixed_work, h->commit_idx, pending, ticks);
          };
          const int wide_blocks = (grid_tiles + 3) / 4;
          const bool wide_one = h->route.wide_occ == 1 || (h->route.wide_occ == 0 && wide_blocks <= h->num_cus);
          switch (solve) {
            case Solve::wide: if constexpr (MM::NU == 1) { if (wide_one) solve_with(k_solve_wide<MM, MF, 1>, wide_blocks, 512); else solve_with(k_solve_wide<MM, MF, 2>, wide_blocks, 256); } break;
            case Solve::wide2: if constexpr (MM::NU == 2) solve_with(k_solve_wide2<MM, MF>, wide_blocks, 256); break;
            case Solve::hex: if constexpr (MM::NU == 1) solve_with(k_solve_hex<MM, MF>, grid_tiles, 512); break;
            case Solve::tile1: solve_with(k_solve_tile<MM, MF, 1>, grid_tiles, 256); break;
            case Solve::tile2: solve_with(k_solve_tile<MM, MF, 2>, grid_tiles, 256); break;
            case Solve::none: break;
          }
        }
        return 0;
      }))
    return rc;
  HIPCHK(hipGetLastError());
  h->commit_pending = (solve != Solve::hex);
  if (h->cands != Cands::none)
    h->cands = (solve == Solve::hex && kHexCandT) ? Cands::grouped : Cands::planes;
  h->recs = ilqr_batch::REC_STALE;
  return timer_end(h, ILQR_STAGE_SOLVE, ev);
}

static int launch_value(ilqr_batch* h, int t0, int nk, double* Vx, double* Vxx, const char** name) {
  const WaveVariant w = value_wave_variant(h->nx, h->nu, h->dtype);
  *name = value_kernel_name(h->aos, w);
  if (!h->aos) {
    const dim3 grid(h->Bp / 64), block(64);
    if (int rc = with_model(h, [&](auto& v, auto& m, auto&) {
          hipLaunchKernelGGL((k_value_t<std::decay_t<decltype(m)>>), grid, block, 0, h->stream, v, t0, nk, Vx, Vxx);
          return 0;
        }))
      return rc;
  } else if (int rc = with_int<1, 2>(w.nt, [&](auto nt) { return with_int<1, 2>(w.mt, [&](auto mt) { return with_bool(w.f32, [&](auto f32) {
               constexpr int MT = decltype(mt)::value;
               using S = std::conditional_t<decltype(f32)::value, float, double>;
               if constexpr (MT == 2 && decltype(f32)::value) {
                 return fail(ILQR_ERR_UNSUPPORTED, "%s: no fp32 handle has more than %d controls", *name, WM);
               } else {
                 hipLaunchKernelGGL((k_value_w<decltype(nt)::value, MT, S>), dim3(h->B), dim3(64), 0, h->stream, view_of<S>(h), h->nx, h->nu, t0, nk, Vx, Vxx);
                 return 0;
               }
             }); }); }))
    return rc;
  HIPCHK(hipGetLastError());
  return 0;
}

static int launch_covariance(ilqr_batch* h, const CovArgs& q, const char** name) {
  const WaveVariant w = value_wave_variant(h->nx, h->nu, h->dtype);
  *name = covariance_kernel_name(h->aos, w);
  if (!h->aos) {
    const dim3 grid(h->Bp / 64), block(64);
    if (int rc = with_model(h, [&](auto& v, auto& m, auto&) {
          hipLaunchKernelGGL((k_covariance_t<std::decay_t<decltype(m)>>), grid, block, 0, h->stream, v, q);
          return 0;
        }))
      return rc;
  } else if (int rc = with_int<1, 2>(w.nt, [&](auto nt) { return with_int<1, 2>(w.mt, [&](auto mt) { return with_bool(w.f32, [&](auto f32) {
               constexpr int MT = decltype(mt)::value;
               using S = std::conditional_t<decltype(f32)::value, float, double>;
               if constexpr (MT == 2 && decltype(f32)::value) {
                 return fail(ILQR_ERR_UNSUPPORTED, "%s: no fp32 handle has more than %d controls", *name, WM);
               } else {
                 hipLaunchKernelGGL((k_covariance_w<decltype(nt)::value, MT, S>), dim3(h->B), dim3(64), 0, h->stream, view_of<S>(h), h->nx, h->nu, q);
                 return 0;
               }
             }); }); }))
    return rc;
  HIPCHK(hipGetLastError());
  return 0;
}

template <class Args, class Tiled, class Wave>
static int launch_sensitivity(ilqr_batch* h, const Args& q, const char* kernel_name, Tiled&& tiled, Wave&& wave) {
  const WaveVariant w = value_wave_variant(h->nx, h->nu, h->dtype);
  if (!h->aos) {
    const dim3 grid((unsigned)(h->Bp / 64) * (unsigned)q.nd), block(64);
    if (int rc = with_model(h, [&](auto& v, auto& m, auto&) {
          tiled(v, m, grid, block);
          return 0;
        }))
      return rc;
  } else if (int rc = with_int<1, 2>(w.nt, [&](auto nt) { return with_int<1, 2>(w.mt, [&](auto mt) { return with_bool(w.f32, [&](auto f32) {
               constexpr int MT = decltype(mt)::value;
               using S = std::conditional_t<decltype(f32)::value, float, double>;
               if constexpr (MT == 2 && decltype(f32)::value) {
                 return fail(ILQR_ERR_UNSUPPORTED, "%s: no fp32 handle has more than %d controls", kernel_name, WM);
               } else {
                 wave(nt, mt, S(), dim3((unsigned)h->B * (unsigned)((q.nd + 15) / 16)), dim3(64));
                 return 0;
               }
             }); }); }))
    return rc;
  HIPCHK(hipGetLastError());
  return 0;
}
static int launch_tangent(ilqr_batch* h, const TangentArgs& q, const char** name) {
  *name = tangent_kernel_name(h->aos, value_wave_variant(h->nx, h->nu, h->dtype));
  return launch_sensitivity(h, q, *name,
      [&](auto& v, auto& m, dim3 grid, dim3 block) { hipLaunchKernelGGL((k_tangent_t<std::decay_t<decltype(m)>>), grid, block, 0, h->stream, v, q); },
      [&](auto nt, auto mt, auto s, dim3 grid, dim3 block) {
        using S = decltype(s);
        hipLaunchKernelGGL((k_tangent_w<decltype(nt)::value, decltype(mt)::value, S>), grid, block, 0, h->stream, view_of<S>(h), h->nx, h->nu, q);
      });
}
static int launch_adjoint(ilqr_batch* h, const AdjointArgs& q, const char** name) {
  *name = adjoint_kernel_name(h->aos, value_wave_variant(h->nx, h->nu, h->dtype));
  return launch_sensitivity(h, q, *name,
      [&](auto& v, auto& m, dim3 grid, dim3 block) { hipLaunchKernelGGL((k_adjoint_t<std::decay_t<decltype(m)>>), grid, block, 0, h->stream, v, q); },
      [&](auto nt, auto mt, auto s, dim3 grid, dim3 block) {
        using S = decltype(s);
        hipLaunchKernelGGL((k_adjoint_w<decltype(nt)::value, decltype(mt)::value, S>), grid, block, 0, h->stream, view_of<S>(h), h->nx, h->nu, q);
      });
}

static int launch_lq_solve(ilqr_batch* h, const LqArgs& q, const char** name) {
  const WaveVariant w = value_wave_variant(h->nx, h->nu, h->dtype);
  *name = lq_solve_kernel_name(h->aos, w);
  if (!h->aos) {
    const dim3 block(64), per_traj((unsigned)(h->Bp / 64)), per_dir((unsigned)(h->Bp / 64) * (unsigned)q.nd);
    if (int rc = with_model(h, [&](auto& v, auto& m, auto&) {
          using Mdl = std::decay_t<decltype(m)>;
          hipLaunchKernelGGL((k_lq_gain_t<Mdl>), per_traj, block, 0, h->stream, v, q);
          hipLaunchKernelGGL((k_lq_dir_t<Mdl>), per_dir, block, 0, h->stream, v, q);
          return 0;
        }))
      return rc;
  } else if (int rc = with_int<1, 2>(w.nt, [&](auto nt) { return with_int<1, 2>(w.mt, [&](auto mt) { return with_bool(w.f32, [&](auto f32) {
               constexpr int NT = decltype(nt)::value, MT = decltype(mt)::value;
               using S = std::conditional_t<decltype(f32)::value, float, double>;
               if constexpr (MT == 2 && decltype(f32)::value) {
                 return fail(ILQR_ERR_UNSUPPORTED, "%s: no fp32 handle has more than %d controls", *name, WM);
               } else {
                 const dim3 block(64), per_traj((unsigned)h->B), per_tile((unsigned)h->B * (unsigned)((q.nd + 15) / 16));
                 hipLaunchKernelGGL((k_lq_gain_w<NT, MT, S>), per_traj, block, 0, h->stream, view_of<S>(h), h->nx, h->nu, q);
                 hipLaunchKernelGGL((k_lq_back_w<NT, MT, S>), per_tile, block, 0, h->stream, view_of<S>(h), h->nx, h->nu, q);
                 hipLaunchKernelGGL((k_lq_fwd_w<NT, MT, S>), per_tile, block, 0, h->stream, view_of<S>(h), h->nx, h->nu, q);
                 return 0;
               }
             }); }); }))
    return rc;
  HIPCHK(hipGetLastError());
  return 0;
}

static int launch_estimator(ilqr_batch* h, const EstArgs& q, const char** name) {
  const WaveVariant w = value_wave_variant(h->nx, h->nu, h->dtype);
  const int yt = q.ny > 16 ? 2 : 1;
  *name = estimator_kernel_name(h->aos, w.nt, yt);
  if (!h->aos) {
    const dim3 grid(h->Bp / 64), block(64);
    if (int rc = with_model(h, [&](auto& v, auto& m, auto&) {
          hipLaunchKernelGGL((k_estimator_t<std::decay_t<decltype(m)>>), grid, block, 0, h->stream, v, q);
          return 0;
        }))
      return rc;
    HIPCHK(hipGetLastError());
    return 0;
  }
// ... 113 lines not shown
```

### ilqr_amd/csrc/profile.hpp

```cpp
#pragma once
#include "launch.hpp"

extern "C" {
int ilqr_profile_enable(ilqr_batch* h, int enable) {
  if (!h) return fail(ILQR_ERR_INVALID, "null handle");
  h->profile = enable != 0;
  return 0;
}
int ilqr_profile_reset(ilqr_batch* h) {
  if (!h) return fail(ILQR_ERR_INVALID, "null handle");
  if (int rc = timers_drain(h)) return rc;
  for (auto& t : h->timers) {
    t.ms = 0;
    t.launches = 0;
  }
  HIPCHK(hipMemsetAsync(h->phase_ticks, 0, 5 * (size_t)h->ntiles * sizeof(long long), h->stream));
  return 0;
}
int ilqr_profile_read(ilqr_batch* h, double ms_out[ILQR_NUM_STAGES], int launches_out[ILQR_NUM_STAGES]) {
  if (!h) return fail(ILQR_ERR_INVALID, "null handle");
  if (int rc = timers_drain(h)) return rc;
  double ms[ILQR_NUM_STAGES];
  int ln[ILQR_NUM_STAGES];
  for (int s = 0; s < ILQR_NUM_STAGES; s++) {
    ms[s] = h->timers[s].ms;
    ln[s] = h->timers[s].launches;
  }
  if (h->timers[ILQR_STAGE_SOLVE].launches > 0) {
    std::vector<long long> tk(5 * (size_t)h->ntiles);
    HIPCHK(hipMemcpyAsync(tk.data(), h->phase_ticks, tk.size() * sizeof(long long), hipMemcpyDeviceToHost, h->stream));
    HIPCHK(hipStreamSynchronize(h->stream));
    double sweep = 0, roll = 0, its = 0;
    for (int t = 0; t < h->ntiles; t++) {
      sweep += (double)tk[5 * t];
      roll += (double)tk[5 * t + 1];
      its += (double)tk[5 * t + 2];
    }
    const double to_ms = 1.0 / h->wall_clock_khz / h->ntiles;
    ms[ILQR_STAGE_BACKWARD] += sweep * to_ms;
    ms[ILQR_STAGE_ROLLOUT] += roll * to_ms;
    ln[ILQR_STAGE_BACKWARD] += (int)(its / h->ntiles + 0.5);
    ln[ILQR_STAGE_ROLLOUT] += (int)(its / h->ntiles + 0.5);
  }
  for (int s = 0; s < ILQR_NUM_STAGES; s++) {
    if (ms_out) ms_out[s] = ms[s];
    if (launches_out) launches_out[s] = ln[s];
  }
  return 0;
}
int ilqr_profile_shader_clock(ilqr_batch* h, double* mhz_out) {
  if (!h || !mhz_out) return fail(ILQR_ERR_INVALID, "null argument");
  std::vector<long long> tk(5 * (size_t)h->ntiles);
  HIPCHK(hipMemcpyAsync(tk.data(), h->phase_ticks, tk.size() * sizeof(long long), hipMemcpyDeviceToHost, h->stream));
  HIPCHK(hipStreamSynchronize(h->stream));
  double cyc = 0, wall = 0;
  for (int t = 0; t < h->ntiles; t++) {
    cyc += (double)tk[5 * t + 3];
    wall += (double)tk[5 * t + 4];
  }
  *mhz_out = (wall > 0) ? cyc / wall * h->wall_clock_khz * 1e-3 : 0.0;
  return 0;
}
const char* ilqr_stage_kernel_name(ilqr_batch* h, int stage) {
  static const RoutePlan kNoHandle{};
  return stage_kernel_name(h ? h->plan : kNoHandle, stage);
}

}
```

### ilqr_amd/csrc/quad_lanes.hpp

```cpp
#pragma once
#include "common.hpp"

namespace ilqr {

constexpr int kQuad = 4;

constexpr int quad_rollout_lanes(int nalpha) { return kQuad * nalpha; }
constexpr int quad_lane_alpha(int lane) { return lane / kQuad; }
constexpr int quad_lane_q(int lane) { return lane % kQuad; }
constexpr int quad_traj(int s, int q) { return kQuad * s + q; }
constexpr int quad_fetch_row(int lane, int nrows) { return lane / kQuad < nrows ? lane / kQuad : nrows - 1; }

constexpr int rollout_share_slot(int row, int l) { return ((row >> 1) * TW + l) * 2 + (row & 1); }
constexpr int rollout_share_pair(int p, int l) { return (p * TW + l) * 2; }
constexpr int rollout_rows(int nx, int nu) { return 2 * nu + nu * nx + nx; }

enum { ROW_US = 0, ROW_KFF = 1, ROW_KFB = 2, ROW_XS = 3 };
struct RowSource {
  int array, elem, E, S;
};
constexpr RowSource rollout_row_source(int row, int nx, int nu, int T) {
  return row < nu                 ? RowSource{ROW_US, row, nu, T}
         : row < 2 * nu           ? RowSource{ROW_KFF, row - nu, nu, T}
         : row < 2 * nu + nu * nx ? RowSource{ROW_KFB, row - 2 * nu, nu * nx, T}
                                  : RowSource{ROW_XS, row - 2 * nu - nu * nx, nx, T + 1};
}
constexpr size_t rollout_row_elem(const RowSource& r, int tile, int tt, int l) {
  return ((((size_t)tile * r.S) * r.E + r.elem) * TW + l) + (size_t)tt * r.E * TW;
}

}
```

### ilqr_amd/csrc/rollout.hpp

```cpp
#pragma once
#include "layout.hpp"
#include "quad_lanes.hpp"

namespace ilqr {

template <class View, class CostOf>
__device__ __forceinline__ void accept_one(const View& v, const SolverParams& sp, int b, CostOf cost_of,
                                           int* __restrict__ commit_idx, bool count_running = true) {
  if (b >= v.Bp) return;
  int commit = -1;
  if (b < v.B && v.status[b] == 0) {
    double lambda = v.lambda[b], dlambda = v.dlambda[b];
    const double cost_s = v.cost[b];
    bool fwd = false;
    double new_cost = 0, dcost = 0;
    int acc = -1;
    if (v.backpass_done[b]) {
      const double dV0 = v.dV[b], dV1 = v.dV[v.Bp + b];
      for (int a = 0; a < NALPHA; a++) {
        const double alpha = kAlpha[a];
        new_cost = cost_of(a);
        dcost = cost_s - new_cost;
        double expected;
        {
#pragma clang fp contract(off)
          expected = -alpha * (dV0 + alpha * dV1);
        }
        double z;
        if (expected > 0)
          z = dcost / expected;
        else
          z = (double)((0.0 < dcost) - (dcost < 0.0));
        if (z > sp.z_min) {
          fwd = true;
          acc = a;
          break;
        }
      }
    }
    int status = 0;
    if (fwd) {
      dlambda = fmin(dlambda / sp.lambda_factor, 1 / sp.lambda_factor);
      lambda = lambda * dlambda * (lambda > sp.lambda_min ? 1.0 : 0.0);
      v.cost[b] = new_cost;
      v.flg_change[b] = 1;
      commit = acc;
      if (!sp.fixed_work && dcost < sp.tol_fun) status = 2;
    } else {
      dlambda = fmax(dlambda * sp.lambda_factor, sp.lambda_factor);
      lambda = fmax(lambda * dlambda, sp.lambda_min);
      v.flg_change[b] = 0;
      if (!sp.fixed_work && lambda > sp.lambda_max) status = 3;
    }
    v.lambda[b] = lambda;
    v.dlambda[b] = dlambda;
    v.alpha_idx[b] = acc;
    const int it = v.iters[b] + 1;
    v.iters[b] = it;
    if (status == 0 && !sp.fixed_work && it >= sp.max_iter) status = 4;
    v.status[b] = status;
    if (status == 0 && count_running) atomicAdd(v.n_running, 1);
  }
  commit_idx[b] = commit;
}
template <class real>
__global__ void k_accept(BatchViewT<real> v, SolverParams sp, int* __restrict__ commit_idx) {
  const int b = blockIdx.x * blockDim.x + threadIdx.x;
  accept_one(v, sp, b, [&](int a) { return v.cost_c[(size_t)a * v.Bp + b]; }, commit_idx);
}

struct AlphaSet {
  double a[NALPHA];
};

#ifndef ILQR_ROLLOUT_UNCLAMPED_FETCH
#define ILQR_ROLLOUT_UNCLAMPED_FETCH 1
#endif
constexpr int kRolloutFetchSlack = 8;
constexpr size_t rollout_fetch_slack_elems(int nx, int nu) { return (size_t)kRolloutFetchSlack * nu * nx * TW; }
template <class M>
constexpr int kDeepPrefetch = (M::NU * M::NX + M::NX + 2 * M::NU <= 10) ? 8 : 4;

constexpr int CG = 4;
static_assert(CT % CG == 0, "a chunk of the commit is a whole number of control groups");
__host__ __device__ inline int cand_groups(int T) { return (T + CT + CG - 1) / CG; }
__host__ __device__ inline size_t cand_g_u(int ta, int grp, int l, int T) { return (((size_t)ta * cand_groups(T) + grp) * TW + l) * CG; }
__host__ __device__ inline size_t cand_g_x(int ta, int c, int l, int nch, int NX) { return (((size_t)ta * nch + c) * TW + l) * NX; }
template <class M, bool GAINS, bool CAND, int PD, bool ACCEPT, bool SHARE = false, bool NOFIX = false, int NG = 1, bool CANDT = false, bool QUAD = false>
__device__ __forceinline__ void rollout_tile(const BatchViewT<typename M::real>& v, const M& model, const AlphaSet& alphas, int n_alpha,
                                             double* __restrict__ cost_out, int mode, const SolverParams& sp,
                                             int* __restrict__ commit_idx, int tile, double* lds_cost, bool count_running = true, int rwave = -1,
                                             typename M::real* share = nullptr) {
  using real = typename M::real;
  constexpr int NX = M::NX, NU = M::NU;
  static_assert(NG == 1 || (SHARE && GAINS && !ACCEPT), "several alpha groups per wavefront: the shared-row rollout of the wide tiles");
  static_assert(!QUAD || (SHARE && GAINS && NG == 1 && quad_rollout_lanes(NALPHA) <= 64 && kQuad * rollout_rows(NX, NU) <= quad_rollout_lanes(NALPHA)),
                "quad rollouts: every alpha of four trajectories in one wavefront, whose lanes also fetch the quad's rows");
  static_assert(!CANDT || (CAND && SHARE && GAINS && NU == 1 && NX == 4 && PD % CG == 0), "grouped candidates: the matrix-core kernel's rollouts (nx = 4, nu = 1)");
  const int wave = (rwave >= 0) ? rwave : (int)(threadIdx.x >> 6);
  const int lane = threadIdx.x & 63;
  const int l = QUAD ? quad_traj(wave & 3, quad_lane_q(lane)) : lane & (TW - 1);
  const bool idle = QUAD && lane >= quad_rollout_lanes(NALPHA);
  const int a_sub = lane >> 4;
  const int b = tile * TW + l;
  int a[NG];
  bool active[NG];
  bool any_active = false;
  const bool eligible = (b < v.B) && (mode != 1 || (v.status[b < v.B ? b : 0] == 0 && v.backpass_done[b < v.B ? b : 0]));
#pragma unroll
  for (int g = 0; g < NG; g++) {
    a[g] = QUAD ? quad_lane_alpha(lane) : (wave + g) * 4 + a_sub;
    active[g] = eligible && (a[g] < n_alpha) && (!QUAD || wave < 4);
    any_active = any_active || active[g];
  }
  const bool run = (SHARE && GAINS) ? (__ballot(any_active) != 0ull) : any_active;
  if (!ACCEPT && !run) return;
  if (run && !idle) {
  const int T = v.T;
  real alpha[NG];
#pragma unroll
  for (int g = 0; g < NG; g++) alpha[g] = (real)alphas.a[a[g] < NALPHA ? a[g] : NALPHA - 1];
  const real dt = (real)v.dt;

  real x[NG][NX];
#pragma unroll
  for (int i = 0; i < NX; i++) {
    const real x0i = v.x0[tidx(tile, 0, i, l, 1, NX)];
#pragma unroll
    for (int g = 0; g < NG; g++) x[g][i] = x0i;
  }
  double total[NG];
#pragma unroll
  for (int g = 0; g < NG; g++) total[g] = 0;

  struct StepIn {
    real u[NU], k[GAINS ? NU : 1], K[GAINS ? NU * NX : 1], xnom[GAINS ? NX : 1];
  };
  auto load_step = [&](int t, StepIn& d) __attribute__((always_inline)) {
    t = (t < T) ? t : T - 1;
#pragma unroll
    for (int j = 0; j < NU; j++) d.u[j] = v.us[tidx(tile, t, j, l, T, NU)];
    if (GAINS) {
#pragma unroll
      for (int j = 0; j < NU; j++) d.k[j] = v.kff[tidx(tile, t, j, l, T, NU)];
#pragma unroll
      for (int e = 0; e < NU * NX; e++) d.K[e] = v.Kfb[tidx(tile, t, e, l, T, NU * NX)];
#pragma unroll
      for (int i = 0; i < NX; i++) d.xnom[i] = v.xs[tidx(tile, t, i, l, T + 1, NX)];
    }
  };
  int ta_store[NG];
#pragma unroll
  for (int g = 0; g < NG; g++) ta_store[g] = ((SHARE && CAND && !active[g]) ? NALPHA : a[g]) * v.ntiles + tile;
  typedef real real4v __attribute__((ext_vector_type(4)));
  real pend[NG][CG - 1];
#pragma unroll
  for (int g = 0; g < NG; g++)
#pragma unroll
    for (int q = 0; q < CG - 1; q++) pend[g][q] = 0;
  auto store_group = [&](int g, int t, real last) __attribute__((always_inline)) {
    real4v w;
    w.x = pend[g][0];
    w.y = pend[g][1];
    w.z = pend[g][2];
    w.w = last;
    *reinterpret_cast<real4v*>(v.cand_u + cand_g_u(ta_store[g], t / CG, l, T)) = w;
  };
  auto emit_knot = [&](int g, int t, const real* xx, const real* uu, auto with_u, auto ph) __attribute__((always_inline)) {
    if (SHARE && !CAND && !active[g]) return;
    if constexpr (CANDT) {
      constexpr int p = decltype(ph)::value;
      if (with_u) {
        if constexpr (p == CG - 1)
          store_group(g, t, uu[0]);
        else
          pend[g][p] = uu[0];
      }
      if ((t & (CT - 1)) == 0) {
        real4v w;
        w.x = xx[0];
        w.y = xx[1];
        w.z = xx[2];
        w.w = xx[3];
        *reinterpret_cast<real4v*>(v.cand_x + cand_g_x(ta_store[g], t / CT, l, v.nch, NX)) = w;
      }
    } else if (CAND) {
      const int ta = ta_store[g];
      if (with_u) {
#pragma unroll
        for (int q = 0; q < NU; q++) v.cand_u[tidx(ta, t, q, l, T, NU)] = uu[q];
      }
      if ((t & (CT - 1)) == 0) {
#pragma unroll
        for (int i = 0; i < NX; i++) v.cand_x[tidx(ta, t / CT, i, l, v.nch, NX)] = xx[i];
      }
    } else {
#pragma unroll
      for (int i = 0; i < NX; i++) v.xs[tidx(tile, t, i, l, T + 1, NX)] = xx[i];
      if (with_u) {
#pragma unroll
        for (int q = 0; q < NU; q++) v.us[tidx(tile, t, q, l, T, NU)] = uu[q];
      }
    }
  };
  const WithTrigConsts<M> rmodel(model);
  auto do_step = [&](int t, const StepIn& d, auto ph) __attribute__((always_inline)) {
#pragma unroll
    for (int g = 0; g < NG; g++) {
      real u[NU];
#pragma unroll
      for (int j = 0; j < NU; j++) u[j] = d.u[j];
      if (GAINS) {
#pragma unroll
        for (int j = 0; j < NU; j++) {
          u[j] += d.k[j] * alpha[g];
          real acc = 0;
#pragma unroll
          for (int i = 0; i < NX; i++) acc += d.K[j + NU * i] * (x[g][i] - d.xnom[i]);
          u[j] += acc;
        }
      }
      if (!NOFIX && (sp.fixes & 1)) {
#pragma unroll
        for (int j = 0; j < NU; j++) u[j] = min_of(max_of(u[j], model.u_min[j]), model.u_max[j]);
      }
      emit_knot(g, t, x[g], u, std::true_type(), ph);
      total[g] += (double)model.cost(x[g], u);
      real x1[NX];
      integrate_dynamics(rmodel, x[g], u, dt, x1);
#pragma unroll
      for (int i = 0; i < NX; i++) x[g][i] = x1[i];
    }
  };
  if constexpr (SHARE && GAINS) {
    static_assert(PD % 2 == 0 || PD == 1, "static ring indices");
    static_assert((size_t)PD * NU * NX * TW <= rollout_fetch_slack_elems(NX, NU), "PD knots past the end");
    constexpr int NROWS = 2 * NU + NU * NX + NX;
    static_assert(NROWS == rollout_rows(NX, NU), "quad_lanes.hpp counts the same rows");
    constexpr int NLD = QUAD ? 1 : (NROWS + 3) / 4;
    struct Raw {
      real r[NLD];
    };
    const real* rbase[NLD];
    unsigned rstride[NLD];
#pragma unroll
    for (int j = 0; j < NLD; j++) {
      const int row = QUAD ? quad_fetch_row(lane, NROWS) : (a_sub + 4 * j < NROWS) ? a_sub + 4 * j : NROWS - 1;
      if (row < NU) {
        rbase[j] = v.us + tidx(tile, 0, row, l, T, NU);
        rstride[j] = NU * TW;
      } else if (row < 2 * NU) {
        rbase[j] = v.kff + tidx(tile, 0, row - NU, l, T, NU);
        rstride[j] = NU * TW;
      } else if (row < 2 * NU + NU * NX) {
// ... 166 lines not shown
```

### include/ilqr_amd.h

```cpp
#ifndef ILQR_AMD_H_
#define ILQR_AMD_H_

#include <stddef.h>

#ifdef __cplusplus
extern "C" {
#endif

#define ILQR_AMD_ABI_VERSION 6

typedef struct ilqr_batch ilqr_batch;

enum ilqr_status_code {
  ILQR_OK = 0,
  ILQR_ERR_INVALID = -1,
  ILQR_ERR_NO_DEVICE = -2,
  ILQR_ERR_HIP = -3,
  ILQR_ERR_STATE = -4,
  ILQR_ERR_UNSUPPORTED = -5
};

enum ilqr_model_id {
  ILQR_MODEL_ACROBOT = 0,
  ILQR_MODEL_DOUBLE_INTEGRATOR = 1,
  ILQR_MODEL_LQ = 2,
  ILQR_MODEL_HOST = 3,
  ILQR_MODEL_USER = 4
};

enum ilqr_dtype { ILQR_DTYPE_F64 = 0, ILQR_DTYPE_F32 = 1 };

enum ilqr_traj_status {
  ILQR_RUNNING = 0,
  ILQR_CONVERGED_GRAD = 1,
  ILQR_CONVERGED_COST = 2,
  ILQR_LAMBDA_MAX = 3,
  ILQR_MAX_ITER = 4
};

enum ilqr_flags {
  ILQR_FLAG_FIXED_WORK = 1,
  ILQR_FLAG_BACKWARD_THREAD_PER_TRAJ = 2,
  ILQR_FLAG_UNFUSED = 8,
  ILQR_FLAG_ANALYTIC_DERIVATIVES = 16,
  ILQR_FLAG_STAGED = 32,
  ILQR_FLAG_REFERENCE_FIXES = 64,
  ILQR_FLAG_REGULARIZE_VXX = 128
};

typedef struct ilqr_params {
  int max_iter;
  double tol_fun;
  double tol_grad;
  double lambda_init;
  double dlambda_init;
  double lambda_factor;
  double lambda_max;
  double lambda_min;
  double z_min;
} ilqr_params;

typedef struct ilqr_desc {
  int abi_version;
  int model;
  int nx, nu;
  int T;
  int B;
  double dt;
  int device;
  int flags;
  int dtype;
  const double* u_min;
  const double* u_max;
  const double* goal;
  const double *lq_A, *lq_B, *lq_Q, *lq_R, *lq_Qf;
  void* stream;
  const ilqr_params* params;
  const double* user_params;
  int n_user_params;
  int route;
  int assume_cus;
} ilqr_desc;

enum ilqr_route {
  ILQR_ROUTE_AUTO = 0,
  ILQR_ROUTE_TILE_PER_CU = 1,
  ILQR_ROUTE_TWO_TILES_PER_CU = 2,
  ILQR_ROUTE_WIDE_TILES = 3,
  ILQR_ROUTE_WIDE_ONE_PER_CU = 4,
  ILQR_ROUTE_WIDE_TWO_PER_CU = 8,
  ILQR_ROUTE_NO_COMPACTION = 16,
  ILQR_ROUTE_FULL_RECORDS = 32,
  ILQR_ROUTE_LQ_THREAD_ROLLOUT = 64,
  ILQR_ROUTE_QUAD_CHAIN = 256,
  ILQR_ROUTE_LQ_RECOMMIT = 512,
  ILQR_ROUTE_LQ_DENSE_FD = 2048,
  ILQR_ROUTE_WAVE_PER_TRAJECTORY = 4096,
  ILQR_ROUTE_BACKWARD_W2 = 1024,
  ILQR_ROUTE_TWO_CONTROL_TILES = 8192
};

const char* ilqr_last_error(void);
int ilqr_abi_version(void);
int ilqr_has_user_model(void);
void ilqr_default_params(ilqr_params* p);

int ilqr_create(const ilqr_desc* desc, ilqr_batch** out);
void ilqr_destroy(ilqr_batch* h);
int ilqr_set_stream(ilqr_batch* h, void* hip_stream);
int ilqr_synchronize(ilqr_batch* h);

int ilqr_init_traj(ilqr_batch* h, const double* x0, const double* u0, double* cost_out);
int ilqr_generate_trajectory(ilqr_batch* h);
int ilqr_solve(ilqr_batch* h, const double* x0, const double* u0);
int ilqr_warm_start(ilqr_batch* h, const double* x0);
int ilqr_iterate(ilqr_batch* h, int n_iters);

enum ilqr_tail { ILQR_TAIL_HOLD = 0, ILQR_TAIL_ZERO = 1 };
int ilqr_shift_horizon(ilqr_batch* h, int shift, int tail);
int ilqr_mpc_step(ilqr_batch* h, const double* x0, const void* x0_device, int shift, int tail, int n_iters);
int ilqr_copy_controls_to_device(ilqr_batch* h, int t0, int n_knots, void* u_device);

enum ilqr_reset_rule { ILQR_RESET_NONFINITE = 1, ILQR_RESET_LAMBDA_MAX = 2 };
enum ilqr_reset_why { ILQR_WAS_MASKED = 1, ILQR_WAS_NONFINITE = 2, ILQR_WAS_LAMBDA_MAX = 4 };
int ilqr_set_reset_controls(ilqr_batch* h, const double* u0, const void* u0_device);
int ilqr_reset_trajectories(ilqr_batch* h, const int* mask, const void* mask_device, int rules);
int ilqr_mpc_step_reset(ilqr_batch* h, const double* x0, const void* x0_device, int shift, int tail, int n_iters, const int* mask,
                        const void* mask_device, int rules);
int ilqr_get_reset_flags(ilqr_batch* h, int* flags);
int ilqr_copy_reset_flags_to_device(ilqr_batch* h, void* flags_device);

enum ilqr_clone_why { ILQR_WAS_CLONED = 1, ILQR_CLONE_REFUSED = 2 };
int ilqr_select_best(ilqr_batch* h, int group, int* src, void* src_device);
int ilqr_clone_trajectories(ilqr_batch* h, const int* src, const void* src_device, const void* du_device);
int ilqr_clone_best(ilqr_batch* h, int group, const void* du_device);
int ilqr_get_clone_flags(ilqr_batch* h, int* flags);
int ilqr_copy_clone_flags_to_device(ilqr_batch* h, void* flags_device);

int ilqr_get_value(ilqr_batch* h, int t0, int n_knots, double* Vx, double* Vxx);
int ilqr_copy_value_to_device(ilqr_batch* h, int t0, int n_knots, void* Vx_device, void* Vxx_device);

int ilqr_get_covariance(ilqr_batch* h, int t0, int n_knots, const double* Sigma0, const double* W, double* Sigma, double* Su,
                        double* expected_cost);
int ilqr_copy_covariance_to_device(ilqr_batch* h, int t0, int n_knots, const void* Sigma0_device, const void* W_device, void* Sigma_device,
                                   void* Su_device, void* expected_cost_device);

int ilqr_get_tangent(ilqr_batch* h, int t0, int n_knots, int n_dirs, const double* dx0, const double* dv, double* dxs, double* dus);
int ilqr_copy_tangent_to_device(ilqr_batch* h, int t0, int n_knots, int n_dirs, const void* dx0_device, const void* dv_device, void* dxs_device,
                                void* dus_device);
int ilqr_get_adjoint(ilqr_batch* h, int t0, int n_knots, int n_dirs, const double* gx, const double* gu, double* g_x0, double* g_v);
int ilqr_copy_adjoint_to_device(ilqr_batch* h, int t0, int n_knots, int n_dirs, const void* gx_device, const void* gu_device, void* g_x0_device,
                                void* g_v_device);

enum ilqr_lq_flags { ILQR_LQ_HOLD_CLAMPED = 1 };
int ilqr_solve_lq(ilqr_batch* h, int n_dirs, int flags, double mu, const double* dx0, const double* gx, const double* gu, double* dxs, double* dus,
                  double* dlam, int* info);
int ilqr_solve_lq_on_device(ilqr_batch* h, int n_dirs, int flags, double mu, const void* dx0_device, const void* gx_device, const void* gu_device,
                            void* dxs_device, void* dus_device, void* dlam_device, void* info_device);

int ilqr_get_estimator(ilqr_batch* h, int t0, int n_knots, int ny, const double* H, const double* P0, const double* W, const double* V,
                       double* Pp, double* Pf, double* L, double* Sigma, double* Su, double* expected_cost, int* info);
int ilqr_copy_estimator_to_device(ilqr_batch* h, int t0, int n_knots, int ny, const void* H_device, const void* P0_device, const void* W_device,
                                  const void* V_device, void* Pp_device, void* Pf_device, void* L_device, void* Sigma_device, void* Su_device,
                                  void* expected_cost_device, void* info_device);

int ilqr_get_risk_sensitive(ilqr_batch* h, int nw, double theta, int flags, double mu, const double* C, double* K, double* k, double* Vx,
                            double* Vxx, double* risk_cost, int* info);
int ilqr_copy_risk_sensitive_to_device(ilqr_batch* h, int nw, double theta, int flags, double mu, const void* C_device, void* K_device,
                                       void* k_device, void* Vx_device, void* Vxx_device, void* risk_cost_device, void* info_device);

enum ilqr_eval_flags { ILQR_EVAL_CLAMP = 1 };
int ilqr_evaluate_policy(ilqr_batch* h, int t0, int n_knots, int n_samples, int flags, const double* x, double* cost, double* x_end,
                         double* u_first);
int ilqr_evaluate_policy_on_device(ilqr_batch* h, int t0, int n_knots, int n_samples, int flags, const void* x_device, void* cost_device,
                                   void* x_end_device, void* u_first_device);

int ilqr_trajectory_params_count(void);
int ilqr_set_trajectory_params(ilqr_batch* h, const double* p, const void* p_device, int n);
int ilqr_get_trajectory_params(ilqr_batch* h, double* p, int n);
int ilqr_clear_trajectory_params(ilqr_batch* h);

enum ilqr_param_gradient_flags { ILQR_PARAM_GRADIENT_NO_FLAGS = 0 };
int ilqr_get_param_gradient(ilqr_batch* h, int n_dirs, int flags, double eps_p, const double* dxs, const double* dus, const double* dlam,
                            double* gp, double* lam);
int ilqr_param_gradient_on_device(ilqr_batch* h, int n_dirs, int flags, double eps_p, const void* dxs_device, const void* dus_device,
                                  const void* dlam_device, void* gp_device, void* lam_device);

int ilqr_compute_derivatives(ilqr_batch* h);
int ilqr_backward_pass(ilqr_batch* h, int* diverge_out);
int ilqr_backward_step(ilqr_batch* h);
int ilqr_rollout_candidates(ilqr_batch* h, double* cost_out);
int ilqr_line_search(ilqr_batch* h);
int ilqr_accept_candidates(ilqr_batch* h, const double* cost_c, int* accepted);
int ilqr_reset_state(ilqr_batch* h, int warm);

int ilqr_set_trajectory(ilqr_batch* h, const double* x0, const double* xs, const double* us, const double* cost);
int ilqr_set_gains(ilqr_batch* h, const double* k, const double* K);
int ilqr_set_derivatives(ilqr_batch* h, const double* fx, const double* fu, const double* cx,
                         const double* cu, const double* cxx, const double* cxu, const double* cuu);
int ilqr_set_lambda(ilqr_batch* h, const double* lambda, const double* dlambda);

int ilqr_get_trajectory(ilqr_batch* h, double* xs, double* us);
int ilqr_get_gains(ilqr_batch* h, double* k, double* K);
int ilqr_get_derivatives(ilqr_batch* h, double* fx, double* fu, double* cx, double* cu,
                         double* cxx, double* cxu, double* cuu);
int ilqr_get_cost(ilqr_batch* h, double* cost);
int ilqr_get_lambda(ilqr_batch* h, double* lambda, double* dlambda);
int ilqr_get_dV(ilqr_batch* h, double* dV);
int ilqr_get_gnorm(ilqr_batch* h, double* gnorm);
int ilqr_get_status(ilqr_batch* h, int* status, int* iters, int* alpha_idx);
int ilqr_get_candidate(ilqr_batch* h, int alpha_idx, double* xs, double* us);
int ilqr_count_running(ilqr_batch* h, int* n_running);
int ilqr_copy_cost_to_device(ilqr_batch* h, void* dst_device);
int ilqr_copy_trajectory_to_device(ilqr_batch* h, void* xs_device, void* us_device);
int ilqr_copy_gains_to_device(ilqr_batch* h, void* k_device, void* K_device);
int ilqr_get_results_async(ilqr_batch* h, double* xs, double* us, double* k, double* K, double* cost);
int ilqr_host_register(void* ptr, size_t bytes);
int ilqr_host_unregister(void* ptr);

typedef struct ilqr_group ilqr_group;
int ilqr_group_create(ilqr_batch* const* shards, int n_shards, int flags, ilqr_group** out);
void ilqr_group_destroy(ilqr_group* g);
int ilqr_group_gather_costs(ilqr_group* g, double* cost_out);
int ilqr_group_uses_rccl(ilqr_group* g, int* n_ranks);

enum ilqr_stage { ILQR_STAGE_DERIVATIVES = 0, ILQR_STAGE_BACKWARD = 1, ILQR_STAGE_ROLLOUT = 2,
                  ILQR_STAGE_ACCEPT = 3, ILQR_STAGE_SOLVE = 4, ILQR_NUM_STAGES = 5 };
int ilqr_profile_enable(ilqr_batch* h, int enable);
int ilqr_profile_reset(ilqr_batch* h);
int ilqr_profile_read(ilqr_batch* h, double ms_out[ILQR_NUM_STAGES], int launches_out[ILQR_NUM_STAGES]);
int ilqr_profile_shader_clock(ilqr_batch* h, double* mhz_out);
const char* ilqr_stage_kernel_name(ilqr_batch* h, int stage);

#ifdef __cplusplus
}
#endif
#endif
```

Measured before the change: 4.638 billion trajectory-timesteps/s.

## Add load-balanced trajectory-to-chain mapping for hex backward sweep

Adds per-trajectory box-QP search load counters in LDS, updated inside the hex backward pass, and an optional lane map that assigns trajectories to the four backward chains greedily by the previous iteration's load. A scrambled map is offered as a control. The rollout honours the same map. The aim is to even out the slowest-chain time in the backward sweep. The balanced and scrambled maps are only opt-in route flags. The default identity path still pays for the LDS atomic counting, the extra map indirection and the load store-back each iteration.

```diff
diff --git a/ilqr_amd/batch.py b/ilqr_amd/batch.py
--- a/ilqr_amd/batch.py
+++ b/ilqr_amd/batch.py
@@ -573,6 +573,17 @@
         self._check(self.lib.ilqr_profile_read(self.h, ms, n))
         return {capi.STAGE_NAMES[i]: (ms[i], n[i]) for i in range(capi.NUM_STAGES)}
 
+    def hex_load(self):
+        load = np.zeros(self.B, dtype=np.int32)
+        self._check(self.lib.ilqr_get_hex_load(self.h, load.ctypes.data_as(C.POINTER(C.c_int))))
+        return load
+
+    def chain_clocks(self):
+        nt = (self.B + 63) // 64 * 4
+        chain, slowest, phase, its = np.zeros((nt, 4)), np.zeros(nt), np.zeros((nt, 2)), np.zeros(nt, dtype=np.int32)
+        self._check(self.lib.ilqr_profile_chain_clocks(self.h, _p(chain), _p(slowest), _p(phase), _pi(its)))
+        return chain, slowest, phase, its
+
     def shader_clock_mhz(self):
         mhz = C.c_double(0)
         self._check(self.lib.ilqr_profile_shader_clock(self.h, C.byref(mhz)))
diff --git a/ilqr_amd/capi.py b/ilqr_amd/capi.py
--- a/ilqr_amd/capi.py
+++ b/ilqr_amd/capi.py
@@ -17,6 +17,7 @@
 ROUTE_WIDE_ONE_PER_CU, ROUTE_WIDE_TWO_PER_CU, ROUTE_NO_COMPACTION, ROUTE_FULL_RECORDS, ROUTE_LQ_THREAD_ROLLOUT, ROUTE_QUAD_CHAIN, ROUTE_LQ_RECOMMIT, ROUTE_BACKWARD_W2, ROUTE_LQ_DENSE_FD = 4, 8, 16, 32, 64, 256, 512, 1024, 2048
 ROUTE_WAVE_PER_TRAJECTORY = 4096
 ROUTE_TWO_CONTROL_TILES = 8192
+ROUTE_HEX_BALANCED_MAP, ROUTE_HEX_SCRAMBLED_MAP = 16384, 32768
 NUM_STAGES = 5
 STAGE_NAMES = ("derivatives", "backward", "rollout", "accept", "solve")
 
@@ -125,6 +126,8 @@
     "ilqr_profile_reset": (C.c_int, [_H]),
     "ilqr_profile_read": (C.c_int, [_H, _dp, _ip]),
     "ilqr_profile_shader_clock": (C.c_int, [_H, _dp]),
+    "ilqr_profile_chain_clocks": (C.c_int, [_H, _dp, _dp, _dp, _ip]),
+    "ilqr_get_hex_load": (C.c_int, [_H, _ip]),
     "ilqr_stage_kernel_name": (C.c_char_p, [_H, C.c_int]),
 }
 
diff --git a/ilqr_amd/csrc/backward_hex.hpp b/ilqr_amd/csrc/backward_hex.hpp
--- a/ilqr_amd/csrc/backward_hex.hpp
+++ b/ilqr_amd/csrc/backward_hex.hpp
@@ -1,4 +1,5 @@
 #pragma once
+#include "hex_balance.hpp"
 #include "solve_tile.hpp"
 
 namespace ilqr {
@@ -132,11 +133,24 @@
   }
 };
 
+constexpr int kHexLoadMore = 25, kHexLoadPass = 100, kHexLoadGoesOn = 45, kHexLoadTrip = 115;
+typedef __attribute__((address_space(3))) int hex_lds_int;
+template <int WEIGHT>
+__device__ __forceinline__ void hex_count(hex_lds_int* load_sub, int t4, bool who) {
+  if (load_sub != nullptr && who) {
+    int w, t4_here;
+    asm volatile("v_mov_b32 %0, %1" : "=v"(w) : "n"(WEIGHT));
+    asm volatile("v_mov_b32 %0, %1" : "=v"(t4_here) : "v"(t4));
+    __hip_atomic_fetch_add(load_sub + (t4_here >> 2), w, __ATOMIC_RELAXED, __HIP_MEMORY_SCOPE_WORKGROUP);
+  }
+}
+
 __device__ __forceinline__ int hex_first(unsigned long long bal, int t4) {
   return __builtin_ctzll(((bal >> t4) & 0x000F000F000F000Full) | 0x8000000000000000ull);
 }
 template <class Under>
-__device__ __forceinline__ void qp1_search_hex(QP1StateT<double>& q, int j, int t4, double step_j0, const double* __restrict__ lds_steps, Under under_read) {
+__device__ __forceinline__ void qp1_search_hex(QP1StateT<double>& q, int j, int t4, double step_j0, const double* __restrict__ lds_steps, Under under_read,
+                                               hex_lds_int* load_sub = nullptr ) {
   const double t_x1 = clamp_of(q.x + step_j0 * q.search, q.lo, q.hi);
   const double t_v1 = qp1_value(q, t_x1);
   const bool t_pass = !qp1_armijo_fails(q, t_v1, step_j0);
@@ -154,6 +168,7 @@
   q.v1 = qp1_value(q, q.x1);
   bool more = p_and(!success, !q.early);
   if (__builtin_expect(__ballot(more) == 0ull, 1)) return;
+  hex_count<kHexLoadMore>(load_sub, t4, p_and(more, j == 0));
   {
     const bool stuck = p_and(j >= 1, t_x1 == q.x);
     const int qs = hex_first(__ballot(p_and(stuck, more)), t4);
@@ -164,6 +179,7 @@
     if (__ballot(more) == 0ull) return;
   }
   for (int base = 16;; base += 16) {
+    hex_count<kHexLoadPass>(load_sub, t4, p_and(more, j == 0));
     const int kn = base + j;
     const double my_step = lds_steps[kn < 104 ? kn : 103];
     const double my_x1 = qp1_trial(q, my_step);
@@ -199,7 +215,8 @@
 template <class M, class Gate, class RS>
 __device__ __forceinline__ void backward_hex(const BatchViewT<typename M::real>& v, const M& model, const SolverParams& sp, int mode, int tile, int sub,
                                              int lane, const double* __restrict__ lds_steps, Gate& gate, const typename M::real* __restrict__ ring,
-                                             const typename M::real* __restrict__ term ) {
+                                             const typename M::real* __restrict__ term ,
+                                             const int* lane_map , int* chain_load ) {
   using real = typename M::real;
   using creal = double;
   static_assert(M::NX == 4 && M::NU == 1, "hex chain: nx = 4, nu = 1");
@@ -207,8 +224,9 @@
   typedef real real2_t __attribute__((ext_vector_type(2)));
   const int r_ = lane >> 4, t_ = (lane >> 2) & 3, c_ = lane & 3, j16 = 4 * r_ + c_;
   const int t4 = 4 * t_;
-  const int l = sub * HT + t_;
+  const int l = lane_map[sub * HT + t_];
   const int b = tile * TW + l;
+  hex_lds_int* const load_sub = (hex_lds_int*)(size_t)__builtin_amdgcn_readfirstlane((unsigned)(size_t)(hex_lds_int*)(chain_load + sub * HT));
   if (b >= v.B) return;
   if (mode == 1 && v.status[b] != 0) return;
   const int T = v.T;
@@ -333,13 +351,18 @@
           products_1();
           __builtin_amdgcn_sched_barrier(0);
         }
-      });
+      }, load_sub);
       if constexpr (kHexMfmaSpread) products_2();
       bool goes_on;
       bool ok = qp1_finish_ok(q1, x, free0, minv, goes_on);
-      if (goes_on)
+      if (goes_on) {
+        hex_count<kHexLoadGoesOn>(load_sub, t4, j16 == 0);
         ok = qp1_continue(
-                 q1, [&](QP1StateT<creal>& qs) __attribute__((always_inline)) { qp1_search_hex(qs, j16, t4, step_j0, lds_steps, [] {}); }, x, free0) >= 1;
+                 q1, [&](QP1StateT<creal>& qs) __attribute__((always_inline)) {
+                   hex_count<kHexLoadTrip>(load_sub, t4, j16 == 0);
+                   qp1_search_hex(qs, j16, t4, step_j0, lds_steps, [] {}, load_sub);
+                 }, x, free0) >= 1;
+      }
       if (!ok) diverge = i;
       const creal Qxx_rc = (creal)raw.cxx_rc + Tm, Qxx_cr = (creal)raw.cxx_cr + Tt;
       const creal Qx_r = (creal)raw.cx_r + aQx;
@@ -475,7 +498,8 @@
 
 template <class M, class MFD, class P>
 __device__ __forceinline__ void sweep_backward_hex(const BatchViewT<typename M::real>& v, const M& model, const MFD& fdm, const SolverParams& sp, int mode,
-                                                   int force, int tile, P* pairs, const double* __restrict__ lds_steps, int role) {
+                                                   int force, int tile, P* pairs, const double* __restrict__ lds_steps, int role,
+                                                   const int* lane_map, int* chain_load, long long* __restrict__ chain_ticks, long long* chain_last ) {
   using RS = typename P::RS;
   const int lane = threadIdx.x & 63;
   if (threadIdx.x < 4) {
@@ -489,13 +513,19 @@
   if (role < 4) {
     __builtin_amdgcn_s_setprio(3);
     HexGate<P> gate(sh, T);
-    backward_hex<M, decltype(gate), RS>(v, model, sp, mode, tile, role, lane, lds_steps, gate, sh.ring, sh.term);
+    const long long c0 = chain_ticks ? wall_clock64() : 0;
+    backward_hex<M, decltype(gate), RS>(v, model, sp, mode, tile, role, lane, lds_steps, gate, sh.ring, sh.term, lane_map, chain_load);
+    const long long c1 = chain_ticks ? wall_clock64() : 0;
     gate.finish();
+    if (chain_ticks && lane == 0) {
+      chain_ticks[5 * tile + role] += c1 - c0;
+      chain_last[role] = c1 - c0;
+    }
     __builtin_amdgcn_s_setprio(0);
   } else {
     const int sub = role - 4;
     const int lp = lane & (HT - 1), ks = lane >> 2;
-    const int l = sub * HT + lp;
+    const int l = lane_map[sub * HT + lp];
     const int nrounds = (T + 1 + kHexKnotsPerRound - 1) / kHexKnotsPerRound, N = nrounds * kHexKnotsPerRound;
     for (int pass = 0;; pass++) {
       unsigned long long lanes = ~0ull;
@@ -638,11 +668,29 @@
   }
 }
 
+__device__ __forceinline__ int hex_deal_lanes(int load, int p) {
+  const int key = hex_balance_key(load, p);
+  int rank = 0;
+#pragma unroll
+  for (int j = 0; j < kHexTile; j++) rank += __builtin_amdgcn_readlane(key, j) > key;
+  HexDeal d;
+  int mine = p;
+#pragma unroll
+  for (int r = 0; r < kHexTile; r++) {
+    const int kr = __builtin_amdgcn_readlane(key, __builtin_ctzll(__ballot(rank == r)));
+    if (hex_deal_next(d, hex_key_load(kr)) == p) mine = hex_key_index(kr);
+  }
+  return mine;
+}
+
+enum { kHexMapIdentity = 0, kHexMapBalanced = 1, kHexMapScrambled = 2 };
+
 template <class M, class MFD>
 __global__ __launch_bounds__(512) __attribute__((amdgpu_waves_per_eu(2, 2))) void k_solve_hex(BatchViewT<typename M::real> v, M model, MFD fdm, AlphaSet alphas,
                                                                                                  SolverParams sp, int n_iters, int force,
                                                                                                  int* __restrict__ commit_idx, int commit_pending,
-                                                                                                 long long* __restrict__ phase_ticks) {
+                                                                                                 long long* __restrict__ phase_ticks,
+                                                                                                 long long* __restrict__ chain_ticks, int map_mode) {
   using real = typename M::real;
   using P = HexPair<real, M::NX, M::NU, state_free_running_cost<M>::value>;
   __shared__ P pairs[4];
@@ -651,7 +699,14 @@
   __shared__ int tile_running;
   __shared__ int simd_count[4];
   __shared__ int lds_commit[TW];
+  __shared__ int lane_map[TW], chain_load[TW], qp_load[TW];
+  __shared__ long long chain_last[4];
   if (threadIdx.x < 4) simd_count[threadIdx.x] = 0;
+  if (threadIdx.x < TW) {
+    lane_map[threadIdx.x] = threadIdx.x;
+    chain_load[threadIdx.x] = 0;
+    qp_load[threadIdx.x] = v.qp_load[blockIdx.x * TW + threadIdx.x];
+  }
   load_step_table(steps);
   const int wave = (int)(threadIdx.x >> 6);
   int role = wave;
@@ -680,10 +735,21 @@
   int it = 0;
   for (; it < n_iters; it++) {
     if (timing) t0 = wall_clock64();
-    sweep_backward_hex<M, MFD, P>(v, model, fdm, sp, 1, force, tile, pairs, steps, role);
+    if (map_mode != kHexMapIdentity && threadIdx.x < TW)
+      lane_map[threadIdx.x] = (map_mode == kHexMapBalanced) ? hex_deal_lanes(qp_load[threadIdx.x], (int)threadIdx.x) : hex_scrambled_map(tile, it, (int)threadIdx.x);
+    if (timing) chain_last[0] = chain_last[1] = chain_last[2] = chain_last[3] = 0;
+    sweep_backward_hex<M, MFD, P>(v, model, fdm, sp, 1, force, tile, pairs, steps, role, lane_map, chain_load, chain_ticks, chain_last);
     phase_barrier();
+    if (threadIdx.x < TW) {
+      qp_load[lane_map[threadIdx.x]] = chain_load[threadIdx.x];
+      chain_load[threadIdx.x] = 0;
+    }
     if (timing) {
       const long long t1 = wall_clock64();
+      if (chain_ticks) {
+        const long long a = chain_last[0] > chain_last[1] ? chain_last[0] : chain_last[1], b = chain_last[2] > chain_last[3] ? chain_last[2] : chain_last[3];
+        chain_ticks[5 * tile + 4] += a > b ? a : b;
+      }
 #ifdef ILQR_HEX_SECTIONS
       t_sweep_last = t1 - t0;
 #endif
@@ -691,7 +757,7 @@
       t0 = t1;
     }
     rollout_tile<M, true, true, kDeepPrefetch<M>, true, true, true, 1, kHexCandT, kHexQuadRollout>(v, model, alphas, NALPHA, v.cost_c, 1, sp, commit_idx, tile, lds_cost, it == n_iters - 1, rwave,
-                                               pairs[role & 3].ring);
+                                               pairs[role & 3].ring, lane_map);
 #ifdef ILQR_HEX_SECTIONS
 #define ILQR_HEX_MARK(n)                                   \
     if (ILQR_HEX_SECTIONS == n && timing) {                \
@@ -713,7 +779,10 @@
     if (timing) t_roll += wall_clock64() - t0;
     if (!sp.fixed_work) {
       const int b = tile * TW + (int)threadIdx.x;
-      if (threadIdx.x < TW && b < v.B && v.status[b] == 0) tile_running = 1;
+      if (threadIdx.x < TW) {
+        if (b < v.B && v.status[b] == 0) tile_running = 1;
+        else qp_load[threadIdx.x] = 0;
+      }
       __syncthreads();
       if (!tile_running) {
         it++;
@@ -721,6 +790,7 @@
       }
     }
   }
+  if (threadIdx.x < TW) v.qp_load[tile * TW + threadIdx.x] = qp_load[threadIdx.x];
   if (timing) {
     phase_ticks[5 * tile + 0] += t_sweep;
     phase_ticks[5 * tile + 1] += t_roll;
diff --git a/ilqr_amd/csrc/capi.hip b/ilqr_amd/csrc/capi.hip
--- a/ilqr_amd/csrc/capi.hip
+++ b/ilqr_amd/csrc/capi.hip
@@ -157,6 +157,7 @@
   h->route.full_records = (d->route & ILQR_ROUTE_FULL_RECORDS) != 0;
   h->route.no_compaction = (d->route & ILQR_ROUTE_NO_COMPACTION) != 0;
   h->route.wide_occ = (d->route & ILQR_ROUTE_WIDE_ONE_PER_CU) ? 1 : (d->route & ILQR_ROUTE_WIDE_TWO_PER_CU) ? 2 : 0;
+  h->route.hex_map = (d->route & ILQR_ROUTE_HEX_SCRAMBLED_MAP) ? kHexMapScrambled : (d->route & ILQR_ROUTE_HEX_BALANCED_MAP) ? kHexMapBalanced : kHexMapIdentity;
   h->aos = generic_layout(d->model, d->route, kUserTiled, kUserSmall);
   h->model = d->model; h->dtype = d->dtype; h->flags = d->flags;
   h->nx = d->nx; h->nu = d->nu; h->T = d->T; h->B = d->B; h->dt = d->dt;
@@ -287,7 +288,11 @@
   rc |= dev_alloc(h, &v.n_running, 1);
   rc |= dev_alloc(h, &h->x0_stage, (size_t)h->B * nx);
   rc |= dev_alloc(h, &h->phase_ticks, 5 * (size_t)h->ntiles);
+  rc |= dev_alloc(h, &h->chain_ticks, 5 * (size_t)h->ntiles);
+  rc |= dev_alloc(h, &v.qp_load, Bp);
   if (rc) return ILQR_ERR_HIP;
+  HIPCHK(hipMemsetAsync(v.qp_load, 0, Bp * sizeof(int), h->stream));
+  HIPCHK(hipMemsetAsync(h->chain_ticks, 0, 5 * (size_t)h->ntiles * sizeof(long long), h->stream));
   HIPCHK(hipMemsetAsync(h->commit_idx, 0xFF, Bp * sizeof(int), h->stream));
   sync_float_view(h);
   return 0;
@@ -452,6 +457,12 @@
   }
   if (!h->aos && n_iters > 0) h->recs = ilqr_batch::REC_STALE;
   return flush_commit(h);
+}
+
+int ilqr_get_hex_load(ilqr_batch* h, int* load_out) {
+  if (!h || !load_out) return fail(ILQR_ERR_INVALID, "null argument");
+  HIPCHK(hipSetDevice(h->device));
+  return scalars_to_host(h, h->v.qp_load, load_out);
 }
 
 int ilqr_count_running(ilqr_batch* h, int* n) {
@@ -515,6 +526,7 @@
   rc |= scalar(v.diverge, Bp);
   rc |= scalar(v.backpass_done, Bp);
   if (rc) return rc;
+  HIPCHK(hipMemsetAsync(v.qp_load, 0, Bp * sizeof(int), h->stream));
   h->recs = ilqr_batch::REC_STALE;
   h->cands = Cands::none;
   return 0;
@@ -1511,6 +1523,7 @@
   if (xs) if (int rc = upload(h, xs, {h->v.xs, h->T + 1, h->nx})) return rc;
   if (us) if (int rc = upload(h, us, {h->v.us, h->T, h->nu})) return rc;
   if (cost) if (int rc = scalars_to_dev(h, cost, h->v.cost)) return rc;
+  HIPCHK(hipMemsetAsync(h->v.qp_load, 0, (size_t)h->Bp * sizeof(int), h->stream));
   h->initialised = true;
   return 0;
 }
diff --git a/ilqr_amd/csrc/common.hpp b/ilqr_amd/csrc/common.hpp
--- a/ilqr_amd/csrc/common.hpp
+++ b/ilqr_amd/csrc/common.hpp
@@ -101,6 +101,7 @@
   int* backpass_done;
   int* n_running;
   int analytic;
+  int* qp_load;
 };
 using BatchView = BatchViewT<double>;
 
diff --git a/ilqr_amd/csrc/handle.hpp b/ilqr_amd/csrc/handle.hpp
--- a/ilqr_amd/csrc/handle.hpp
+++ b/ilqr_amd/csrc/handle.hpp
@@ -67,6 +67,7 @@
   bool own_stream = false;
   int* commit_idx = nullptr;
   long long* phase_ticks = nullptr;
+  long long* chain_ticks = nullptr;
   double wall_clock_khz = 100000.0;
   double* staging = nullptr;
   double* x0_stage = nullptr;
@@ -94,6 +95,7 @@
   struct {
     bool full_records = false, no_compaction = false;
     int wide_occ = 0;
+    int hex_map = 0;
   } route;
   StageTimer timers[ILQR_NUM_STAGES];
   std::vector<hipEvent_t> event_pool;
@@ -117,7 +119,7 @@
   f.D = (float*)v.D; f.cand_u = (float*)v.cand_u; f.cand_x = (float*)v.cand_x; f.nch = v.nch;
   f.cost_c = v.cost_c; f.cost = v.cost; f.lambda = v.lambda; f.dlambda = v.dlambda; f.dV = v.dV; f.gnorm = v.gnorm;
   f.status = v.status; f.iters = v.iters; f.flg_change = v.flg_change; f.alpha_idx = v.alpha_idx; f.diverge = v.diverge;
-  f.backpass_done = v.backpass_done; f.n_running = v.n_running; f.analytic = v.analytic;
+  f.backpass_done = v.backpass_done; f.n_running = v.n_running; f.analytic = v.analytic; f.qp_load = v.qp_load;
 }
 template <class F>
 static int with_real(ilqr_batch* h, F&& f) {
diff --git a/ilqr_amd/csrc/hex_balance.hpp b/ilqr_amd/csrc/hex_balance.hpp
--- /dev/null
+++ b/ilqr_amd/csrc/hex_balance.hpp
@@ -0,0 +1,58 @@
+#pragma once
+
+#include <hip/hip_runtime.h>
+
+namespace ilqr {
+
+constexpr int kHexChains = 4, kHexPerChain = 4, kHexTile = kHexChains * kHexPerChain;
+constexpr int kHexLoadMax = (1 << 26) - 1;
+
+__host__ __device__ inline int hex_balance_key(int load, int idx) {
+  const int w = load < 0 ? 0 : load > kHexLoadMax ? kHexLoadMax : load;
+  return (w << 4) | (kHexTile - 1 - idx);
+}
+__host__ __device__ inline int hex_key_load(int key) { return key >> 4; }
+__host__ __device__ inline int hex_key_index(int key) { return kHexTile - 1 - (key & (kHexTile - 1)); }
+
+struct HexDeal {
+  int sum[kHexChains] = {0, 0, 0, 0}, cnt[kHexChains] = {0, 0, 0, 0};
+};
+__host__ __device__ inline int hex_deal_next(HexDeal& d, int load) {
+  int c = -1, best = 0;
+#pragma unroll
+  for (int k = 0; k < kHexChains; k++) {
+    const bool ok = d.cnt[k] < kHexPerChain && (c < 0 || d.sum[k] < best);
+    c = ok ? k : c;
+    best = ok ? d.sum[k] : best;
+  }
+  int pos = 0;
+#pragma unroll
+  for (int k = 0; k < kHexChains; k++) {
+    const bool take = (k == c);
+    pos = take ? d.cnt[k] : pos;
+    d.sum[k] += take ? load : 0;
+    d.cnt[k] += take ? 1 : 0;
+  }
+  return kHexPerChain * c + pos;
+}
+
+__host__ __device__ inline void hex_balance_map(const int load[kHexTile], int map[kHexTile]) {
+  int key[kHexTile];
+  for (int i = 0; i < kHexTile; i++) key[i] = hex_balance_key(load[i], i);
+  HexDeal d;
+  for (int r = 0; r < kHexTile; r++) {
+    for (int i = 0; i < kHexTile; i++) {
+      int rank = 0;
+      for (int j = 0; j < kHexTile; j++) rank += key[j] > key[i];
+      if (rank == r) map[hex_deal_next(d, hex_key_load(key[i]))] = hex_key_index(key[i]);
+    }
+  }
+}
+
+__host__ __device__ inline int hex_scrambled_map(int tile, int iteration, int place) {
+  const unsigned h = ((unsigned)tile * 2654435761u) ^ ((unsigned)iteration * 40503u + 0x9e3779b9u);
+  const unsigned mul = 2u * ((h >> 7) & 7u) + 1u, add = (h >> 13) & 15u;
+  return (int)(((unsigned)place * mul + add) & (kHexTile - 1));
+}
+
+}
diff --git a/ilqr_amd/csrc/launch.hpp b/ilqr_amd/csrc/launch.hpp
--- a/ilqr_amd/csrc/launch.hpp
+++ b/ilqr_amd/csrc/launch.hpp
@@ -136,6 +136,7 @@
   h->cands = Cands::none;
   h->commit_pending = false;
   HIPCHK(hipMemsetAsync(h->commit_idx, 0xFF, (size_t)h->Bp * sizeof(int), h->stream));
+  HIPCHK(hipMemsetAsync(h->v.qp_load, 0, (size_t)h->Bp * sizeof(int), h->stream));
   return 0;
 }
 static int fresh_trajectory(ilqr_batch* h) {
@@ -330,7 +331,11 @@
           switch (solve) {
             case Solve::wide: if constexpr (MM::NU == 1) { if (wide_one) solve_with(k_solve_wide<MM, MF, 1>, wide_blocks, 512); else solve_with(k_solve_wide<MM, MF, 2>, wide_blocks, 256); } break;
             case Solve::wide2: if constexpr (MM::NU == 2) solve_with(k_solve_wide2<MM, MF>, wide_blocks, 256); break;
-            case Solve::hex: if constexpr (MM::NU == 1) solve_with(k_solve_hex<MM, MF>, grid_tiles, 512); break;
+            case Solve::hex:
+              if constexpr (MM::NU == 1)
+                hipLaunchKernelGGL((k_solve_hex<MM, MF>), dim3(grid_tiles), dim3(512), 0, h->stream, v, m, fdm, al, h->sp, n_iters, h->sp.fixed_work, h->commit_idx, pending, ticks,
+                                   ticks ? h->chain_ticks : nullptr, h->route.hex_map);
+              break;
             case Solve::tile1: solve_with(k_solve_tile<MM, MF, 1>, grid_tiles, 256); break;
             case Solve::tile2: solve_with(k_solve_tile<MM, MF, 2>, grid_tiles, 256); break;
             case Solve::none: break;
diff --git a/ilqr_amd/csrc/profile.hpp b/ilqr_amd/csrc/profile.hpp
--- a/ilqr_amd/csrc/profile.hpp
+++ b/ilqr_amd/csrc/profile.hpp
@@ -15,6 +15,7 @@
     t.launches = 0;
   }
   HIPCHK(hipMemsetAsync(h->phase_ticks, 0, 5 * (size_t)h->ntiles * sizeof(long long), h->stream));
+  HIPCHK(hipMemsetAsync(h->chain_ticks, 0, 5 * (size_t)h->ntiles * sizeof(long long), h->stream));
   return 0;
 }
 int ilqr_profile_read(ilqr_batch* h, double ms_out[ILQR_NUM_STAGES], int launches_out[ILQR_NUM_STAGES]) {
@@ -61,6 +62,25 @@
   *mhz_out = (wall > 0) ? cyc / wall * h->wall_clock_khz * 1e-3 : 0.0;
   return 0;
 }
+int ilqr_profile_chain_clocks(ilqr_batch* h, double* chain_ms_out, double* slowest_ms_out, double* phase_ms_out, int* iterations_out) {
+  if (!h) return fail(ILQR_ERR_INVALID, "null handle");
+  std::vector<long long> tk(5 * (size_t)h->ntiles), ck(5 * (size_t)h->ntiles);
+  HIPCHK(hipMemcpyAsync(tk.data(), h->phase_ticks, tk.size() * sizeof(long long), hipMemcpyDeviceToHost, h->stream));
+  HIPCHK(hipMemcpyAsync(ck.data(), h->chain_ticks, ck.size() * sizeof(long long), hipMemcpyDeviceToHost, h->stream));
+  HIPCHK(hipStreamSynchronize(h->stream));
+  const double to_ms = 1.0 / h->wall_clock_khz;
+  for (int t = 0; t < h->ntiles; t++) {
+    if (chain_ms_out)
+      for (int c = 0; c < 4; c++) chain_ms_out[4 * t + c] = (double)ck[5 * t + c] * to_ms;
+    if (slowest_ms_out) slowest_ms_out[t] = (double)ck[5 * t + 4] * to_ms;
+    if (phase_ms_out) {
+      phase_ms_out[2 * t] = (double)tk[5 * t] * to_ms;
+      phase_ms_out[2 * t + 1] = (double)tk[5 * t + 1] * to_ms;
+    }
+    if (iterations_out) iterations_out[t] = (int)tk[5 * t + 2];
+  }
+  return 0;
+}
 const char* ilqr_stage_kernel_name(ilqr_batch* h, int stage) {
   static const RoutePlan kNoHandle{};
   return stage_kernel_name(h ? h->plan : kNoHandle, stage);
diff --git a/ilqr_amd/csrc/quad_lanes.hpp b/ilqr_amd/csrc/quad_lanes.hpp
--- a/ilqr_amd/csrc/quad_lanes.hpp
+++ b/ilqr_amd/csrc/quad_lanes.hpp
@@ -9,6 +9,7 @@
 constexpr int quad_lane_alpha(int lane) { return lane / kQuad; }
 constexpr int quad_lane_q(int lane) { return lane % kQuad; }
 constexpr int quad_traj(int s, int q) { return kQuad * s + q; }
+constexpr int quad_dealt(const int* map, int place) { return map ? map[place] : place; }
 constexpr int quad_fetch_row(int lane, int nrows) { return lane / kQuad < nrows ? lane / kQuad : nrows - 1; }
 
 constexpr int rollout_share_slot(int row, int l) { return ((row >> 1) * TW + l) * 2 + (row & 1); }
diff --git a/ilqr_amd/csrc/rollout.hpp b/ilqr_amd/csrc/rollout.hpp
--- a/ilqr_amd/csrc/rollout.hpp
+++ b/ilqr_amd/csrc/rollout.hpp
@@ -90,7 +90,7 @@
 __device__ __forceinline__ void rollout_tile(const BatchViewT<typename M::real>& v, const M& model, const AlphaSet& alphas, int n_alpha,
                                              double* __restrict__ cost_out, int mode, const SolverParams& sp,
                                              int* __restrict__ commit_idx, int tile, double* lds_cost, bool count_running = true, int rwave = -1,
-                                             typename M::real* share = nullptr) {
+                                             typename M::real* share = nullptr, const int* quad_map = nullptr) {
   using real = typename M::real;
   constexpr int NX = M::NX, NU = M::NU;
   static_assert(NG == 1 || (SHARE && GAINS && !ACCEPT), "several alpha groups per wavefront: the shared-row rollout of the wide tiles");
@@ -99,7 +99,7 @@
   static_assert(!CANDT || (CAND && SHARE && GAINS && NU == 1 && NX == 4 && PD % CG == 0), "grouped candidates: the matrix-core kernel's rollouts (nx = 4, nu = 1)");
   const int wave = (rwave >= 0) ? rwave : (int)(threadIdx.x >> 6);
   const int lane = threadIdx.x & 63;
-  const int l = QUAD ? quad_traj(wave & 3, quad_lane_q(lane)) : lane & (TW - 1);
+  const int l = QUAD ? quad_dealt(quad_map, quad_traj(wave & 3, quad_lane_q(lane))) : lane & (TW - 1);
   const bool idle = QUAD && lane >= quad_rollout_lanes(NALPHA);
   const int a_sub = lane >> 4;
   const int b = tile * TW + l;
diff --git a/include/ilqr_amd.h b/include/ilqr_amd.h
--- a/include/ilqr_amd.h
+++ b/include/ilqr_amd.h
@@ -97,7 +97,9 @@
   ILQR_ROUTE_LQ_DENSE_FD = 2048,
   ILQR_ROUTE_WAVE_PER_TRAJECTORY = 4096,
   ILQR_ROUTE_BACKWARD_W2 = 1024,
-  ILQR_ROUTE_TWO_CONTROL_TILES = 8192
+  ILQR_ROUTE_TWO_CONTROL_TILES = 8192,
+  ILQR_ROUTE_HEX_BALANCED_MAP = 16384,
+  ILQR_ROUTE_HEX_SCRAMBLED_MAP = 32768
 };
 
 const char* ilqr_last_error(void);
@@ -230,6 +232,8 @@
 int ilqr_profile_reset(ilqr_batch* h);
 int ilqr_profile_read(ilqr_batch* h, double ms_out[ILQR_NUM_STAGES], int launches_out[ILQR_NUM_STAGES]);
 int ilqr_profile_shader_clock(ilqr_batch* h, double* mhz_out);
+int ilqr_get_hex_load(ilqr_batch* h, int* load_out);
+int ilqr_profile_chain_clocks(ilqr_batch* h, double* chain_ms_out, double* slowest_ms_out, double* phase_ms_out, int* iterations_out);
 const char* ilqr_stage_kernel_name(ilqr_batch* h, int stage);
 
 #ifdef __cplusplus
```

After: 4.585 billion trajectory-timesteps/s. 1.1% lower.
